# mir-group/nequip

Hardware: AMD Instinct MI355X
Metric: atom-steps/s (energy+forces) for 10k-atom l_max=2 box at 1/2/4/8 MI355X (higher is better)
Workload: dtype f32; 1 GPU; water10k: 10125-atom water box, 400558 edges, r_max 4.5, l_max=2, 64 features, 3 layers, parity=False, radial MLP 8-128(x1)-W, fp32 model / fp64 positions, energy+forces (autograd), random-init weights; atoms_per_gpu=10125, edges_per_gpu=400558, parallelism=replicas x1 (frames independent, no data-path collective), launch=hipGraph replay, radial-MLP backward on a side stream (parallel graph branch)

## Files before the change

include/nequip_amd.h:

```cpp
#ifndef NEQUIP_AMD_H
#define NEQUIP_AMD_H

#include <stdint.h>

#ifdef __cplusplus
extern "C" {
#endif

#define NQA_ABI_VERSION 1

enum nqa_status {
  NQA_OK = 0,
  NQA_ERR_INVALID = -1,
  NQA_ERR_UNSUPPORTED = -2,
  NQA_ERR_LAUNCH = -3,
  NQA_ERR_WORKSPACE = -4
};

enum nqa_dtype { NQA_F32 = 0, NQA_F64 = 1 };
enum nqa_layout { NQA_LAYOUT_MUL_IR = 0, NQA_LAYOUT_IR_MUL = 1 };

enum nqa_plan_field {
  NQA_PLAN_DIM_IN1 = 0,
  NQA_PLAN_DIM_IN2 = 1,
  NQA_PLAN_DIM_OUT = 2,
  NQA_PLAN_WEIGHT_NUMEL = 3,
  NQA_PLAN_NUM_INSTR = 4,
  NQA_PLAN_OUT_NEEDS_ZERO = 5,
  NQA_PLAN_YPART_WIDTH = 6,
  NQA_PLAN_HAS_SPECIALIZED = 7,
  NQA_PLAN_FUSED_ROWS_OK = 8
};

typedef struct nqa_plan nqa_plan;
typedef void* nqa_stream;

int nqa_abi_version(void);
const char* nqa_last_error(void);
int nqa_lmax(void);
int nqa_sh_lmax(void);

int nqa_plan_create(int32_t n_in1, const int32_t* in1_mul, const int32_t* in1_l, const int32_t* in1_p,
                    int32_t n_in2, const int32_t* in2_mul, const int32_t* in2_l, const int32_t* in2_p,
                    int32_t n_out, const int32_t* out_mul, const int32_t* out_l, const int32_t* out_p,
                    int32_t n_instr, const int32_t* instr_i1, const int32_t* instr_i2,
                    const int32_t* instr_io, const double* instr_path_weight,
                    int32_t layout_in1, int32_t layout_out, nqa_plan** plan);
void nqa_plan_destroy(nqa_plan* plan);
int64_t nqa_plan_query(const nqa_plan* plan, int32_t field);
int64_t nqa_plan_image_bytes(const nqa_plan* plan);
int nqa_plan_image_write(const nqa_plan* plan, void* host_dst, int64_t host_dst_bytes);

int64_t nqa_csr_workspace_bytes(int64_t num_nodes, int64_t num_edges);
int nqa_csr_build(const int64_t* key, const int64_t* other, int64_t num_nodes, int64_t num_edges,
                  int32_t* rowptr, int32_t* edge_id, int32_t* other_sorted, int32_t* status_flag,
                  void* workspace, int64_t workspace_bytes, nqa_stream stream);

int nqa_tp_scatter_fwd(const nqa_plan* plan, const void* plan_image, int32_t dtype, const void* x, const void* y, const void* w,
                       const int32_t* rowptr_dst, const int32_t* edge_id_dst, const int32_t* src_sorted,
                       void* out, int64_t num_nodes, int64_t num_edges, nqa_stream stream);

int64_t nqa_tp_bwd_edge_workspace_bytes(const nqa_plan* plan, int32_t dtype, int64_t num_edges);
int nqa_tp_scatter_bwd_edge(const nqa_plan* plan, const void* plan_image, int32_t dtype, const void* x, const void* y, const void* w,
                            const void* grad_out, const int32_t* rowptr_dst, const int32_t* edge_id_dst,
                            const int32_t* src_sorted, void* grad_w, void* grad_y, void* workspace,
                            int64_t workspace_bytes, int64_t num_nodes, int64_t num_edges, nqa_stream stream);

int nqa_tp_scatter_bwd_x(const nqa_plan* plan, const void* plan_image, int32_t dtype, const void* y, const void* w, const void* grad_out,
                         const int32_t* rowptr_src, const int32_t* edge_id_src, const int32_t* dst_sorted,
                         void* grad_x, int64_t num_nodes, int64_t num_edges, nqa_stream stream);

int64_t nqa_tp_bwd_fused_workspace_bytes(const nqa_plan* plan, int32_t dtype, int64_t num_edges);
int nqa_tp_scatter_bwd_fused(const nqa_plan* plan, const void* plan_image, int32_t dtype, const void* x, const void* y,
                             const void* w, const void* grad_out, const int32_t* rowptr_dst,
                             const int32_t* edge_id_dst, const int32_t* src_sorted, const int32_t* rowptr_src,
                             const int32_t* edge_id_src, void* grad_w, void* grad_y, void* grad_x, void* workspace,
                             int64_t workspace_bytes, int64_t num_nodes, int64_t num_edges, nqa_stream stream);

int nqa_edge_vectors_fwd(const double* pos, const int64_t* edge_dst, const int64_t* edge_src,
                         const double* edge_cell_shift, const double* cell, const int64_t* batch,
                         int64_t num_edges, double* edge_vec, nqa_stream stream);
int nqa_edge_vectors_bwd(const double* g_edge_vec, const double* edge_cell_shift, const int32_t* rowptr_dst,
                         const int32_t* edge_id_dst, const int32_t* rowptr_src, const int32_t* edge_id_src,
                         int64_t num_nodes, double sign, double* g_pos, double* g_cell_per_node, nqa_stream stream);
int nqa_virial_finalize(const double* per_atom, const int64_t* batch, const double* cell, int64_t num_nodes,
                        int64_t num_frames, double* virial, double* stress, nqa_stream stream);
int nqa_frame_sum(const double* rows, const int64_t* batch, int64_t num_nodes, int32_t width, int64_t num_frames,
                  double* out, nqa_stream stream);

int nqa_edge_embed_fwd(int32_t dtype, int32_t lmax, const double* edge_vec, int64_t num_edges,
                       double rmax_recip, const double* rmax_recip_edge, int32_t num_bessels,
                       const double* bessel_weights, double cutoff_p, double factor, void* sh, void* emb,
                       void* cutoff, nqa_stream stream);
int nqa_edge_embed_bwd(int32_t dtype, int32_t lmax, const double* edge_vec, int64_t num_edges,
                       double rmax_recip, const double* rmax_recip_edge, int32_t num_bessels,
                       const double* bessel_weights, double cutoff_p, double factor, const void* g_sh,
                       const void* g_emb, double* g_edge_vec, nqa_stream stream);
int nqa_edge_embed_fwd_paired(int32_t dtype, int32_t lmax, const double* edge_vec, int64_t num_edges,
                              double rmax_recip, int32_t num_bessels, const double* bessel_weights, double cutoff_p,
                              double factor, const int32_t* pair_row, int64_t num_pairs, void* sh, void* emb,
                              void* emb_pairs, nqa_stream stream);
int nqa_edge_embed_bwd_paired(int32_t dtype, int32_t lmax, const double* edge_vec, int64_t num_edges,
                              double rmax_recip, int32_t num_bessels, const double* bessel_weights, double cutoff_p,
                              double factor, const int32_t* pair_row, int64_t num_pairs, const void* g_sh,
                              const void* g_emb, const void* g_emb_pairs, double* g_edge_vec, nqa_stream stream);
int nqa_edge_embed_bwd_bwd(int32_t dtype, int32_t lmax, const double* edge_vec, int64_t num_edges,
                           double rmax_recip, const double* rmax_recip_edge, int32_t num_bessels,
                           const double* bessel_weights, double cutoff_p, double factor, const void* g_sh,
                           const void* g_emb, const double* cot_g_edge_vec, void* gg_sh, void* gg_emb,
                           double* g_edge_vec2, nqa_stream stream);

#define NQA_MLP_FP32 0
#define NQA_MLP_BF16X6 1
#define NQA_MLP_F16X3 2
#define NQA_MLP_HINT_DEVICE_IS_IDLE 0x100
int nqa_radial_mlp_supported(int32_t dtype, int32_t num_basis, int32_t hidden, int32_t out_features);
int64_t nqa_radial_mlp_workspace_bytes(int32_t mode, int32_t backward, int32_t hidden, int32_t out_features);
int nqa_radial_mlp_fwd(int32_t dtype, int32_t mode, const void* edge_embedding, const void* w0, double alpha0,
                       const void* w1, double alpha1, int32_t num_basis, int32_t hidden, int32_t out_features,
                       int64_t num_edges, void* edge_weight, void* workspace, int64_t workspace_bytes,
                       int32_t workspace_ready, nqa_stream stream);
int nqa_radial_mlp_bwd(int32_t dtype, int32_t mode, const void* edge_embedding, const void* w0, double alpha0,
                       const void* w1, double alpha1, const void* grad_edge_weight, int32_t num_basis,
                       int32_t hidden, int32_t out_features, int64_t num_edges, void* grad_edge_embedding,
                       void* workspace, int64_t workspace_bytes, int32_t workspace_ready, nqa_stream stream);

int nqa_radial_mlp_bwd_paired(int32_t dtype, int32_t mode, const void* edge_embedding, const void* w0, double alpha0,
                              const void* w1, double alpha1, const void* grad_edge_weight,
                              const void* grad_edge_weight2, int32_t num_basis, int32_t hidden, int32_t out_features,
                              int64_t num_edges, void* grad_edge_embedding, void* workspace, int64_t workspace_bytes,
                              int32_t workspace_ready, nqa_stream stream);
int64_t nqa_radial_mlp_train_tiles(int64_t num_edges);
int nqa_radial_mlp_bwd_train(int32_t dtype, int32_t mode, const void* edge_embedding, const void* cotangent,
                             const void* w0, double alpha0, const void* w1, double alpha1,
                             const void* grad_edge_weight, int32_t num_basis, int32_t hidden, int32_t out_features,
                             int64_t num_edges, void* grad_edge_embedding, void* hidden_out, void* w0_partials,
                             void* workspace, int64_t workspace_bytes, int32_t workspace_ready, nqa_stream stream);
int nqa_radial_mlp_fwd_tangent(int32_t dtype, int32_t mode, const void* edge_embedding, const void* cotangent,
                               const void* w0, double alpha0, const void* w1, double alpha1, int32_t num_basis,
                               int32_t hidden, int32_t out_features, int64_t num_edges, void* out, void* workspace,
                               int64_t workspace_bytes, int32_t workspace_ready, nqa_stream stream);

int nqa_radial_mlp_last_fwd(int32_t dtype, int32_t mode, const void* pre, const void* w, double alpha, int32_t hidden,
                            int32_t out_features, int64_t num_edges, void* out, void* workspace, int64_t workspace_bytes,
                            int32_t workspace_ready, nqa_stream stream);
int nqa_radial_mlp_last_bwd(int32_t dtype, int32_t mode, const void* pre, const void* w, double alpha,
                            const void* grad_out, const void* grad_out2, int32_t hidden, int32_t out_features,
                            int64_t num_edges, void* grad_pre, void* workspace, int64_t workspace_bytes,
                            int32_t workspace_ready, nqa_stream stream);


int nqa_node_linear(int32_t dtype, const void* x, const void* weights, const void* addend, void* out,
                    const int64_t* atom_types, const void* chunk_table, int32_t n_chunks, const void* instr_table,
                    int32_t n_instr, int32_t n_types, int64_t weight_stride, int32_t dim_in, int32_t dim_out,
                    int64_t num_nodes, double scale, int32_t chunk_width, nqa_stream stream);
int nqa_node_linear_ordered(int32_t dtype, const void* x, const void* weights, const void* addend, void* out,
                            const int64_t* atom_types, const int32_t* atom_order, const void* chunk_table, int32_t n_chunks,
                            const void* instr_table, int32_t n_instr, int32_t n_types, int64_t weight_stride,
                            int32_t dim_in, int32_t dim_out, int64_t num_nodes, double scale, int32_t chunk_width,
                            nqa_stream stream);
int nqa_gate(int32_t dtype, int32_t backward, const void* input, const void* grad_out, const void* cotangent,
             void* out, const void* col_table, int32_t dim_in, int32_t dim_out, int64_t num_nodes, nqa_stream stream);

int64_t nqa_node_weights_pack_bytes(const void* chunk_table, int32_t n_chunks, const void* instr_table, int32_t n_instr,
                                    int32_t n_types);
int nqa_node_weights_pack(const void* weights, const void* chunk_table, int32_t n_chunks, const void* instr_table,
                          int32_t n_instr, int32_t n_types, int64_t weight_stride, void* packed, nqa_stream stream);
int nqa_node_linear_packed(const void* x, const void* packed, const void* addend, void* out, const int64_t* atom_types,
                           const void* chunk_table, int32_t n_chunks, const void* instr_table, int32_t n_instr,
                           int32_t n_types, int32_t dim_in, int32_t dim_out, int64_t num_nodes, double scale,
                           nqa_stream stream);
int nqa_node_linear_packed_ordered(const void* x, const void* packed, const void* addend, void* out,
                                   const int64_t* atom_types, const int32_t* atom_order, const void* chunk_table,
                                   int32_t n_chunks, const void* instr_table, int32_t n_instr, int32_t n_types,
                                   int32_t dim_in, int32_t dim_out, int64_t num_nodes, double scale, nqa_stream stream);

typedef struct nqa_gate_block {
  int32_t out_off, d, mul, val_off, gate_off, act;
  double cst;
} nqa_gate_block;

typedef struct nqa_node_part {
  const void* x;
  const void* packed;
  const void* chunk_table;
  const void* instr_table;
  int32_t n_chunks, n_instr, n_types, dim_in;
  void* out;
  const void* addend;
  int32_t dim_out, accumulate;
  double scale;
  const nqa_gate_block* in_gate;
  int32_t n_in_gate, pad;
} nqa_node_part;

int nqa_node_fused(const nqa_node_part* parts, int32_t n_parts, const int64_t* atom_types, const int32_t* atom_order,
                   int64_t num_nodes, const nqa_gate_block* out_gate, int32_t n_out_gate, const void* gate_h,
                   int32_t gate_dim, nqa_stream stream);
int nqa_node_fused_plan(const nqa_node_part* parts, int32_t n_parts, const nqa_gate_block* out_gate, int32_t n_out_gate,
                        int32_t* chunks_out, int32_t chunks_cap, int32_t* instr_out, int32_t instr_cap);

int nqa_energy_head(int32_t backward, const void* h, const void* readout_weight, const void* scales, int32_t n_scales,
                    const void* shifts, int32_t n_shifts, const int64_t* atom_types, const void* grad_e, void* out,
                    int32_t dim, int32_t act, double cst, int64_t num_nodes, nqa_stream stream);

int64_t nqa_energy_head_train_workspace_bytes(int64_t num_nodes, int32_t dim, int32_t n_scales, int32_t n_shifts);
int nqa_energy_head_train_bwd(const void* h, const void* readout_weight, const void* scales, int32_t n_scales,
                              int32_t n_shifts, const int64_t* atom_types, const void* grad_e, void* grad_h, void* grad_w,
                              void* grad_scales, void* grad_shifts, void* workspace, int64_t workspace_bytes, int32_t dim,
                              int32_t act, double cst, int64_t num_nodes, nqa_stream stream);
int nqa_energy_head_train_bwd_bwd(const void* h, const void* readout_weight, const void* scales, int32_t n_scales,
                                  const int64_t* atom_types, const void* grad_e, const void* cot_grad_h, void* grad_grad_e,
                                  void* grad_h, void* grad_w, void* grad_scales, void* workspace, int64_t workspace_bytes,
                                  int32_t dim, int32_t act, double cst, int64_t num_nodes, nqa_stream stream);

int nqa_zbl_fwd(const double* edge_vec, const int32_t* rowptr_dst, const int32_t* edge_id_dst, const int32_t* src_sorted,
                const int64_t* atom_types, const double* z_table, const double* rmax_recip_edge, double rmax_recip, double p,
                int32_t round_f32, const double* qqr2e_half, int64_t num_nodes, int64_t num_out, const double* pe_in,
                double* pe_out, nqa_stream stream);
int nqa_zbl_bwd(const double* edge_vec, const int32_t* rowptr_dst, const int32_t* edge_id_dst, const int32_t* src_sorted,
                const int64_t* atom_types, const double* z_table, const double* rmax_recip_edge, double rmax_recip, double p,
                int32_t round_f32, const double* qqr2e_half, int64_t num_nodes, int64_t num_out, const double* g_pe,
                double* g_edge_vec, nqa_stream stream);
int nqa_zbl_bwd_bwd(const double* edge_vec, const int32_t* rowptr_dst, const int32_t* edge_id_dst,
                    const int32_t* src_sorted, const int64_t* atom_types, const double* z_table,
                    const double* rmax_recip_edge, double rmax_recip, double p, int32_t round_f32, const double* qqr2e_half,
                    int64_t num_nodes, int64_t num_out, const double* g_pe, const double* cot_edge_vec, double* gg_pe,
                    double* g_edge_vec2, nqa_stream stream);

int64_t nqa_edge_pairs_workspace_bytes(int64_t num_edges);
int nqa_edge_pairs(const int64_t* edge_dst, const int64_t* edge_src, const void* edge_cell_shift, int32_t shift_dtype,
                   const int32_t* rowptr_dst, const int32_t* edge_id_dst, const int32_t* src_sorted, int64_t num_edges,
                   int64_t num_nodes, void* workspace, int64_t workspace_bytes, int32_t* weight_rows, int64_t* rep_edge,
                   int32_t* partner_edge, int32_t* ok, nqa_stream stream);
int nqa_csr_from_pairs(const int32_t* edge_id_dst, const int32_t* partner_edge, int64_t num_edges, int32_t* edge_id_src,
                       nqa_stream stream);
int nqa_pair_gather(const void* rows_in, const int64_t* rep_edge, int64_t num_pairs, int32_t width, void* rows_out,
                    nqa_stream stream);
int64_t nqa_pair_owner_workspace_bytes(int64_t num_edges, int64_t num_nodes);
int nqa_pair_owner_lists(const int32_t* weight_rows, const int64_t* rep_edge, const int32_t* rowptr_dst,
                         const int32_t* edge_id_dst, const int32_t* src_sorted, int64_t num_edges, int64_t num_nodes,
                         void* workspace, int64_t workspace_bytes, int32_t* owner_rowptr, int32_t* pair_other,
                         int32_t* pair_row, int32_t* pair_edge_in, int32_t* pair_edge_out, int32_t* other_rowptr,
                         int32_t* other_slot, nqa_stream stream);
int nqa_pair_owner_lists_guard(const int32_t* ok, int64_t num_nodes, int32_t* owner_rowptr, int32_t* other_rowptr,
                               nqa_stream stream);
int nqa_pair_expand(const void* pair_rows, const int32_t* weight_rows, int64_t num_edges, int64_t num_pairs,
                    int32_t width, void* edge_rows, nqa_stream stream);
int nqa_tp_scatter_fwd_paired(const nqa_plan* plan, const void* plan_image, int32_t dtype, const void* x, const void* y,
                              const void* w, const int32_t* rowptr_dst, const int32_t* edge_id_dst,
                              const int32_t* src_sorted, void* out, int64_t num_nodes, int64_t num_edges,
                              const int32_t* weight_rows, int64_t num_pairs, nqa_stream stream);
int nqa_tp_scatter_bwd_edge_paired(const nqa_plan* plan, const void* plan_image, int32_t dtype, const void* x,
                                   const void* y, const void* w, const void* grad_out, const int32_t* rowptr_dst,
                                   const int32_t* edge_id_dst, const int32_t* src_sorted, void* grad_w, void* grad_y,
                                   void* workspace, int64_t workspace_bytes, int64_t num_nodes, int64_t num_edges,
                                   const int32_t* weight_rows, int64_t num_pairs, nqa_stream stream);
int nqa_tp_scatter_bwd_fused_paired(const nqa_plan* plan, const void* plan_image, int32_t dtype, const void* x,
                                    const void* y, const void* w, const void* grad_out, const int32_t* rowptr_dst,
                                    const int32_t* edge_id_dst, const int32_t* src_sorted, const int32_t* rowptr_src,
                                    const int32_t* edge_id_src, void* grad_w, void* grad_y, void* grad_x,
                                    void* workspace, int64_t workspace_bytes, int64_t num_nodes, int64_t num_edges,
                                    const int32_t* weight_rows, int64_t num_pairs, nqa_stream stream);
int nqa_tp_scatter_bwd_x_paired(const nqa_plan* plan, const void* plan_image, int32_t dtype, const void* y,
                                const void* w, const void* grad_out, const int32_t* rowptr_src,
                                const int32_t* edge_id_src, const int32_t* dst_sorted, void* grad_x, int64_t num_nodes,
                                int64_t num_edges, const int32_t* weight_rows, int64_t num_pairs, nqa_stream stream);

int64_t nqa_tp_bwd_pairs_workspace_bytes(const nqa_plan* plan, int32_t dtype, int64_t num_edges);
int nqa_tp_scatter_bwd_pairs(const nqa_plan* plan, const void* plan_image, int32_t dtype, const void* x, const void* y,
                             const void* w, const void* grad_out, const int32_t* owner_rowptr,
                             const int32_t* pair_other, const int32_t* pair_row, const int32_t* pair_edge_in,
                             const int32_t* pair_edge_out, const int32_t* other_rowptr, const int32_t* other_slot,
                             void* grad_w, void* grad_y, void* grad_x, void* workspace, int64_t workspace_bytes,
                             int64_t num_nodes, int64_t num_edges, nqa_stream stream);

int32_t nqa_tp_bwd_pairs_dual_supported(const nqa_plan* plan, int32_t dtype);
int nqa_tp_scatter_bwd_pairs_dual(const nqa_plan* plan, const void* plan_image, int32_t dtype, const void* x,
                                  const void* x_cot, const void* y, const void* y_cot, const void* w, const void* w_cot,
                                  const void* grad_out, const int32_t* owner_rowptr, const int32_t* pair_other,
                                  const int32_t* pair_row, const int32_t* pair_edge_in, const int32_t* pair_edge_out,
                                  void* grad_w, void* grad_y, void* workspace, int64_t workspace_bytes,
                                  int64_t num_nodes, int64_t num_edges, nqa_stream stream);

int32_t nqa_tp_fwd_jvp_supported(const nqa_plan* plan, int32_t dtype);
int nqa_tp_scatter_fwd_jvp(const nqa_plan* plan, const void* plan_image, int32_t dtype, const void* x, const void* y,
                           const void* w, const void* x_cot, const void* y_cot, const void* w_cot,
                           const int32_t* rowptr_dst, const int32_t* edge_id_dst, const int32_t* src_sorted, void* out,
                           int64_t num_nodes, int64_t num_edges, const int32_t* weight_rows, int64_t num_pairs,
                           nqa_stream stream);
int nqa_tp_scatter_bwd_x_dual(const nqa_plan* plan, const void* plan_image, int32_t dtype, const void* y, const void* w,
                              const void* y_cot, const void* w_cot, const void* grad_out, const int32_t* rowptr_src,
                              const int32_t* edge_id_src, const int32_t* dst_sorted, void* grad_x, int64_t num_nodes,
                              int64_t num_edges, const int32_t* weight_rows, int64_t num_pairs, nqa_stream stream);

int32_t nqa_wgrad_splits(const void* instr_table, int32_t n_instr, int32_t n_types, int64_t num_rows);
int nqa_wgrad(int32_t dtype, const void* a_rows, const void* b_rows, const int64_t* row_types,
              const void* instr_table, int32_t n_instr, int64_t lda, int64_t ldb, int64_t num_rows, int32_t n_types,
              int64_t out_stride, int32_t splits, void* partials, nqa_stream stream);

int64_t nqa_neighbor_list_workspace_bytes(int64_t num_atoms);
int nqa_neighbor_list_count(const double* pos, const double* cell, const int32_t* pbc, double r_max, int64_t num_atoms,
                            void* workspace, int64_t workspace_bytes, int32_t* rowptr, nqa_stream stream);
int nqa_neighbor_list_fill(const void* workspace, const int32_t* rowptr, int64_t num_atoms, int64_t num_edges,
                           int64_t* edge_index, double* edge_cell_shift, nqa_stream stream);
int nqa_neighbor_list_fill_padded(const void* workspace, const int32_t* rowptr, int64_t num_atoms, int64_t edge_capacity,
                                  int32_t* rowptr_padded, int64_t* edge_index, double* edge_cell_shift, int32_t* src_sorted,
                                  int32_t* status, nqa_stream stream);
int64_t nqa_neighbor_list_batched_workspace_bytes(int64_t num_atoms, int64_t num_frames);
int nqa_neighbor_list_batched_count(const double* pos, const double* cell, const int32_t* pbc, const int64_t* frame_ptr,
                                    double r_max, int64_t num_atoms, int64_t num_frames, void* workspace,
                                    int64_t workspace_bytes, int32_t* rowptr, int32_t* status, nqa_stream stream);
int nqa_neighbor_list_batched_fill(const void* workspace, const int32_t* rowptr, int64_t num_atoms, int64_t num_frames,
                                   int64_t num_edges, int64_t* edge_index, double* edge_cell_shift, nqa_stream stream);
int64_t nqa_neighbor_list_typed_workspace_bytes(int64_t num_atoms, int64_t num_types);
int nqa_neighbor_list_count_typed(const double* pos, const double* cell, const int32_t* pbc, double r_max,
                                  const int64_t* atom_types, const double* cutoff_table, int64_t num_types, int32_t symmetrise,
                                  int64_t num_atoms, void* workspace, int64_t workspace_bytes, int32_t* rowptr, int32_t* status,
                                  nqa_stream stream);
int nqa_neighbor_list_fill_typed(const void* workspace, const int32_t* rowptr, const int64_t* atom_types, int64_t num_atoms,
                                 int64_t num_types, int64_t num_edges, int64_t* edge_index, double* edge_cell_shift,
                                 nqa_stream stream);
int nqa_neighbor_list_fill_padded_typed(const void* workspace, const int32_t* rowptr, const int64_t* atom_types,
                                        int64_t num_atoms, int64_t num_types, int64_t edge_capacity, int32_t* rowptr_padded,
                                        int64_t* edge_index, double* edge_cell_shift, int32_t* src_sorted, int32_t* status,
                                        nqa_stream stream);
int64_t nqa_neighbor_list_batched_typed_workspace_bytes(int64_t num_atoms, int64_t num_frames, int64_t num_types);
int nqa_neighbor_list_batched_count_typed(const double* pos, const double* cell, const int32_t* pbc, const int64_t* frame_ptr,
                                          double r_max, const int64_t* atom_types, const double* cutoff_table,
                                          int64_t num_types, int64_t num_atoms, int64_t num_frames, void* workspace,
                                          int64_t workspace_bytes, int32_t* rowptr, int32_t* status, nqa_stream stream);
int nqa_neighbor_list_batched_fill_typed(const void* workspace, const int32_t* rowptr, const int64_t* atom_types,
                                         int64_t num_atoms, int64_t num_frames, int64_t num_types, int64_t num_edges,
                                         int64_t* edge_index, double* edge_cell_shift, nqa_stream stream);


#define NQA_METRICS_MAX_STREAMS 8
#define NQA_METRICS_MAX_TERMS 32
#define NQA_METRICS_MAX_TYPES 16
#define NQA_METRICS_MAX_STRATA 8
#define NQA_METRICS_GROUPS 64

enum nqa_metric_kind {
  NQA_METRIC_MSE = 0,
  NQA_METRIC_MAE = 1,
  NQA_METRIC_RMSE = 2,
  NQA_METRIC_MAXABS = 3,
  NQA_METRIC_HUBER = 4,
  NQA_METRIC_STRATIFIED_HUBER = 5
};

typedef struct nqa_metric_stream {
  const void* pred;
  const void* target;
  const double* row_scale;
  const int64_t* group;
  void* grad_pred;
  int64_t rows;
  int32_t cols, pred_dtype, target_dtype, pad;
} nqa_metric_stream;

typedef struct nqa_metric_term {
  int32_t stream, kind, n_groups, ignore_nan, reduce_sum, n_strata, has_coeff, has_group_coeffs, slot0, out0;
  double coeff, delta;
  double bound[NQA_METRICS_MAX_STRATA], stratum_delta[NQA_METRICS_MAX_STRATA];
  double group_coeff[NQA_METRICS_MAX_TYPES];
} nqa_metric_term;

int32_t nqa_metrics_groups(void);
int64_t nqa_metrics_workspace_bytes(int32_t n_slots);
int nqa_metrics_fwd(const nqa_metric_stream* streams, int32_t n_streams, const nqa_metric_term* terms,
                    const nqa_metric_term* terms_device, int32_t n_terms, int32_t n_values, int32_t weighted_sum_index,
                    void* workspace, int64_t workspace_bytes, void* state, void* saved, double* values, nqa_stream stream);
int nqa_metrics_bwd(const nqa_metric_stream* streams, int32_t n_streams, const nqa_metric_term* terms,
                    const nqa_metric_term* terms_device, int32_t n_terms, int32_t n_values, int32_t weighted_sum_index,
                    const void* saved, const double* grad_values, nqa_stream stream);

typedef struct nqa_mt_chunk {
  int64_t offset;
  int32_t tensor, pad;
} nqa_mt_chunk;

#define NQA_EMA_CHUNK 1024

typedef struct nqa_ema_tensor {
  void* ema;
  void* param;
  int64_t numel;
  int32_t dtype, pad;
} nqa_ema_tensor;

int32_t nqa_ema_chunk_elems(void);
int nqa_ema_update(const nqa_ema_tensor* tensors, const nqa_mt_chunk* chunks, int64_t chunk_capacity, const int64_t* n_chunks,
                   double decay, int64_t* counter, nqa_stream stream);
int nqa_ema_swap(const nqa_ema_tensor* tensors, const nqa_mt_chunk* chunks, int64_t chunk_capacity, const int64_t* n_chunks,
                 nqa_stream stream);

typedef struct nqa_sfree_tensor {
  void* param;
  void* grad;
  void* z;
  void* exp_avg_sq;
  int64_t numel;
  int32_t dtype, group;
} nqa_sfree_tensor;

typedef struct nqa_sfree_group {
  double lr, beta1, beta2, eps, weight_decay, r, weight_lr_power;
  int64_t warmup_steps;
  int64_t k;
  double weight_sum, lr_max, scheduled_lr;
} nqa_sfree_group;

int nqa_sfree_step(const nqa_sfree_tensor* tensors, const nqa_mt_chunk* chunks, int64_t chunk_capacity, const int64_t* n_chunks,
                   nqa_sfree_group* groups, int32_t n_groups, nqa_stream stream);
int nqa_sfree_swap(const nqa_sfree_tensor* tensors, const nqa_mt_chunk* chunks, int64_t chunk_capacity, const int64_t* n_chunks,
                   const nqa_sfree_group* groups, int32_t n_groups, int32_t to_eval, nqa_stream stream);

typedef struct nqa_adam_tensor {
  void* param;
  const void* grad;
  void* exp_avg;
  void* exp_avg_sq;
  void* max_exp_avg_sq;
  float* step;
  int64_t numel;
  int32_t dtype, group;
} nqa_adam_tensor;
// ... 171 lines not shown
```

nequip_amd/_lib.py:

```python

from __future__ import annotations

import ctypes
import os
import threading
from ctypes import POINTER, c_char_p, c_double, c_int32, c_int64, c_uint64, c_void_p

_HERE = os.path.dirname(os.path.abspath(__file__))
LIB_PATH = os.path.join(_HERE, "csrc", "libnequip_amd.so")

NQA_OK = 0
NQA_F32 = 0
NQA_F64 = 1
NQA_MLP_FP32 = 0
NQA_MLP_BF16X6 = 1
NQA_MLP_F16X3 = 2
NQA_MLP_HINT_DEVICE_IS_IDLE = 0x100
NQA_LAYOUT_MUL_IR = 0
NQA_LAYOUT_IR_MUL = 1

NQA_PLAN_DIM_IN1 = 0
NQA_PLAN_DIM_IN2 = 1
NQA_PLAN_DIM_OUT = 2
NQA_PLAN_WEIGHT_NUMEL = 3
NQA_PLAN_NUM_INSTR = 4
NQA_PLAN_OUT_NEEDS_ZERO = 5
NQA_PLAN_YPART_WIDTH = 6
NQA_PLAN_HAS_SPECIALIZED = 7
NQA_PLAN_FUSED_ROWS_OK = 8

_P32 = POINTER(c_int32)


class GateBlock(ctypes.Structure):

    _fields_ = [("out_off", c_int32), ("d", c_int32), ("mul", c_int32), ("val_off", c_int32), ("gate_off", c_int32),
                ("act", c_int32), ("cst", c_double)]


class NodePart(ctypes.Structure):

    _fields_ = [("x", c_void_p), ("packed", c_void_p), ("chunk_table", c_void_p), ("instr_table", c_void_p),
                ("n_chunks", c_int32), ("n_instr", c_int32), ("n_types", c_int32), ("dim_in", c_int32),
                ("out", c_void_p), ("addend", c_void_p), ("dim_out", c_int32), ("accumulate", c_int32),
                ("scale", c_double), ("in_gate", c_void_p), ("n_in_gate", c_int32), ("pad", c_int32)]


NQA_METRICS_MAX_STREAMS = 8
NQA_METRICS_MAX_TERMS = 32
NQA_METRICS_MAX_TYPES = 16
NQA_METRICS_MAX_STRATA = 8
NQA_METRICS_GROUPS = 64
NQA_METRIC_MSE, NQA_METRIC_MAE, NQA_METRIC_RMSE, NQA_METRIC_MAXABS, NQA_METRIC_HUBER, NQA_METRIC_STRATIFIED_HUBER = range(6)


class MetricStream(ctypes.Structure):

    _fields_ = [("pred", c_void_p), ("target", c_void_p), ("row_scale", c_void_p), ("group", c_void_p),
                ("grad_pred", c_void_p), ("rows", c_int64), ("cols", c_int32), ("pred_dtype", c_int32),
                ("target_dtype", c_int32), ("pad", c_int32)]


class MetricTerm(ctypes.Structure):

    _fields_ = [("stream", c_int32), ("kind", c_int32), ("n_groups", c_int32), ("ignore_nan", c_int32),
                ("reduce_sum", c_int32), ("n_strata", c_int32), ("has_coeff", c_int32), ("has_group_coeffs", c_int32),
                ("slot0", c_int32), ("out0", c_int32), ("coeff", c_double), ("delta", c_double),
                ("bound", c_double * NQA_METRICS_MAX_STRATA), ("stratum_delta", c_double * NQA_METRICS_MAX_STRATA),
                ("group_coeff", c_double * NQA_METRICS_MAX_TYPES)]


NQA_STATS_MAX_STREAMS = 8
NQA_STATS_MAX_TERMS = 32
NQA_STATS_MAX_NODE_TYPES = 128
NQA_STATS_MAX_EDGE_TYPES = 16
NQA_STATS_MAX_SLOTS = 1024
NQA_STATS_GROUPS = 256
NQA_STATS_F32, NQA_STATS_F64, NQA_STATS_I32, NQA_STATS_I64 = range(4)
NQA_STATS_MOD_IDENTITY, NQA_STATS_MOD_ABS, NQA_STATS_MOD_SQUARE = range(3)
NQA_STATS_GROUP_NONE, NQA_STATS_GROUP_NODE, NQA_STATS_GROUP_EDGE = range(3)


class StatsStream(ctypes.Structure):

    _fields_ = [("data", c_void_p), ("row_scale", c_void_p), ("atom_types", c_void_p), ("edge_index", c_void_p),
                ("rows", c_int64), ("num_atoms", c_int64), ("cols", c_int32), ("dtype", c_int32), ("group_kind", c_int32),
                ("num_types", c_int32)]


class StatsTerm(ctypes.Structure):

    _fields_ = [("stream", c_int32), ("mod", c_int32), ("n_groups", c_int32), ("ignore_nan", c_int32), ("slot0", c_int32),
                ("pad", c_int32 * 3)]


SIGNATURES = {
    "nqa_abi_version": (c_int32, []),
    "nqa_last_error": (c_char_p, []),
    "nqa_lmax": (c_int32, []),
    "nqa_sh_lmax": (c_int32, []),
    "nqa_plan_create": (
        c_int32,
        [c_int32, _P32, _P32, _P32, c_int32, _P32, _P32, _P32, c_int32, _P32, _P32, _P32]
        + [c_int32, _P32, _P32, _P32, POINTER(c_double), c_int32, c_int32, POINTER(c_void_p)],
    ),
    "nqa_plan_destroy": (None, [c_void_p]),
    "nqa_plan_query": (c_int64, [c_void_p, c_int32]),
    "nqa_plan_image_bytes": (c_int64, [c_void_p]),
    "nqa_plan_image_write": (c_int32, [c_void_p, c_void_p, c_int64]),
    "nqa_csr_workspace_bytes": (c_int64, [c_int64, c_int64]),
    "nqa_csr_build": (
        c_int32,
        [c_void_p, c_void_p, c_int64, c_int64, c_void_p, c_void_p, c_void_p, c_void_p, c_void_p, c_int64, c_void_p],
    ),
    "nqa_tp_scatter_fwd": (
        c_int32,
        [c_void_p, c_void_p, c_int32, c_void_p, c_void_p, c_void_p, c_void_p, c_void_p, c_void_p, c_void_p]
        + [c_int64, c_int64, c_void_p],
    ),
    "nqa_tp_bwd_edge_workspace_bytes": (c_int64, [c_void_p, c_int32, c_int64]),
    "nqa_tp_scatter_bwd_edge": (
        c_int32,
        [c_void_p, c_void_p, c_int32, c_void_p, c_void_p, c_void_p, c_void_p, c_void_p, c_void_p, c_void_p]
        + [c_void_p, c_void_p, c_void_p, c_int64, c_int64, c_int64, c_void_p],
    ),
    "nqa_tp_bwd_fused_workspace_bytes": (c_int64, [c_void_p, c_int32, c_int64]),
    "nqa_tp_scatter_bwd_fused": (
        c_int32,
        [c_void_p, c_void_p, c_int32, c_void_p, c_void_p, c_void_p, c_void_p]
        + [c_void_p] * 5
        + [c_void_p, c_void_p, c_void_p, c_void_p, c_int64, c_int64, c_int64, c_void_p],
    ),
    "nqa_tp_scatter_bwd_x": (
        c_int32,
        [c_void_p, c_void_p, c_int32, c_void_p, c_void_p, c_void_p, c_void_p, c_void_p, c_void_p, c_void_p]
        + [c_int64, c_int64, c_void_p],
    ),
    "nqa_frame_sum": (c_int32, [c_void_p, c_void_p, c_int64, c_int32, c_int64, c_void_p, c_void_p]),
    "nqa_edge_pairs_workspace_bytes": (c_int64, [c_int64]),
    "nqa_edge_pairs": (
        c_int32,
        [c_void_p, c_void_p, c_void_p, c_int32, c_void_p, c_void_p, c_void_p, c_int64, c_int64, c_void_p, c_int64, c_void_p,
         c_void_p, c_void_p, c_void_p, c_void_p],
    ),
    "nqa_csr_from_pairs": (c_int32, [c_void_p, c_void_p, c_int64, c_void_p, c_void_p]),
    "nqa_pair_owner_workspace_bytes": (c_int64, [c_int64, c_int64]),
    "nqa_pair_owner_lists": (
        c_int32,
        [c_void_p, c_void_p, c_void_p, c_void_p, c_void_p, c_int64, c_int64, c_void_p, c_int64, c_void_p, c_void_p, c_void_p,
         c_void_p, c_void_p, c_void_p, c_void_p, c_void_p],
    ),
    "nqa_pair_owner_lists_guard": (c_int32, [c_void_p, c_int64, c_void_p, c_void_p, c_void_p]),
    "nqa_pair_gather": (c_int32, [c_void_p, c_void_p, c_int64, c_int32, c_void_p, c_void_p]),
    "nqa_pair_expand": (c_int32, [c_void_p, c_void_p, c_int64, c_int64, c_int32, c_void_p, c_void_p]),
    "nqa_tp_bwd_pairs_workspace_bytes": (c_int64, [c_void_p, c_int32, c_int64]),
    "nqa_tp_scatter_bwd_pairs": (
        c_int32,
        [c_void_p, c_void_p, c_int32, c_void_p, c_void_p, c_void_p, c_void_p]
        + [c_void_p] * 7
        + [c_void_p, c_void_p, c_void_p, c_void_p, c_int64, c_int64, c_int64, c_void_p],
    ),
    "nqa_tp_fwd_jvp_supported": (c_int32, [c_void_p, c_int32]),
    "nqa_tp_scatter_fwd_jvp": (
        c_int32,
        [c_void_p, c_void_p, c_int32] + [c_void_p] * 6
        + [c_void_p, c_void_p, c_void_p, c_void_p, c_int64, c_int64, c_void_p, c_int64, c_void_p],
    ),
    "nqa_tp_scatter_bwd_x_dual": (
        c_int32,
        [c_void_p, c_void_p, c_int32] + [c_void_p] * 5
        + [c_void_p, c_void_p, c_void_p, c_void_p, c_int64, c_int64, c_void_p, c_int64, c_void_p],
    ),
    "nqa_tp_bwd_pairs_dual_supported": (c_int32, [c_void_p, c_int32]),
    "nqa_tp_scatter_bwd_pairs_dual": (
        c_int32,
        [c_void_p, c_void_p, c_int32] + [c_void_p] * 7
        + [c_void_p] * 5
        + [c_void_p, c_void_p, c_void_p, c_int64, c_int64, c_int64, c_void_p],
    ),
    "nqa_edge_vectors_fwd": (
        c_int32,
        [c_void_p, c_void_p, c_void_p, c_void_p, c_void_p, c_void_p, c_int64, c_void_p, c_void_p],
    ),
    "nqa_edge_vectors_bwd": (
        c_int32,
        [c_void_p, c_void_p, c_void_p, c_void_p, c_void_p, c_void_p, c_int64, c_double, c_void_p, c_void_p, c_void_p],
    ),
    "nqa_virial_finalize": (c_int32, [c_void_p, c_void_p, c_void_p, c_int64, c_int64, c_void_p, c_void_p, c_void_p]),
    "nqa_edge_embed_fwd": (
        c_int32,
        [c_int32, c_int32, c_void_p, c_int64, c_double, c_void_p, c_int32, c_void_p, c_double, c_double]
        + [c_void_p, c_void_p, c_void_p, c_void_p],
    ),
    "nqa_edge_embed_bwd": (
        c_int32,
        [c_int32, c_int32, c_void_p, c_int64, c_double, c_void_p, c_int32, c_void_p, c_double, c_double]
        + [c_void_p, c_void_p, c_void_p, c_void_p],
    ),
    "nqa_edge_embed_fwd_paired": (
        c_int32,
        [c_int32, c_int32, c_void_p, c_int64, c_double, c_int32, c_void_p, c_double, c_double, c_void_p, c_int64]
        + [c_void_p, c_void_p, c_void_p, c_void_p],
    ),
    "nqa_edge_embed_bwd_paired": (
        c_int32,
        [c_int32, c_int32, c_void_p, c_int64, c_double, c_int32, c_void_p, c_double, c_double, c_void_p, c_int64]
        + [c_void_p, c_void_p, c_void_p, c_void_p, c_void_p],
    ),
    "nqa_edge_embed_bwd_bwd": (
        c_int32,
        [c_int32, c_int32, c_void_p, c_int64, c_double, c_void_p, c_int32, c_void_p, c_double, c_double]
        + [c_void_p, c_void_p, c_void_p, c_void_p, c_void_p, c_void_p, c_void_p],
    ),
    "nqa_radial_mlp_supported": (c_int32, [c_int32, c_int32, c_int32, c_int32]),
    "nqa_radial_mlp_workspace_bytes": (c_int64, [c_int32, c_int32, c_int32, c_int32]),
    "nqa_radial_mlp_fwd": (
        c_int32,
        [c_int32, c_int32, c_void_p, c_void_p, c_double, c_void_p, c_double, c_int32, c_int32, c_int32, c_int64]
        + [c_void_p, c_void_p, c_int64, c_int32, c_void_p],
    ),
    "nqa_radial_mlp_bwd": (
        c_int32,
        [c_int32, c_int32, c_void_p, c_void_p, c_double, c_void_p, c_double, c_void_p, c_int32, c_int32, c_int32]
        + [c_int64, c_void_p, c_void_p, c_int64, c_int32, c_void_p],
    ),
    "nqa_node_linear": (
        c_int32,
        [c_int32, c_void_p, c_void_p, c_void_p, c_void_p, c_void_p, c_void_p, c_int32, c_void_p, c_int32, c_int32]
        + [c_int64, c_int32, c_int32, c_int64, c_double, c_int32, c_void_p],
    ),
    "nqa_node_weights_pack_bytes": (c_int64, [c_void_p, c_int32, c_void_p, c_int32, c_int32]),
    "nqa_node_weights_pack": (
        c_int32, [c_void_p, c_void_p, c_int32, c_void_p, c_int32, c_int32, c_int64, c_void_p, c_void_p],
    ),
    "nqa_node_linear_packed": (
        c_int32,
        [c_void_p, c_void_p, c_void_p, c_void_p, c_void_p, c_void_p, c_int32, c_void_p, c_int32, c_int32, c_int32, c_int32]
        + [c_int64, c_double, c_void_p],
    ),
    "nqa_node_linear_ordered": (
        c_int32,
        [c_int32, c_void_p, c_void_p, c_void_p, c_void_p, c_void_p, c_void_p, c_void_p, c_int32, c_void_p, c_int32, c_int32,
         c_int64, c_int32, c_int32, c_int64, c_double, c_int32, c_void_p],
    ),
    "nqa_node_linear_packed_ordered": (
        c_int32,
        [c_void_p, c_void_p, c_void_p, c_void_p, c_void_p, c_void_p, c_void_p, c_int32, c_void_p, c_int32, c_int32, c_int32]
        + [c_int32, c_int64, c_double, c_void_p],
    ),
    "nqa_node_fused": (
        c_int32, [c_void_p, c_int32, c_void_p, c_void_p, c_int64, c_void_p, c_int32, c_void_p, c_int32, c_void_p],
    ),
    "nqa_node_fused_plan": (c_int32, [c_void_p, c_int32, c_void_p, c_int32, _P32, c_int32, _P32, c_int32]),
    "nqa_radial_mlp_last_fwd": (
        c_int32,
        [c_int32, c_int32, c_void_p, c_void_p, c_double, c_int32, c_int32, c_int64, c_void_p, c_void_p, c_int64, c_int32,
         c_void_p],
    ),
    "nqa_radial_mlp_last_bwd": (
        c_int32,
        [c_int32, c_int32, c_void_p, c_void_p, c_double, c_void_p, c_void_p, c_int32, c_int32, c_int64, c_void_p, c_void_p,
         c_int64, c_int32, c_void_p],
    ),
    "nqa_energy_head": (
        c_int32,
        [c_int32, c_void_p, c_void_p, c_void_p, c_int32, c_void_p, c_int32, c_void_p, c_void_p, c_void_p, c_int32, c_int32,
         c_double, c_int64, c_void_p],
    ),
    "nqa_energy_head_train_workspace_bytes": (c_int64, [c_int64, c_int32, c_int32, c_int32]),
    "nqa_energy_head_train_bwd": (
        c_int32,
        [c_void_p, c_void_p, c_void_p, c_int32, c_int32, c_void_p, c_void_p, c_void_p, c_void_p, c_void_p, c_void_p, c_void_p,
         c_int64, c_int32, c_int32, c_double, c_int64, c_void_p],
    ),
    "nqa_energy_head_train_bwd_bwd": (
        c_int32,
        [c_void_p, c_void_p, c_void_p, c_int32, c_void_p, c_void_p, c_void_p, c_void_p, c_void_p, c_void_p, c_void_p, c_void_p,
         c_int64, c_int32, c_int32, c_double, c_int64, c_void_p],
    ),
    "nqa_zbl_fwd": (
        c_int32,
        [c_void_p, c_void_p, c_void_p, c_void_p, c_void_p, c_void_p, c_void_p, c_double, c_double, c_int32, c_void_p, c_int64,
         c_int64, c_void_p, c_void_p, c_void_p],
    ),
    "nqa_zbl_bwd": (
        c_int32,
        [c_void_p, c_void_p, c_void_p, c_void_p, c_void_p, c_void_p, c_void_p, c_double, c_double, c_int32, c_void_p, c_int64,
         c_int64, c_void_p, c_void_p, c_void_p],
    ),
    "nqa_zbl_bwd_bwd": (
        c_int32,
        [c_void_p, c_void_p, c_void_p, c_void_p, c_void_p, c_void_p, c_void_p, c_double, c_double, c_int32, c_void_p, c_int64,
         c_int64, c_void_p, c_void_p, c_void_p, c_void_p, c_void_p],
    ),
    "nqa_neighbor_list_workspace_bytes": (c_int64, [c_int64]),
    "nqa_neighbor_list_count": (
        c_int32,
        [c_void_p, c_void_p, c_void_p, c_double, c_int64, c_void_p, c_int64, c_void_p, c_void_p],
    ),
    "nqa_neighbor_list_fill": (c_int32, [c_void_p, c_void_p, c_int64, c_int64, c_void_p, c_void_p, c_void_p]),
    "nqa_neighbor_list_fill_padded": (
        c_int32, [c_void_p, c_void_p, c_int64, c_int64, c_void_p, c_void_p, c_void_p, c_void_p, c_void_p, c_void_p]),
    "nqa_neighbor_list_batched_workspace_bytes": (c_int64, [c_int64, c_int64]),
    "nqa_neighbor_list_batched_count": (
        c_int32,
        [c_void_p, c_void_p, c_void_p, c_void_p, c_double, c_int64, c_int64, c_void_p, c_int64, c_void_p, c_void_p, c_void_p],
    ),
    "nqa_neighbor_list_batched_fill": (c_int32, [c_void_p, c_void_p, c_int64, c_int64, c_int64, c_void_p, c_void_p, c_void_p]),
    "nqa_neighbor_list_typed_workspace_bytes": (c_int64, [c_int64, c_int64]),
    "nqa_neighbor_list_count_typed": (
        c_int32,
        [c_void_p, c_void_p, c_void_p, c_double, c_void_p, c_void_p, c_int64, c_int32, c_int64, c_void_p, c_int64, c_void_p,
         c_void_p, c_void_p],
# ... 151 lines not shown
```

nequip_amd/csrc/radial_mlp.hip:

```cpp
#include <hip/hip_runtime.h>

#include <cstdint>
#include <cstdlib>
#include <string>
#include <type_traits>

#include "launch_status.h"
#include "mfma_split.h"

namespace nqa {

constexpr int kMlpRows = 128;
constexpr int kMaxNb = 8;

typedef float mlp_v4f __attribute__((ext_vector_type(4)));
__device__ __forceinline__ void mlp_store4(float* p, const float4& v) {
  __builtin_nontemporal_store((mlp_v4f){v.x, v.y, v.z, v.w}, reinterpret_cast<mlp_v4f*>(p));
}

__device__ __forceinline__ void lds_barrier() { asm volatile("s_waitcnt lgkmcnt(0)\n\ts_barrier" ::: "memory"); }

__device__ __forceinline__ float silu_f(float x) { return x / (1.0f + __expf(-x)); }
__device__ __forceinline__ void silu_all_f(float x, float& h, float& d1, float& d2) {
  const float sig = 1.0f / (1.0f + __expf(-x));
// ... 698 lines not shown
      } else {
#pragma unroll
        for (int s2 = 0; s2 < kMaxNb / 2; ++s2) {
          const float av = (2 * s2 + half) < nb ? w0v[kb][s2] * a0 : 0.f;
          const float bv = half ? e[2 * s2 + 1] : e[2 * s2];
          hacc = __builtin_amdgcn_mfma_f32_32x32x2f32(av, bv, hacc, 0, 0, 0);
        }
      }
#pragma unroll
      for (int r = 0; r < 16; r += 2) {
        const float h0 = row_ok ? (XIN ? silu_given_f(hacc[r]) : silu_f(hacc[r])) : 0.f;
        const float h1 = row_ok ? (XIN ? silu_given_f(hacc[r + 1]) : silu_f(hacc[r + 1])) : 0.f;
        if constexpr (F16) {
          hv[kb * 16 + r] = h0;
          hv[kb * 16 + r + 1] = h1;
        } else {
          uint32_t a, b, c;
          split_pair(h0, h1, a, b, c);
          const int s = 2 * kb + (r >> 3), tp = (r & 7) >> 1;
          bh[s][tp] = a; bm[s][tp] = b; bl[s][tp] = c;
        }
      }
    }
    if constexpr (F16) {
      float m = 0.f;
#pragma unroll
      for (int i = 0; i < (H / 32) * 16; ++i) m = fmaxf(m, fabsf(hv[i]));
      m = fmaxf(m, __shfl_xor(m, 32));
      const float su = f16_scale_up(m);
      row_scale = 1.f / su;
#pragma unroll
      for (int kb = 0; kb < H / 32; ++kb) {
#pragma unroll
        for (int r = 0; r < 16; r += 2) {
          uint32_t a, b;
          split_pair_f16(hv[kb * 16 + r] * su, hv[kb * 16 + r + 1] * su, a, b);
          const int s = 2 * kb + (r >> 3), tp = (r & 7) >> 1;
          bh[s][tp] = a; bl[s][tp] = b;
        }
      }
    }
  };
  hidden(ev, blk * kMlpRows + wv * 32 + l31 < E, blk);

  float* __restrict__ tb = tbuf + wv * (32 * kTS);
  auto emit = [&](const f32x16& pa, const f32x16& pb, int tile, int64_t wrow0, float rs) __attribute__((always_inline)) {
    if constexpr (F16) {
      const float f = rs * tile_scale[tile];
#pragma unroll
      for (int g = 0; g < 4; ++g)
        *reinterpret_cast<float4*>(tb + l31 * kTS + 8 * g + 4 * half) =
            make_float4((pa[4 * g] + pb[4 * g]) * f, (pa[4 * g + 1] + pb[4 * g + 1]) * f,
                        (pa[4 * g + 2] + pb[4 * g + 2]) * f, (pa[4 * g + 3] + pb[4 * g + 3]) * f);
    } else {
#pragma unroll
      for (int g = 0; g < 4; ++g)
        *reinterpret_cast<float4*>(tb + l31 * kTS + 8 * g + 4 * half) =
            make_float4(pa[4 * g] + pb[4 * g], pa[4 * g + 1] + pb[4 * g + 1], pa[4 * g + 2] + pb[4 * g + 2],
                        pa[4 * g + 3] + pb[4 * g + 3]);
    }
    const int n0 = tile * 32;
    const int c4 = lane & 7, rsub = lane >> 3;
    if (wrow0 + 32 <= E && n0 + 32 <= W) {
      float* __restrict__ ob = out + (wrow0 + rsub) * W + n0 + 4 * c4;
#pragma unroll
      for (int i = 0; i < 4; ++i)
        mlp_store4(ob + (int64_t)(8 * i) * W, *reinterpret_cast<const float4*>(tb + (8 * i + rsub) * kTS + 4 * c4));
    } else {
#pragma unroll
      for (int i = 0; i < 4; ++i) {
        const int r = 8 * i + rsub;
        const float4 v = *reinterpret_cast<const float4*>(tb + r * kTS + 4 * c4);
        if (wrow0 + r < E && n0 + 4 * c4 + 3 < W) *reinterpret_cast<float4*>(out + (wrow0 + r) * W + n0 + 4 * c4) = v;
      }
    }
  };
  int prev_tile = 0;
  int64_t prev_row0 = 0;
  float prev_rs = 1.f;
  auto unit = [&](int64_t i, f32x16& accA, f32x16& accB, const f32x16& prevA, const f32x16& prevB)
      __attribute__((always_inline)) {
    const int64_t left = (u1 - u0) - i;
    if (t == 0 && i > 0) {
      ++blk;
#pragma unroll
      for (int c = 0; c < kMaxNb; ++c) ev[c] = evn[c];
      hidden(ev, blk * kMlpRows + wv * 32 + l31 < E, blk);
    }
    const int buf = (int)(i & 1);
    if (left > 1) stage_store(buf ^ 1);
    if (left > 2) stage_load(tile_after(t, 2));
    if (t == ntiles - 1 && left > 1) load_ev(blk + 1, evn);
    const u32x4* __restrict__ a = as[buf] + lane;
    accA = (f32x16){0};
    accB = (f32x16){0};
    u32x4 fa[2][NPL];
#pragma unroll
    for (int q = 0; q < NPL; ++q) fa[0][q] = a[q * 64];
#pragma unroll
    for (int s = 0; s < KS; ++s) {
      if (s + 1 < KS) {
#pragma unroll
        for (int q = 0; q < NPL; ++q) fa[(s + 1) & 1][q] = a[((s + 1) * NPL + q) * 64];
      }
      __builtin_amdgcn_sched_barrier(0);
      if constexpr (F16) {
        const u32x4 &ah = fa[s & 1][0], &al = fa[s & 1][1];
        if (s & 1) {
          accB = mfma_f16(ah, bl[s], accB);
          accA = mfma_f16(al, bh[s], accA);
          accB = mfma_f16(ah, bh[s], accB);
        } else {
          accA = mfma_f16(ah, bl[s], accA);
          accB = mfma_f16(al, bh[s], accB);
          accA = mfma_f16(ah, bh[s], accA);
        }
      } else {
        const u32x4 &ah = fa[s & 1][0], &am = fa[s & 1][1], &al = fa[s & 1][2];
        accA = mfma_bf16(ah, bh[s], accA);
        accB = mfma_bf16(am, bm[s], accB);
        accA = mfma_bf16(ah, bm[s], accA);
        accB = mfma_bf16(ah, bl[s], accB);
        accA = mfma_bf16(am, bh[s], accA);
        accB = mfma_bf16(al, bh[s], accB);
      }
      __builtin_amdgcn_sched_barrier(0);
      if (s == 1 && i > 0) {
        emit(prevA, prevB, prev_tile, prev_row0, prev_rs);
        __builtin_amdgcn_sched_barrier(0);
      }
    }
    lds_barrier();
    prev_tile = t;
    prev_row0 = blk * kMlpRows + wv * 32;
    prev_rs = row_scale;
    if (++t == ntiles) t = 0;
  };
  f32x16 a0A, a0B, a1A, a1B;
  const int64_t n = u1 - u0;
  for (int64_t i = 0; i < n; i += 2) {
    unit(i, a0A, a0B, a1A, a1B);
    if (i + 1 < n) unit(i + 1, a1A, a1B, a0A, a0B);
  }
  if (n & 1)
    emit(a0A, a0B, prev_tile, prev_row0, prev_rs);
  else
    emit(a1A, a1B, prev_tile, prev_row0, prev_rs);
}

}
#include "radial_mlp_pipe.h"
namespace nqa {

template <int H, int TM, bool PAIR = false, bool F16 = false, bool XIN = false>
__global__ __launch_bounds__(256, 2) void radial_mlp_bwd_split_kernel(const float* __restrict__ emb,
                                                                    const float* __restrict__ W0,
                                                                    const u32x4* __restrict__ Wb,
                                                                    const float* __restrict__ gw, float a0, int nb,
                                                                    int W, int64_t E, float* __restrict__ g_emb,
                                                                    int dbg, const float* __restrict__ cemb,
                                                                    float* __restrict__ hid_out,
                                                                    float* __restrict__ w0_part,
                                                                    const float* __restrict__ gw2 = nullptr,
                                                                    const int* __restrict__ chunk_exp = nullptr) {
  constexpr int NT = H / 32;
  constexpr int NPL = F16 ? 2 : 3;
  constexpr int CH = 2 * NPL * NT * 64;
  constexpr int NV = CH / 256;
  constexpr int GS = H + 1;
  constexpr int kMainBytes = 2 * CH * 16;
  constexpr int kEpiBytes = kMlpRows * GS * 4;
  constexpr int kBufBytes = kMainBytes > kEpiBytes ? kMainBytes : kEpiBytes;
  __shared__ __align__(16) unsigned char smem_raw[kBufBytes];
  __shared__ float w0s[H * kMaxNb];
  __shared__ float w0t[kMaxNb * H];
  __shared__ float es[kMlpRows * kMaxNb];
  __shared__ int rowexp[F16 ? kMlpRows : 1];
  __shared__ float cs_own[(TM == 2 && H * kMaxNb < kMlpRows * kMaxNb) ? kMlpRows * kMaxNb : 1];
  float* __restrict__ cs = (H * kMaxNb >= kMlpRows * kMaxNb) ? w0s : cs_own;
  u32x4* __restrict__ bsm = reinterpret_cast<u32x4*>(smem_raw);
  const int tid = threadIdx.x;
  const int lane = tid & 63;
  const int wv = tid >> 6;
  const int half = lane >> 5;
  const int l31 = lane & 31;
  const int64_t blk0 = (int64_t)blockIdx.x * kMlpRows;
  const int64_t myrow = blk0 + wv * 32 + l31;
  const bool row_ok = myrow < E;

  if constexpr (!XIN) {
    for (int i = tid; i < H * kMaxNb; i += 256) {
      const int k = i / kMaxNb, c = i - k * kMaxNb;
      const float v = c < nb ? W0[c * H + k] * a0 : 0.f;
      w0s[i] = v;
      w0t[c * H + k] = v;
    }
    for (int i = tid; i < kMlpRows * kMaxNb; i += 256) {
      const int r = i / kMaxNb, c = i - r * kMaxNb;
      const int64_t rr = blk0 + r < E ? blk0 + r : E - 1;
      const float v = emb[rr * nb + (c < nb ? c : nb - 1)];
      es[i] = (c < nb && blk0 + r < E) ? v : 0.f;
    }
  }
  float cvr[kMaxNb];
  if (TM == 2) {
    const float* __restrict__ cr = cemb + (row_ok ? myrow : (E - 1)) * nb;
#pragma unroll
    for (int c = 0; c < kMaxNb; ++c) cvr[c] = cr[c < nb ? c : nb - 1];
#pragma unroll
    for (int c = 0; c < kMaxNb; ++c) cvr[c] = (row_ok && c < nb) ? cvr[c] : 0.f;
  }

  const int nchunks = (W + 31) / 32;
  u32x4 pb[NV];
  const float* __restrict__ grow = gw + (row_ok ? myrow : 0) * W + 16 * half;
  const float* __restrict__ grow2 = PAIR ? gw2 + (row_ok ? myrow : 0) * W + 16 * half : nullptr;
  const bool rows_full = blk0 + kMlpRows <= E;
  auto load_rows = [&](const float* __restrict__ gr, int ch, float4 (&pa)[4]) {
    if (rows_full && 32 * ch + 32 <= W) {
#pragma unroll
      for (int v = 0; v < 4; ++v) pa[v] = *reinterpret_cast<const float4*>(gr + 32 * ch + 4 * v);
    } else {
#pragma unroll
      for (int v = 0; v < 4; ++v) {
        const int k = 32 * ch + 16 * half + 4 * v;
        pa[v] = (row_ok && k + 3 < W) ? *reinterpret_cast<const float4*>(gr + 32 * ch + 4 * v)
                                      : make_float4(0.f, 0.f, 0.f, 0.f);
      }
    }
  };
  auto load_a = [&](int ch, float4 (&pa)[4], float4 (&pc)[4]) {
    if (dbg & 1) return;
    load_rows(grow, ch, pa);
    if (PAIR) load_rows(grow2, ch, pc);
  };
  auto load_b = [&](int ch) {
#pragma unroll
    for (int v = 0; v < NV; ++v) pb[v] = Wb[(int64_t)ch * CH + tid + v * 256];
  };
  auto store_b = [&](int buf) {
#pragma unroll
    for (int v = 0; v < NV; ++v) bsm[buf * CH + tid + v * 256] = pb[v];
  };
  float4 paA[4], paB[4];
  float4 pcA[PAIR ? 4 : 1], pcB[PAIR ? 4 : 1];
  load_b(0);
  load_a(0, paA, reinterpret_cast<float4(&)[4]>(pcA));
  store_b(0);
  if (nchunks > 1) load_a(1, paB, reinterpret_cast<float4(&)[4]>(pcB));
  __syncthreads();

  f32x16 acc[NT];
#pragma unroll
  for (int t = 0; t < NT; ++t) acc[t] = (f32x16){0};
  constexpr int kUnset = 1 << 20;
  int S = kUnset;
  int we_next = F16 ? chunk_exp[0] : 0;
  auto rows_from_lanes = [&](int value, int (&out)[16]) __attribute__((always_inline)) {
    int* __restrict__ rb = rowexp + wv * 32;
    if (half == 0) rb[l31] = value;
    __builtin_amdgcn_fence(__ATOMIC_RELEASE, "wavefront");
    __builtin_amdgcn_wave_barrier();
    __builtin_amdgcn_fence(__ATOMIC_ACQUIRE, "wavefront");
#pragma unroll
    for (int r = 0; r < 16; ++r) out[r] = rb[(r & 3) + 8 * (r >> 2) + 4 * half];
    __builtin_amdgcn_fence(__ATOMIC_RELEASE, "wavefront");
    __builtin_amdgcn_wave_barrier();
  };

  auto body = [&](int ch, float4 (&pa)[4], float4 (&pc)[4]) {
    const int buf = ch & 1;
    if (PAIR) {
#pragma unroll
      for (int v = 0; v < 4; ++v) {
        pa[v].x += pc[v].x; pa[v].y += pc[v].y; pa[v].z += pc[v].z; pa[v].w += pc[v].w;
      }
    }
    u32x4 ah[2], am[F16 ? 1 : 2], al[2];
    if constexpr (F16) {
      const int we = we_next;
      if (ch + 1 < nchunks) we_next = chunk_exp[ch + 1];
      float m = 0.f;
#pragma unroll
      for (int v = 0; v < 4; ++v)
        m = fmaxf(m, fmaxf(fmaxf(fabsf(pa[v].x), fabsf(pa[v].y)), fmaxf(fabsf(pa[v].z), fabsf(pa[v].w))));
      m = fmaxf(m, __shfl_xor(m, 32));
      int shift = 0;
      if (m > 0.f && m < 3.0e38f) {
        int em;
        (void)frexpf(m, &em);
        const int cap = 15 - em + we;
        if (cap < S) {
          int ns = cap - 3;
          ns = ns > we + 100 ? we + 100 : (ns < we - 100 ? we - 100 : ns);
          shift = S == kUnset ? 0 : S - ns;
          S = ns;
        }
      }
      if (ch > 0 && __any(shift > 0)) {
        int kr[16];
        rows_from_lanes(shift, kr);
#pragma unroll
        for (int t = 0; t < NT; ++t)
#pragma unroll
          for (int r = 0; r < 16; ++r) acc[t][r] = ldexpf(acc[t][r], -kr[r]);
      }
      int q = S == kUnset ? 0 : S - we;
      q = q > 120 ? 120 : (q < -120 ? -120 : q);
      const float qs = ldexpf(1.f, q);
#pragma unroll
      for (int s = 0; s < 2; ++s) {
        uint32_t a, b;
        split_pair_f16(pa[2 * s].x * qs, pa[2 * s].y * qs, a, b);
        ah[s][0] = a; al[s][0] = b;
        split_pair_f16(pa[2 * s].z * qs, pa[2 * s].w * qs, a, b);
        ah[s][1] = a; al[s][1] = b;
        split_pair_f16(pa[2 * s + 1].x * qs, pa[2 * s + 1].y * qs, a, b);
// ... 23 lines not shown
      if constexpr (F16) {
#pragma unroll
        for (int q = 0; q < 2; ++q)
#pragma unroll
          for (int t = 0; t < NT; ++t) fb[q][t] = bs[((s * 2 + q) * NT + t) * 64];
        __builtin_amdgcn_sched_barrier(0);
#pragma unroll
        for (int t = 0; t < NT; ++t) acc[t] = mfma_f16(al[s], fb[0][t], acc[t]);
#pragma unroll
        for (int t = 0; t < NT; ++t) acc[t] = mfma_f16(ah[s], fb[1][t], acc[t]);
#pragma unroll
        for (int t = 0; t < NT; ++t) acc[t] = mfma_f16(ah[s], fb[0][t], acc[t]);
        __builtin_amdgcn_sched_barrier(0);
        continue;
      }
      if (!(dbg & 16) || ch == 0) {
#pragma unroll
        for (int q = 0; q < 3; ++q)
#pragma unroll
          for (int t = 0; t < NT; ++t) fb[q][t] = bs[((s * 3 + q) * NT + t) * 64];
      } else {
#pragma unroll
        for (int q = 0; q < 3; ++q)
#pragma unroll
          for (int t = 0; t < NT; ++t) fb[q][t] = (u32x4){0x3f803f80u + (unsigned)lane, 0x3c003c00u, 0x38003800u + (unsigned)t, 0x3f803f80u + (unsigned)q};
      }
      __builtin_amdgcn_sched_barrier(0);
#pragma unroll
      for (int t = 0; t < NT; ++t) acc[t] = mfma_bf16(am[s], fb[1][t], acc[t]);
#pragma unroll
      for (int t = 0; t < NT; ++t) acc[t] = mfma_bf16(ah[s], fb[2][t], acc[t]);
#pragma unroll
      for (int t = 0; t < NT; ++t) acc[t] = mfma_bf16(al[s], fb[0][t], acc[t]);
#pragma unroll
      for (int t = 0; t < NT; ++t) acc[t] = mfma_bf16(ah[s], fb[1][t], acc[t]);
#pragma unroll
      for (int t = 0; t < NT; ++t) acc[t] = mfma_bf16(am[s], fb[0][t], acc[t]);
#pragma unroll
      for (int t = 0; t < NT; ++t) acc[t] = mfma_bf16(ah[s], fb[0][t], acc[t]);
      __builtin_amdgcn_sched_barrier(0);
    }
    if (ch + 1 < nchunks && !(dbg & 2) && !((dbg & 8) && (ch & 1))) store_b(buf ^ 1);
    if (!(dbg & 4)) lds_barrier();
  };
  for (int ch = 0; ch < nchunks; ch += 2) {
    body(ch, paA, reinterpret_cast<float4(&)[4]>(pcA));
    if (ch + 1 < nchunks) body(ch + 1, paB, reinterpret_cast<float4(&)[4]>(pcB));
  }

  if constexpr (F16) {
    int sr[16];
    rows_from_lanes(S == kUnset ? 0 : S, sr);
#pragma unroll
    for (int t = 0; t < NT; ++t)
#pragma unroll
      for (int r = 0; r < 16; ++r) acc[t][r] = ldexpf(acc[t][r], -sr[r]);
  }
  if constexpr (XIN) {
    static_assert(!XIN || TM == 0, "XIN is an inference backward");
#pragma unroll
    for (int t = 0; t < NT; ++t) {
      const int col = t * 32 + l31;
      float pv[16];
#pragma unroll
      for (int r = 0; r < 16; ++r) {
        const int64_t row = blk0 + wv * 32 + (r & 3) + 8 * (r >> 2) + 4 * half;
        pv[r] = emb[(row < E ? row : (E - 1)) * H + col];
      }
#pragma unroll
      for (int r = 0; r < 16; ++r) {
        const int64_t row = blk0 + wv * 32 + (r & 3) + 8 * (r >> 2) + 4 * half;
        if (row < E) g_emb[row * H + col] = acc[t][r] * silu_grad_given_f(pv[r]);
      }
    }
    return;
  }
  float* __restrict__ gp = reinterpret_cast<float*>(smem_raw);
  {
    const float* __restrict__ erow = es + (wv * 32 + l31) * kMaxNb;
#pragma unroll
    for (int t = 0; t < NT; ++t) {
      f32x16 pacc = {0};
#pragma unroll
      for (int s2 = 0; s2 < kMaxNb / 2; ++s2) {
        const float av = erow[2 * s2 + half];
        const float bv = w0t[(2 * s2 + half) * H + t * 32 + l31];
        pacc = __builtin_amdgcn_mfma_f32_32x32x2f32(av, bv, pacc, 0, 0, 0);
      }
      f32x16 qacc = {0};
      if (TM == 2) {
#pragma unroll
        for (int s2 = 0; s2 < kMaxNb / 2; ++s2) {
          const float av = half ? cvr[2 * s2 + 1] : cvr[2 * s2];
          const float bv = w0t[(2 * s2 + half) * H + t * 32 + l31];
          qacc = __builtin_amdgcn_mfma_f32_32x32x2f32(av, bv, qacc, 0, 0, 0);
        }
      }
      const int col = t * 32 + l31;
      if (TM == 0) {
#pragma unroll
        for (int r = 0; r < 16; ++r) {
          const int lr = wv * 32 + (r & 3) + 8 * (r >> 2) + 4 * half;
          gp[lr * GS + col] = acc[t][r] * silu_grad_f(pacc[r]);
        }
      } else {
        float hv[16];
#pragma unroll
        for (int r = 0; r < 16; ++r) {
          const int lr = wv * 32 + (r & 3) + 8 * (r >> 2) + 4 * half;
          float h, d1, d2;
          silu_all_f(pacc[r], h, d1, d2);
          if (TM == 1) {
            gp[lr * GS + col] = acc[t][r] * d1;
            hv[r] = h;
          } else {
            gp[lr * GS + col] = qacc[r] * acc[t][r] * d2;
            hv[r] = qacc[r] * d1;
            acc[t][r] *= d1;
          }
        }
        float* __restrict__ hrow = hid_out + (blk0 + wv * 32 + 4 * half) * (int64_t)H + col;
        if (rows_full) {
#pragma unroll
          for (int r = 0; r < 16; ++r) hrow[(int64_t)((r & 3) + 8 * (r >> 2)) * H] = hv[r];
        } else {
#pragma unroll
          for (int r = 0; r < 16; ++r) {
            const int lr = wv * 32 + (r & 3) + 8 * (r >> 2) + 4 * half;
            if (blk0 + lr < E) hrow[(int64_t)((r & 3) + 8 * (r >> 2)) * H] = hv[r];
          }
        }
      }
    }
  }
  __syncthreads();
  {
    const int r = tid >> 1, kh = tid & 1;
    float sacc[kMaxNb];
#pragma unroll
    for (int c = 0; c < kMaxNb; ++c) sacc[c] = 0.f;
    const float* __restrict__ gr = gp + r * GS + kh * (H / 2);
    const float* __restrict__ wr = w0s + kh * (H / 2) * kMaxNb;
#pragma unroll 4
    for (int k = 0; k < H / 2; ++k) {
      const float gv = gr[k];
      const float4 w0 = *reinterpret_cast<const float4*>(wr + k * kMaxNb);
      const float4 w1 = *reinterpret_cast<const float4*>(wr + k * kMaxNb + 4);
      sacc[0] += gv * w0.x; sacc[1] += gv * w0.y; sacc[2] += gv * w0.z; sacc[3] += gv * w0.w;
      sacc[4] += gv * w1.x; sacc[5] += gv * w1.y; sacc[6] += gv * w1.z; sacc[7] += gv * w1.w;
    }
#pragma unroll
    for (int c = 0; c < kMaxNb; ++c) sacc[c] += __shfl_xor(sacc[c], 1, 64);
    if (kh == 0 && blk0 + r < E) {
      for (int c = 0; c < nb; ++c) g_emb[(blk0 + r) * nb + c] = sacc[c];
    }
  }
  if (TM != 0) {
    constexpr int NCG = 256 / H, CPT = kMaxNb / NCG;
    const int k = tid % H, cg = tid / H;
    float part[CPT];
#pragma unroll
    for (int i = 0; i < CPT; ++i) part[i] = 0.f;
    for (int r = 0; r < kMlpRows; ++r) {
      const float gv = gp[r * GS + k];
#pragma unroll
      for (int i = 0; i < CPT; ++i) part[i] += es[r * kMaxNb + cg * CPT + i] * gv;
    }
    if (TM == 2) {
      __syncthreads();
#pragma unroll
      for (int t = 0; t < NT; ++t)
#pragma unroll
        for (int r = 0; r < 16; ++r)
          gp[(wv * 32 + (r & 3) + 8 * (r >> 2) + 4 * half) * GS + t * 32 + l31] = acc[t][r];
      if (half == 0) {
#pragma unroll
        for (int c = 0; c < kMaxNb; ++c) cs[(wv * 32 + l31) * kMaxNb + c] = cvr[c];
      }
      __syncthreads();
      for (int r = 0; r < kMlpRows; ++r) {
        const float gv = gp[r * GS + k];
#pragma unroll
        for (int i = 0; i < CPT; ++i) part[i] += cs[r * kMaxNb + cg * CPT + i] * gv;
      }
    }
    float* __restrict__ wp = w0_part + (int64_t)blockIdx.x * nb * H;
#pragma unroll
    for (int i = 0; i < CPT; ++i) {
      const int c = cg * CPT + i;
      if (c < nb) wp[c * H + k] = part[i];
    }
  }
}

}

using namespace nqa;

namespace {

int mlp_num_cus() {
  static const int num_cus = [] {
    int dev = 0, n = 0;
    if (hipGetDevice(&dev) != hipSuccess ||
        hipDeviceGetAttribute(&n, hipDeviceAttributeMultiprocessorCount, dev) != hipSuccess || n <= 0)
      n = 256;
    return n;
  }();
  return num_cus;
}

struct MlpLayout {
  int64_t total;
  int64_t second;
};
MlpLayout mlp_layout(int32_t mode, int32_t backward, int32_t H, int32_t W) {
  if (H <= 0 || W <= 0) return {-1, -1};
  const int64_t n32 = (W + 31) / 32;
  if (mode == NQA_MLP_F16X3) {
    const int64_t frag = backward ? n32 * 2 * 2 * (H / 32) * 1024 : n32 * (H / 16) * 2 * 1024;
    return {frag + ((n32 * 4 + 255) & ~(int64_t)255), frag};
  }
  if (mode == NQA_MLP_BF16X6) return {n32 * (H / 16) * 3 * 1024, -1};
  if (mode != NQA_MLP_FP32) return {-1, -1};
  if (!backward) return {0, -1};
  return {(int64_t)H * W * (int64_t)sizeof(float) + 4 * 64 * H * (int64_t)sizeof(float), -1};
}
struct MlpWorkspace {
  u32x4* fragments;
  void* second;
  template <class T>
  T* second_as() const { return static_cast<T*>(second); }
};
MlpWorkspace mlp_view(void* workspace, const MlpLayout& lay) {
  return {static_cast<u32x4*>(workspace),
          lay.second < 0 ? nullptr : reinterpret_cast<void*>(static_cast<char*>(workspace) + lay.second)};
}

int fail(int rc, const std::string& text) {
  set_error(text);
  return rc;
}

struct MlpCall {
  const char* fn;
  int32_t dtype, mode;
  bool xin;
  const void *in, *w0;
  double alpha0;
  const void* w1;
  double alpha1;
  int32_t nb, H, W;
  int64_t E;
  void* workspace;
  int64_t workspace_bytes;
  int32_t workspace_ready;
  nqa_stream stream;
};

int mlp_check(const MlpCall& c, bool io_ok) {
  const std::string fn(c.fn);
  const bool h_ok = c.H == 64 || c.H == 128;
  if (c.xin) {
    if (c.dtype != NQA_F32 || c.mode != NQA_MLP_F16X3)
      return fail(NQA_ERR_UNSUPPORTED, fn + ": float32 on the two-plane fp16 split (NQA_MLP_F16X3) only");
    if (c.E < 0 || !h_ok || c.W <= 0 || c.W % 4 != 0 || (c.E > 0 && (!c.in || !c.w1 || !io_ok)))
      return fail(h_ok ? NQA_ERR_INVALID : NQA_ERR_UNSUPPORTED,
                  fn + ": invalid argument (hidden 64 / 128, out_features % 4 == 0)");
    return NQA_OK;
  }
  if (c.dtype != NQA_F32) return fail(NQA_ERR_UNSUPPORTED, fn + ": only float32 is implemented on MFMA");
  if (c.mode != NQA_MLP_FP32 && c.mode != NQA_MLP_BF16X6 && c.mode != NQA_MLP_F16X3)
    return fail(NQA_ERR_INVALID, fn + ": unknown mode");
  if (c.E < 0 || c.nb <= 0 || c.nb > kMaxNb || c.W <= 0 || (c.E > 0 && (!c.in || !c.w0 || !c.w1)))
    return fail(NQA_ERR_INVALID, fn + ": invalid argument");
  if (!h_ok) return fail(NQA_ERR_UNSUPPORTED, fn + ": hidden width must be 64 or 128 for the fused MFMA kernel");
  return NQA_OK;
}

template <int V>
using ic = std::integral_constant<int, V>;
template <class F>
void by_h(int H, F&& f) {
  if (H == 128) f(ic<128>{});
  else f(ic<64>{});
}
template <class F>
void by_h_tm_pair(int H, int tm, bool pair, F&& f) {
  by_h(H, [&](auto h) {
    if (pair) f(h, ic<0>{}, std::true_type{});
    else if (tm == 0) f(h, ic<0>{}, std::false_type{});
    else if (tm == 1) f(h, ic<1>{}, std::false_type{});
    else f(h, ic<2>{}, std::false_type{});
  });
}

int mlp_fwd(const MlpCall& c, const void* cotangent, void* out) {
  const std::string fn(c.fn);
  int rc = mlp_check(c, out != nullptr);
  if (rc != NQA_OK || c.E == 0) return rc;
  if (out == nullptr || c.W % 4 != 0) return fail(NQA_ERR_INVALID, fn + ": invalid output (needs out_features % 4 == 0)");
  const MlpLayout lay = mlp_layout(c.mode, 0, c.H, c.W);
  if (lay.total > 0 && (c.workspace == nullptr || c.workspace_bytes < lay.total))
    return fail(NQA_ERR_WORKSPACE, fn + ": workspace missing or too small");
  if (cotangent != nullptr && c.mode != NQA_MLP_BF16X6)
    return fail(NQA_ERR_UNSUPPORTED,
                c.mode == NQA_MLP_F16X3
                    ? "nqa_radial_mlp_fwd_tangent: NQA_MLP_F16X3 is a mode of the plain forward (use NQA_MLP_BF16X6)"
                    : "nqa_radial_mlp_fwd_tangent: only NQA_MLP_BF16X6 is implemented");
  const MlpWorkspace ws = mlp_view(c.workspace, lay);
  hipStream_t s = static_cast<hipStream_t>(c.stream);
  const int nb = c.nb, H = c.H, W = c.W;
  const int64_t E = c.E;
  const float a0 = (float)c.alpha0, a1 = (float)c.alpha1;
  const float* e = static_cast<const float*>(c.in);
  const float* a = static_cast<const float*>(c.w0);
  const float* b = static_cast<const float*>(c.w1);
  float* o = static_cast<float*>(out);
  u32x4* wf = ws.fragments;
  const int ntiles = (W + 31) / 32;
  const unsigned grid = (unsigned)((E + kMlpRows - 1) / kMlpRows);
  const auto balanced_grid = [&] {
    const int64_t units = (int64_t)grid * ntiles, slots = 2 * (int64_t)mlp_num_cus();
    return (unsigned)(units < slots ? units : slots);
  };
  if (c.mode == NQA_MLP_F16X3) {
    float* ts = ws.second_as<float>();
    if (!c.workspace_ready)
      hipLaunchKernelGGL(radial_mlp_split_w1_fwd_f16_kernel, dim3((unsigned)ntiles), dim3(256), 0, s, b, a1, H, W, wf, ts);
    const unsigned gb = balanced_grid();
    if (!c.xin && env_flag("NQA_MLP_PIPE", true) && H == 128 && W % 32 == 0 && ntiles <= 128) {
      if (env_flag("NQA_MLP_PIPE_DIRECT", false))
        hipLaunchKernelGGL((radial_mlp_fwd_pipe_kernel<128, true>), dim3(gb), dim3(256), 0, s, e, a, wf, a0, nb, W, E, o, ts);
      else
        hipLaunchKernelGGL((radial_mlp_fwd_pipe_kernel<128, false>), dim3(gb), dim3(256), 0, s, e, a, wf, a0, nb, W, E, o, ts);
      return launch_status(c.fn);
    }
    by_h(H, [&](auto h) {
      constexpr int HH = decltype(h)::value;
      if (c.xin)
        hipLaunchKernelGGL((radial_mlp_fwd_split_bal_kernel<HH, true, true>), dim3(gb), dim3(256), 0, s, e, a, wf, a0, nb,
                           W, E, o, ts);
      else
        hipLaunchKernelGGL((radial_mlp_fwd_split_bal_kernel<HH, true>), dim3(gb), dim3(256), 0, s, e, a, wf, a0, nb, W, E,
                           o, ts);
    });
    return launch_status(c.fn);
  }
  if (c.mode == NQA_MLP_BF16X6) {
    const int nfrag = ntiles * (H / 16) * 64;
    if (!c.workspace_ready)
      hipLaunchKernelGGL(radial_mlp_split_w1_fwd_kernel, dim3((unsigned)((nfrag + 255) / 256)), dim3(256), 0, s, b, a1, H,
                         W, wf);
    if (cotangent != nullptr) {
      const float* ct = static_cast<const float*>(cotangent);
      by_h(H, [&](auto h) {
        hipLaunchKernelGGL((radial_mlp_fwd_bf16x6_kernel<decltype(h)::value, true>), dim3(grid), dim3(256), 0, s, e, a, wf,
                           a0, nb, W, E, o, ct);
      });
      return launch_status("nqa_radial_mlp_fwd_tangent");
    }
    if (env_flag("NQA_MLP_FWD_BALANCED", true)) {
      const unsigned gb = balanced_grid();
      by_h(H, [&](auto h) {
        hipLaunchKernelGGL((radial_mlp_fwd_split_bal_kernel<decltype(h)::value, false>), dim3(gb), dim3(256), 0, s, e, a,
                           wf, a0, nb, W, E, o, nullptr);
      });
      return launch_status(c.fn);
    }
    by_h(H, [&](auto h) {
      hipLaunchKernelGGL((radial_mlp_fwd_bf16x6_kernel<decltype(h)::value>), dim3(grid), dim3(256), 0, s, e, a, wf, a0, nb,
                         W, E, o, nullptr);
    });
    return launch_status(c.fn);
  }
  by_h(H, [&](auto h) {
    hipLaunchKernelGGL(radial_mlp_fwd_kernel<decltype(h)::value>, dim3(grid), dim3(256), 0, s, e, a, b, a0, a1, nb, W, E,
                       o, 0);
  });
  return launch_status(c.fn);
}

int mlp_bwd(MlpCall c, int tm, const void* cotangent, void* hidden_out, void* w0_partials, const void* gw, const void* gw2,
            void* grad_in) {
  const std::string fn(c.fn);
  const bool device_idle = !c.xin && (c.mode & NQA_MLP_HINT_DEVICE_IS_IDLE) != 0;
  if (!c.xin) c.mode &= ~NQA_MLP_HINT_DEVICE_IS_IDLE;
  int rc = mlp_check(c, gw != nullptr && grad_in != nullptr);
  if (rc != NQA_OK || c.E == 0) return rc;
  if (gw == nullptr || grad_in == nullptr || c.W % 4 != 0)
    return fail(NQA_ERR_INVALID, fn + ": invalid argument (needs out_features % 4 == 0)");
  const MlpLayout lay = mlp_layout(c.mode, 1, c.H, c.W);
  if (c.workspace == nullptr || c.workspace_bytes < lay.total)
    return fail(NQA_ERR_WORKSPACE, fn + ": workspace missing or too small");
  if (c.mode == NQA_MLP_FP32 && (tm != 0 || gw2 != nullptr))
    return fail(NQA_ERR_UNSUPPORTED,
                "nqa_radial_mlp_bwd_train / _paired: NQA_MLP_BF16X6 or NQA_MLP_F16X3 (no exact-fp32 form)");
  if (gw2 != nullptr && tm != 0) return fail(NQA_ERR_UNSUPPORTED, "nqa_radial_mlp_bwd_paired: inference backward only");
  const MlpWorkspace ws = mlp_view(c.workspace, lay);
  hipStream_t s = static_cast<hipStream_t>(c.stream);
  const int nb = c.nb, H = c.H, W = c.W;
  const int64_t E = c.E;
  const float a0 = (float)c.alpha0, a1 = (float)c.alpha1;
  const float* e = static_cast<const float*>(c.in);
  const float* a = static_cast<const float*>(c.w0);
  const float* b = static_cast<const float*>(c.w1);
  const float* g = static_cast<const float*>(gw);
  const float* g2 = static_cast<const float*>(gw2);
  const float* ct = static_cast<const float*>(cotangent);
  float* ho = static_cast<float*>(hidden_out);
  float* wp = static_cast<float*>(w0_partials);
  float* o = static_cast<float*>(grad_in);
  u32x4* wb = ws.fragments;
  const int nchunks = (W + 31) / 32;
  const unsigned grid = (unsigned)((E + kMlpRows - 1) / kMlpRows);
  const char* launch_fn = g2 != nullptr && !c.xin ? "nqa_radial_mlp_bwd_paired" : c.fn;
  if (c.mode == NQA_MLP_F16X3) {
    int* ce = ws.second_as<int>();
    if (!c.workspace_ready)
      hipLaunchKernelGGL(radial_mlp_split_w1_bwd_f16_kernel, dim3((unsigned)nchunks), dim3(256), 0, s, b, a1, H, W, wb, ce);
    if (!c.xin && tm == 0 && g2 == nullptr && env_flag("NQA_MLP_PIPE", true)) {
      const int small_mode = env_int("NQA_MLP_BWD_SMALL", 0);
      if ((small_mode == 2 || (small_mode == 1 && device_idle)) && H == 128 && W % 32 == 0 && W <= 256) {
        const size_t lds = (size_t)nchunks * (2 * 2 * (H / 32) * 64) * 16 + (size_t)(H / 32) * 16 * 2 * kMaxNb * 4 +
                           (size_t)kMaxNb * H * 4 + (((size_t)nchunks * 4 + 15) & ~(size_t)15);
        static bool attr_set = false;
        if (!attr_set) {
          if (hipFuncSetAttribute(reinterpret_cast<const void*>(&radial_mlp_bwd_small_kernel<128>),
                                  hipFuncAttributeMaxDynamicSharedMemorySize, 160 * 1024 - 512) != hipSuccess) {
            (void)hipGetLastError();
          }
          attr_set = true;
        }
        const int64_t want = ((E + 31) / 32 + 7) / 8;
        const unsigned gb = (unsigned)(want < (int64_t)mlp_num_cus() ? want : (int64_t)mlp_num_cus());
        hipLaunchKernelGGL((radial_mlp_bwd_small_kernel<128>), dim3(gb), dim3(512), lds, s, e, a, wb, g, a0, nb, W, E, o, ce);
        return launch_status(c.fn);
      }
      const bool balanced = env_flag("NQA_MLP_BWD_BALANCED", false);
      const bool use_coal = env_flag("NQA_MLP_BWD_COAL", false) && H == 128 && W % 64 == 0;
      if (use_coal || (balanced && W % 32 == 0)) {
        const int per_cu = env_int("NQA_MLP_BWD_WGS_PER_CU", 2);
        const int64_t slots = (int64_t)(per_cu >= 1 && per_cu <= 2 ? per_cu : 2) * mlp_num_cus();
        const unsigned gb = (unsigned)((int64_t)grid < slots ? (int64_t)grid : slots);
        if (hipMemsetAsync(o, 0, (size_t)E * nb * sizeof(float), s) != hipSuccess)
          return fail(NQA_ERR_LAUNCH, fn + ": hipMemsetAsync failed");
        const auto launch = [&](auto h, auto pf) {
          hipLaunchKernelGGL((radial_mlp_bwd_pipe_kernel<decltype(h)::value, decltype(pf)::value>), dim3(gb), dim3(256), 0,
                             s, e, a, wb, g, a0, nb, W, E, o, ce);
        };
        if (use_coal && !balanced)
          hipLaunchKernelGGL((radial_mlp_bwd_coal_kernel<128>), dim3(gb), dim3(256), 0, s, e, a, wb, g, a0, nb, W, E, o, ce);
        else if (H == 64) launch(ic<64>{}, ic<2>{});
        else if (env_int("NQA_MLP_BWD_PF", 2) == 4) launch(ic<128>{}, ic<4>{});
        else launch(ic<128>{}, ic<2>{});
        return launch_status(c.fn);
      }
    }
    by_h_tm_pair(H, tm, g2 != nullptr, [&](auto h, auto t, auto p) {
      constexpr int HH = decltype(h)::value, TT = decltype(t)::value;
      constexpr bool PP = decltype(p)::value;
      if constexpr (TT == 0) {
        if (c.xin) {
          hipLaunchKernelGGL((radial_mlp_bwd_split_kernel<HH, 0, PP, true, true>), dim3(grid), dim3(256), 0, s, e, a, wb, g,
                             a0, nb, W, E, o, 0, ct, ho, wp, g2, ce);
          return;
        }
      }
      hipLaunchKernelGGL((radial_mlp_bwd_split_kernel<HH, TT, PP, true>), dim3(grid), dim3(256), 0, s, e, a, wb, g, a0, nb,
                         W, E, o, 0, ct, ho, wp, g2, ce);
    });
    return launch_status(launch_fn);
  }
  if (c.mode == NQA_MLP_BF16X6) {
    const int nfrag = nchunks * 2 * (H / 32) * 64;
    if (!c.workspace_ready)
      hipLaunchKernelGGL(radial_mlp_split_w1_bwd_kernel, dim3((unsigned)((nfrag + 255) / 256)), dim3(256), 0, s, b, a1, H,
                         W, wb);
    by_h_tm_pair(H, tm, g2 != nullptr, [&](auto h, auto t, auto p) {
      constexpr int HH = decltype(h)::value, TT = decltype(t)::value;
      constexpr bool PP = decltype(p)::value;
      hipLaunchKernelGGL((radial_mlp_bwd_split_kernel<HH, TT, PP>), dim3(grid), dim3(256), 0, s, e, a, wb, g, a0, nb, W, E,
                         o, 0, ct, ho, wp, g2, nullptr);
    });
    return launch_status(launch_fn);
  }
  float* w1t = static_cast<float*>(c.workspace);
  if (!c.workspace_ready)
    hipLaunchKernelGGL(radial_mlp_transpose_w1_kernel, dim3((unsigned)((H * W + 255) / 256)), dim3(256), 0, s, b, a1, H, W,
                       w1t);
  by_h(H, [&](auto h) {
    hipLaunchKernelGGL(radial_mlp_bwd_kernel<decltype(h)::value>, dim3(grid), dim3(256), 0, s, e, a, w1t, g, a0, nb, W, E,
                       o);
  });
  return launch_status(c.fn);
}

}

extern "C" {

int nqa_radial_mlp_supported(int32_t dtype, int32_t num_basis, int32_t hidden, int32_t out_features) {
  return (dtype == NQA_F32 && num_basis > 0 && num_basis <= kMaxNb && (hidden == 64 || hidden == 128) &&
          out_features > 0 && out_features % 4 == 0)
             ? 1
             : 0;
}

int64_t nqa_radial_mlp_workspace_bytes(int32_t mode, int32_t backward, int32_t hidden, int32_t out_features) {
  return mlp_layout(mode, backward, hidden, out_features).total;
}

int64_t nqa_radial_mlp_train_tiles(int64_t num_edges) {
  return num_edges <= 0 ? 0 : (num_edges + kMlpRows - 1) / kMlpRows;
}

int nqa_radial_mlp_fwd(int32_t dtype, int32_t mode, const void* edge_embedding, const void* w0, double alpha0,
                       const void* w1, double alpha1, int32_t num_basis, int32_t hidden, int32_t out_features,
                       int64_t num_edges, void* edge_weight, void* workspace, int64_t workspace_bytes,
                       int32_t workspace_ready, nqa_stream stream) {
  return mlp_fwd({"nqa_radial_mlp_fwd", dtype, mode, false, edge_embedding, w0, alpha0, w1, alpha1, num_basis, hidden,
                  out_features, num_edges, workspace, workspace_bytes, workspace_ready, stream},
                 nullptr, edge_weight);
}

int nqa_radial_mlp_fwd_tangent(int32_t dtype, int32_t mode, const void* edge_embedding, const void* cotangent,
                               const void* w0, double alpha0, const void* w1, double alpha1, int32_t num_basis,
                               int32_t hidden, int32_t out_features, int64_t num_edges, void* out, void* workspace,
                               int64_t workspace_bytes, int32_t workspace_ready, nqa_stream stream) {
  if (num_edges > 0 && cotangent == nullptr)
    return fail(NQA_ERR_INVALID, "nqa_radial_mlp_fwd_tangent: cotangent is required");
  return mlp_fwd({"nqa_radial_mlp_fwd", dtype, mode, false, edge_embedding, w0, alpha0, w1, alpha1, num_basis, hidden,
                  out_features, num_edges, workspace, workspace_bytes, workspace_ready, stream},
                 cotangent, out);
}

int nqa_radial_mlp_bwd(int32_t dtype, int32_t mode, const void* edge_embedding, const void* w0, double alpha0,
                       const void* w1, double alpha1, const void* grad_edge_weight, int32_t num_basis,
                       int32_t hidden, int32_t out_features, int64_t num_edges, void* grad_edge_embedding,
                       void* workspace, int64_t workspace_bytes, int32_t workspace_ready, nqa_stream stream) {
  return mlp_bwd({"nqa_radial_mlp_bwd", dtype, mode, false, edge_embedding, w0, alpha0, w1, alpha1, num_basis, hidden,
                  out_features, num_edges, workspace, workspace_bytes, workspace_ready, stream},
                 0, nullptr, nullptr, nullptr, grad_edge_weight, nullptr, grad_edge_embedding);
}

int nqa_radial_mlp_bwd_paired(int32_t dtype, int32_t mode, const void* edge_embedding, const void* w0, double alpha0,
                              const void* w1, double alpha1, const void* grad_edge_weight,
                              const void* grad_edge_weight2, int32_t num_basis, int32_t hidden, int32_t out_features,
                              int64_t num_edges, void* grad_edge_embedding, void* workspace, int64_t workspace_bytes,
                              int32_t workspace_ready, nqa_stream stream) {
  if (num_edges > 0 && grad_edge_weight2 == nullptr)
    return fail(NQA_ERR_INVALID, "nqa_radial_mlp_bwd_paired: second gradient stream is required");
  return mlp_bwd({"nqa_radial_mlp_bwd", dtype, mode, false, edge_embedding, w0, alpha0, w1, alpha1, num_basis, hidden,
                  out_features, num_edges, workspace, workspace_bytes, workspace_ready, stream},
                 0, nullptr, nullptr, nullptr, grad_edge_weight, grad_edge_weight2, grad_edge_embedding);
}

int nqa_radial_mlp_bwd_train(int32_t dtype, int32_t mode, const void* edge_embedding, const void* cotangent,
                             const void* w0, double alpha0, const void* w1, double alpha1,
                             const void* grad_edge_weight, int32_t num_basis, int32_t hidden, int32_t out_features,
                             int64_t num_edges, void* grad_edge_embedding, void* hidden_out, void* w0_partials,
                             void* workspace, int64_t workspace_bytes, int32_t workspace_ready, nqa_stream stream) {
  if (num_edges > 0 && (hidden_out == nullptr || w0_partials == nullptr))
    return fail(NQA_ERR_INVALID, "nqa_radial_mlp_bwd_train: hidden_out and w0_partials are required");
  return mlp_bwd({"nqa_radial_mlp_bwd", dtype, mode, false, edge_embedding, w0, alpha0, w1, alpha1, num_basis, hidden,
                  out_features, num_edges, workspace, workspace_bytes, workspace_ready, stream},
                 cotangent ? 2 : 1, cotangent, hidden_out, w0_partials, grad_edge_weight, nullptr, grad_edge_embedding);
}

int nqa_radial_mlp_last_fwd(int32_t dtype, int32_t mode, const void* pre, const void* w, double alpha, int32_t hidden,
                            int32_t out_features, int64_t num_edges, void* out, void* workspace, int64_t workspace_bytes,
                            int32_t workspace_ready, nqa_stream stream) {
  return mlp_fwd({"nqa_radial_mlp_last_fwd", dtype, mode, true, pre, nullptr, 1.0, w, alpha, 0, hidden, out_features,
                  num_edges, workspace, workspace_bytes, workspace_ready, stream},
                 nullptr, out);
}

int nqa_radial_mlp_last_bwd(int32_t dtype, int32_t mode, const void* pre, const void* w, double alpha,
                            const void* grad_out, const void* grad_out2, int32_t hidden, int32_t out_features,
                            int64_t num_edges, void* grad_pre, void* workspace, int64_t workspace_bytes,
                            int32_t workspace_ready, nqa_stream stream) {
  return mlp_bwd({"nqa_radial_mlp_last_bwd", dtype, mode, true, pre, nullptr, 1.0, w, alpha, 0, hidden, out_features,
                  num_edges, workspace, workspace_bytes, workspace_ready, stream},
                 0, nullptr, nullptr, nullptr, grad_out, grad_out2, grad_pre);
}

}
```

nequip_amd/csrc/tp_generic.hip:

```cpp
#include <hip/hip_runtime.h>

#include <algorithm>
#include <cstdint>

#include "generated/cg_generated.h"
#include "plan.h"
#include "tp_spec.h"

namespace nqa {

constexpr int kWavesPerBlock = 4;
constexpr int kBlock = 64 * kWavesPerBlock;

template <typename T>
struct TPArgs {
  const T* __restrict__ x;
  const T* __restrict__ y;
  const T* __restrict__ w;
  const T* __restrict__ g;
  T* __restrict__ out;
  T* __restrict__ gw;
  T* __restrict__ ypart;
  const int32_t* __restrict__ rowptr;
  const int32_t* __restrict__ eid;
// ... 339 lines not shown
  }
  return NQA_OK;
}

template <typename T>
static int launch_bwd_x(TPArgs<T> a, void* gx, int64_t N, hipStream_t stream) {
  a.out = static_cast<T*>(gx);
  a.n_items = N * (int64_t)a.n_xchunks;
  if (a.n_items == 0) return NQA_OK;
  unsigned grid;
  int rc = grid_for(a.n_items, &grid);
  if (rc != NQA_OK) return rc;
  hipLaunchKernelGGL(tp_bwd_x_kernel<T>, dim3(grid), dim3(kBlock), 0, stream, a);
  return check_launch("nqa_tp_scatter_bwd_x");
}

static bool force_generic() {
  static const bool v = env_set("NQA_FORCE_GENERIC");
  return v;
}
static bool spec_masked() {
  static const bool v = env_flag("NQA_SPEC_MASKED", false);
  return v;
}

static bool use_spec(const nqa_plan* P, int32_t dtype) {
  return P->spec != nullptr && dtype == NQA_F32 && !force_generic();
}

static int spec_chunks(const nqa_plan* P) { return (P->uniform_mul + 63) / 64; }

static int spec_wpn(const nqa_plan* P, int64_t N) {
  const int64_t items = N * (int64_t)spec_chunks(P);
  const int forced = env_int("NQA_SPEC_WPN", 0);
  if (forced == 1 || forced == 4) return forced;
  return items < 49152 ? 4 : 1;
}

static int spec_launch(const nqa_plan* P, SpecKernel which, const SpecArgs<float>& a, hipStream_t stream, bool ring = false) {
  const bool sums = which == SpecKernel::RowsSumSrc || which == SpecKernel::RowsSumPairs || which == SpecKernel::AccFinish;
  return P->spec->launch(which, SpecLaunchOpts{sums ? 1 : spec_wpn(P, a.N), ring, spec_masked()}, a, stream);
}

__global__ __launch_bounds__(256) void spec_gy_reduce_kernel(const float* __restrict__ part, float* __restrict__ gy,
                                                             int32_t S, int32_t nchunk, int64_t total) {
  const int64_t t = (int64_t)blockIdx.x * blockDim.x + threadIdx.x;
  if (t >= total) return;
  const int64_t e = t / S;
  const int j = (int)(t - e * S);
  float r = 0.f;
  for (int c = 0; c < nchunk; ++c) r += part[e * (int64_t)(nchunk * S) + c * S + j];
  gy[t] = r;
}

static SpecArgs<float> spec_node_operands(const nqa_plan* P, int64_t N) {
  SpecArgs<float> a{};
  a.N = (int32_t)N;
  a.mul = P->uniform_mul;
  a.din = P->dim_in1;
  a.dout = P->dim_out;
  a.wn = P->weight_numel;
  a.gy_stride = P->dim_in2;
  return a;
}

static SpecArgs<float> spec_edge_operands(const nqa_plan* P, int64_t N, const Values& v, const EdgeCsr& c,
                                          const PairedRows* paired) {
  SpecArgs<float> a = spec_node_operands(P, N);
  a.x = static_cast<const float*>(v.x);
  a.y = static_cast<const float*>(v.y);
  a.w = static_cast<const float*>(v.w);
  a.g = static_cast<const float*>(v.g);
  a.rowptr = c.rowptr;
  a.eid = c.eid;
  a.nbr = c.nbr;
  a.wid = paired ? paired->rows : c.eid;
  a.wP = paired ? (int32_t)paired->num_pairs : INT32_MAX;
  return a;
}

static SpecArgs<float> spec_owner_operands(const nqa_plan* P, int64_t N, const Values& v, const OwnerCsr& c) {
  const PairedRows own_rows{c.row, INT32_MAX};
  SpecArgs<float> a = spec_edge_operands(P, N, v, EdgeCsr{c.rowptr, c.edge_in, c.other}, &own_rows);
  a.eid2 = c.edge_out;
  return a;
}

enum class TpWs { Edge, Fused, Pairs };
struct TpWsLayout {
  int64_t total;
  int32_t nchunk;
  int32_t gy_stride;
  int64_t gxe_off;
};

static TpWsLayout tp_ws_layout(const nqa_plan* plan, int32_t dtype, TpWs kind, int64_t num_edges) {
  TpWsLayout l{-1, 1, 0, 0};
  if (plan == nullptr || num_edges < 0) return l;
  const bool spec = use_spec(plan, dtype);
  if (kind != TpWs::Edge && !spec) return l;
  if (kind == TpWs::Pairs && ((num_edges & 1) || !plan->spec->pair)) return l;
  if (spec) {
    l.nchunk = spec_chunks(plan) * (kind == TpWs::Pairs ? plan->spec->pair : 1);
    l.gy_stride = plan->dim_in2 * l.nchunk;
  }
  if (kind == TpWs::Edge) {
    const int64_t per_edge = std::max<int64_t>(plan->ypart_width, spec ? l.gy_stride : 0);
    l.total = num_edges * per_edge * (dtype == NQA_F64 ? 8 : 4);
    return l;
  }
  const int64_t ypart = l.nchunk > 1 ? num_edges * (int64_t)l.gy_stride * 4 : 0;
  const int64_t rows = kind == TpWs::Pairs ? num_edges / 2 : num_edges;
  l.gxe_off = (ypart + 255) & ~(int64_t)255;
  l.total = l.gxe_off + rows * (int64_t)plan->dim_in1 * 4;
  return l;
}

struct TpWsView {
  float* ypart;
  float* gxe;
};
static TpWsView tp_ws_view(void* workspace, const TpWsLayout& l) {
  return {static_cast<float*>(workspace), reinterpret_cast<float*>(static_cast<char*>(workspace) + l.gxe_off)};
}

enum class GyMode {
  Direct,
  Partial,
  Atomic,
};

static void route_gy(SpecArgs<float>& a, const TpWsLayout& l, void* grad_y, void* workspace, GyMode mode) {
  if (mode == GyMode::Partial) {
    a.gy = tp_ws_view(workspace, l).ypart;
    a.gy_stride = l.gy_stride;
  } else {
    a.gy = static_cast<float*>(grad_y);
    a.gy_atomic = mode == GyMode::Atomic;
  }
}

static int finish_gy(const nqa_plan* plan, const TpWsLayout& l, void* grad_y, void* workspace, GyMode mode,
                     int64_t num_edges, const char* label, hipStream_t s) {
  if (mode != GyMode::Partial || num_edges == 0) return NQA_OK;
  const int64_t total = num_edges * (int64_t)plan->dim_in2;
  hipLaunchKernelGGL(spec_gy_reduce_kernel, dim3((unsigned)((total + 255) / 256)), dim3(256), 0, s,
                     tp_ws_view(workspace, l).ypart, static_cast<float*>(grad_y), plan->dim_in2, l.nchunk, total);
  return check_launch(label);
}

struct PairForm {
  bool ring, gx_atomic, gy_atomic;
};
static PairForm pair_form(const nqa_plan* plan, const TpWsLayout& l, int64_t N, int64_t E, bool want_gx) {
  const bool R = env_flag("NQA_PAIR_RING", true), A = env_flag("NQA_PAIR_GX_ATOMIC", true);
  const int ring = plan->spec->ring;
  const bool fits = (plan->uniform_mul & 63) == 0 && E / 2 >= N;
  const bool acc = A && fits && (ring == 2 || (ring == 1 && R));
  const bool many = l.nchunk > 1 && E > 0;
  return {R, acc && want_gx, acc && R && many && (ring == 1 || want_gx)};
}

static int check_common(const nqa_plan* P, const void* image, int32_t dtype, const char* fn) {
  if (P == nullptr || image == nullptr) {
    set_error(std::string(fn) + ": NULL plan or plan image");
    return NQA_ERR_INVALID;
  }
  if (dtype != NQA_F32 && dtype != NQA_F64) {
    set_error(std::string(fn) + ": unsupported dtype");
    return NQA_ERR_UNSUPPORTED;
  }
  return NQA_OK;
}

static int fail(int code, const char* fn, const char* what) {
  set_error(std::string(fn) + what);
  return code;
}
static const char kNullOperand[] = ": NULL operand";
static const char kNoSpec[] = ": no structure-specialised float32 kernel for this plan";
static const char kNoSpecPaired[] = "_paired: no structure-specialised float32 kernel for this plan";
static const char kWorkspace[] = ": workspace missing or too small";

static int check_paired(const char* fn, const int32_t* rows, int64_t num_pairs) {
  if (rows == nullptr || num_pairs <= 0 || num_pairs > 1073741823)
    return fail(NQA_ERR_INVALID, fn, "_paired: weight_rows / num_pairs missing or out of range");
  return NQA_OK;
}

static int tp_fwd(const nqa_plan* plan, const void* image, int32_t dtype, const Values& v, const EdgeCsr& dst, void* out,
                  int64_t N, int64_t E, const PairedRows* paired, hipStream_t s) {
  const char* fn = "nqa_tp_scatter_fwd";
  int rc = check_common(plan, image, dtype, fn);
  if (rc != NQA_OK) return rc;
  if (N < 0 || E < 0 || (N > 0 && (!out || !dst.rowptr)) || (E > 0 && (!v.x || !v.y || !v.w || !dst.eid || !dst.nbr)))
    return fail(NQA_ERR_INVALID, fn, kNullOperand);
  if (use_spec(plan, dtype)) {
    if (N == 0) return NQA_OK;
    SpecArgs<float> a = spec_edge_operands(plan, N, v, dst, paired);
    a.out = static_cast<float*>(out);
    spec_launch(plan, SpecKernel::Fwd, a, s);
    return check_launch("nqa_tp_scatter_fwd(spec)");
  }
  if (paired != nullptr) return fail(NQA_ERR_UNSUPPORTED, fn, kNoSpecPaired);
  return by_dtype(dtype, [&](auto t) { return launch_fwd(generic_args<decltype(t)>(plan, image, v, dst), out, N, s); });
}

static int tp_bwd_edge(const nqa_plan* plan, const void* image, int32_t dtype, const Values& v, const EdgeCsr& dst,
                       void* grad_w, void* grad_y, void* workspace, int64_t workspace_bytes, int64_t N, int64_t E,
                       const PairedRows* paired, hipStream_t s) {
  const char* fn = "nqa_tp_scatter_bwd_edge";
  int rc = check_common(plan, image, dtype, fn);
  if (rc != NQA_OK) return rc;
  if (grad_w == nullptr && grad_y == nullptr) return NQA_OK;
  if (E > 0 && (!v.x || !v.y || !v.w || !v.g || !dst.rowptr || !dst.eid || !dst.nbr))
    return fail(NQA_ERR_INVALID, fn, kNullOperand);
  const TpWsLayout l = tp_ws_layout(plan, dtype, TpWs::Edge, E);
  if (grad_y != nullptr && E > 0 && (workspace == nullptr || workspace_bytes < l.total))
    return fail(NQA_ERR_WORKSPACE, fn, kWorkspace);
  if (use_spec(plan, dtype)) {
    if (N == 0 || E == 0) return NQA_OK;
    SpecArgs<float> a = spec_edge_operands(plan, N, v, dst, paired);
    a.gw = static_cast<float*>(grad_w);
    const GyMode mode = l.nchunk == 1 || grad_y == nullptr ? GyMode::Direct : GyMode::Partial;
    route_gy(a, l, grad_y, workspace, mode);
    spec_launch(plan, SpecKernel::BwdEdge, a, s);
    rc = check_launch("nqa_tp_scatter_bwd_edge(spec)");
    if (rc != NQA_OK) return rc;
    return finish_gy(plan, l, grad_y, workspace, mode, E, "nqa_tp_scatter_bwd_edge(spec reduce)", s);
  }
  if (paired != nullptr) return fail(NQA_ERR_UNSUPPORTED, fn, kNoSpecPaired);
  return by_dtype(dtype, [&](auto t) {
    return launch_bwd_edge(generic_args<decltype(t)>(plan, image, v, dst), plan, image, grad_w, grad_y, workspace, N, E, s);
  });
}

static int tp_bwd_fused(const nqa_plan* plan, const void* image, int32_t dtype, const Values& v, const EdgeCsr& dst,
                        const EdgeCsr& src, void* grad_w, void* grad_y, void* grad_x, void* workspace,
                        int64_t workspace_bytes, int64_t N, int64_t E, const PairedRows* paired, hipStream_t s) {
  const char* fn = "nqa_tp_scatter_bwd_fused";
  int rc = check_common(plan, image, dtype, fn);
  if (rc != NQA_OK) return rc;
  if (!use_spec(plan, dtype)) return fail(NQA_ERR_UNSUPPORTED, fn, kNoSpec);
  if ((N > 0 && (!grad_x || !dst.rowptr || !src.rowptr)) ||
      (E > 0 && (!v.x || !v.y || !v.w || !v.g || !dst.eid || !dst.nbr || !src.eid || !grad_w || !grad_y)))
    return fail(NQA_ERR_INVALID, fn, kNullOperand);
  const TpWsLayout l = tp_ws_layout(plan, dtype, TpWs::Fused, E);
  if (E > 0 && (workspace == nullptr || workspace_bytes < l.total)) return fail(NQA_ERR_WORKSPACE, fn, kWorkspace);
  if (N == 0) return NQA_OK;
  float* gxe = tp_ws_view(workspace, l).gxe;
  if (E > 0) {
    SpecArgs<float> a = spec_edge_operands(plan, N, v, dst, paired);
    a.gw = static_cast<float*>(grad_w);
    a.gxe = gxe;
    const GyMode mode = l.nchunk == 1 ? GyMode::Direct : GyMode::Partial;
    route_gy(a, l, grad_y, workspace, mode);
    spec_launch(plan, SpecKernel::BwdEdge, a, s);
    rc = check_launch("nqa_tp_scatter_bwd_fused(edge)");
    if (rc != NQA_OK) return rc;
    rc = finish_gy(plan, l, grad_y, workspace, mode, E, "nqa_tp_scatter_bwd_fused(reduce)", s);
    if (rc != NQA_OK) return rc;
  }
  SpecArgs<float> b = spec_node_operands(plan, N);
  b.gxe = gxe;
  b.out = static_cast<float*>(grad_x);
  b.rowptr = src.rowptr;
  b.eid = src.eid;
  spec_launch(plan, SpecKernel::RowsSumSrc, b, s);
  return check_launch("nqa_tp_scatter_bwd_fused(sum)");
}

static int tp_bwd_x(const nqa_plan* plan, const void* image, int32_t dtype, const Values& v, const EdgeCsr& src,
                    void* grad_x, int64_t N, int64_t E, const PairedRows* paired, hipStream_t s) {
  const char* fn = "nqa_tp_scatter_bwd_x";
  int rc = check_common(plan, image, dtype, fn);
  if (rc != NQA_OK) return rc;
  if ((N > 0 && (!grad_x || !src.rowptr)) || (E > 0 && (!v.y || !v.w || !v.g || !src.eid || !src.nbr)))
    return fail(NQA_ERR_INVALID, fn, kNullOperand);
  if (use_spec(plan, dtype)) {
    if (N == 0) return NQA_OK;
    SpecArgs<float> a = spec_edge_operands(plan, N, v, src, paired);
    a.out = static_cast<float*>(grad_x);
    spec_launch(plan, SpecKernel::BwdX, a, s);
    return check_launch("nqa_tp_scatter_bwd_x(spec)");
  }
  if (paired != nullptr) return fail(NQA_ERR_UNSUPPORTED, fn, kNoSpecPaired);
  return by_dtype(dtype, [&](auto t) { return launch_bwd_x(generic_args<decltype(t)>(plan, image, v, src), grad_x, N, s); });
}

}

using namespace nqa;

extern "C" {

int64_t nqa_tp_bwd_edge_workspace_bytes(const nqa_plan* plan, int32_t dtype, int64_t num_edges) {
  return tp_ws_layout(plan, dtype, TpWs::Edge, num_edges).total;
}

int64_t nqa_tp_bwd_fused_workspace_bytes(const nqa_plan* plan, int32_t dtype, int64_t num_edges) {
  return tp_ws_layout(plan, dtype, TpWs::Fused, num_edges).total;
}

int64_t nqa_tp_bwd_pairs_workspace_bytes(const nqa_plan* plan, int32_t dtype, int64_t num_edges) {
  return tp_ws_layout(plan, dtype, TpWs::Pairs, num_edges).total;
}

int nqa_tp_scatter_fwd(const nqa_plan* plan, const void* plan_image, int32_t dtype, const void* x, const void* y,
                       const void* w, const int32_t* rowptr_dst, const int32_t* edge_id_dst,
                       const int32_t* src_sorted, void* out, int64_t num_nodes, int64_t num_edges,
                       nqa_stream stream) {
  return tp_fwd(plan, plan_image, dtype, {x, y, w, nullptr}, {rowptr_dst, edge_id_dst, src_sorted}, out, num_nodes,
                num_edges, nullptr, static_cast<hipStream_t>(stream));
}

int nqa_tp_scatter_fwd_paired(const nqa_plan* plan, const void* plan_image, int32_t dtype, const void* x, const void* y,
                              const void* w, const int32_t* rowptr_dst, const int32_t* edge_id_dst,
                              const int32_t* src_sorted, void* out, int64_t num_nodes, int64_t num_edges,
                              const int32_t* weight_rows, int64_t num_pairs, nqa_stream stream) {
  const PairedRows paired{weight_rows, num_pairs};
  int rc = check_paired("nqa_tp_scatter_fwd", weight_rows, num_pairs);
  if (rc != NQA_OK) return rc;
  return tp_fwd(plan, plan_image, dtype, {x, y, w, nullptr}, {rowptr_dst, edge_id_dst, src_sorted}, out, num_nodes,
                num_edges, &paired, static_cast<hipStream_t>(stream));
}

int nqa_tp_scatter_bwd_edge(const nqa_plan* plan, const void* plan_image, int32_t dtype, const void* x,
                            const void* y, const void* w, const void* grad_out, const int32_t* rowptr_dst,
                            const int32_t* edge_id_dst, const int32_t* src_sorted, void* grad_w, void* grad_y,
                            void* workspace, int64_t workspace_bytes, int64_t num_nodes, int64_t num_edges,
                            nqa_stream stream) {
  return tp_bwd_edge(plan, plan_image, dtype, {x, y, w, grad_out}, {rowptr_dst, edge_id_dst, src_sorted}, grad_w, grad_y,
                     workspace, workspace_bytes, num_nodes, num_edges, nullptr, static_cast<hipStream_t>(stream));
}

int nqa_tp_scatter_bwd_edge_paired(const nqa_plan* plan, const void* plan_image, int32_t dtype, const void* x,
                                   const void* y, const void* w, const void* grad_out, const int32_t* rowptr_dst,
                                   const int32_t* edge_id_dst, const int32_t* src_sorted, void* grad_w, void* grad_y,
                                   void* workspace, int64_t workspace_bytes, int64_t num_nodes, int64_t num_edges,
                                   const int32_t* weight_rows, int64_t num_pairs, nqa_stream stream) {
  const PairedRows paired{weight_rows, num_pairs};
  int rc = check_paired("nqa_tp_scatter_bwd_edge", weight_rows, num_pairs);
  if (rc != NQA_OK) return rc;
  return tp_bwd_edge(plan, plan_image, dtype, {x, y, w, grad_out}, {rowptr_dst, edge_id_dst, src_sorted}, grad_w, grad_y,
                     workspace, workspace_bytes, num_nodes, num_edges, &paired, static_cast<hipStream_t>(stream));
}

int nqa_tp_scatter_bwd_fused(const nqa_plan* plan, const void* plan_image, int32_t dtype, const void* x,
                             const void* y, const void* w, const void* grad_out, const int32_t* rowptr_dst,
                             const int32_t* edge_id_dst, const int32_t* src_sorted, const int32_t* rowptr_src,
                             const int32_t* edge_id_src, void* grad_w, void* grad_y, void* grad_x, void* workspace,
                             int64_t workspace_bytes, int64_t num_nodes, int64_t num_edges, nqa_stream stream) {
  return tp_bwd_fused(plan, plan_image, dtype, {x, y, w, grad_out}, {rowptr_dst, edge_id_dst, src_sorted},
                      {rowptr_src, edge_id_src, nullptr}, grad_w, grad_y, grad_x, workspace, workspace_bytes, num_nodes,
                      num_edges, nullptr, static_cast<hipStream_t>(stream));
}

int nqa_tp_scatter_bwd_fused_paired(const nqa_plan* plan, const void* plan_image, int32_t dtype, const void* x,
                                    const void* y, const void* w, const void* grad_out, const int32_t* rowptr_dst,
                                    const int32_t* edge_id_dst, const int32_t* src_sorted, const int32_t* rowptr_src,
                                    const int32_t* edge_id_src, void* grad_w, void* grad_y, void* grad_x, void* workspace,
                                    int64_t workspace_bytes, int64_t num_nodes, int64_t num_edges,
                                    const int32_t* weight_rows, int64_t num_pairs, nqa_stream stream) {
  const PairedRows paired{weight_rows, num_pairs};
  int rc = check_paired("nqa_tp_scatter_bwd_fused", weight_rows, num_pairs);
  if (rc != NQA_OK) return rc;
  return tp_bwd_fused(plan, plan_image, dtype, {x, y, w, grad_out}, {rowptr_dst, edge_id_dst, src_sorted},
                      {rowptr_src, edge_id_src, nullptr}, grad_w, grad_y, grad_x, workspace, workspace_bytes, num_nodes,
                      num_edges, &paired, static_cast<hipStream_t>(stream));
}

int nqa_tp_scatter_bwd_x(const nqa_plan* plan, const void* plan_image, int32_t dtype, const void* y, const void* w,
                         const void* grad_out, const int32_t* rowptr_src, const int32_t* edge_id_src,
                         const int32_t* dst_sorted, void* grad_x, int64_t num_nodes, int64_t num_edges,
                         nqa_stream stream) {
  return tp_bwd_x(plan, plan_image, dtype, {nullptr, y, w, grad_out}, {rowptr_src, edge_id_src, dst_sorted}, grad_x,
                  num_nodes, num_edges, nullptr, static_cast<hipStream_t>(stream));
}

int nqa_tp_scatter_bwd_x_paired(const nqa_plan* plan, const void* plan_image, int32_t dtype, const void* y, const void* w,
                                const void* grad_out, const int32_t* rowptr_src, const int32_t* edge_id_src,
                                const int32_t* dst_sorted, void* grad_x, int64_t num_nodes, int64_t num_edges,
                                const int32_t* weight_rows, int64_t num_pairs, nqa_stream stream) {
  const PairedRows paired{weight_rows, num_pairs};
  int rc = check_paired("nqa_tp_scatter_bwd_x", weight_rows, num_pairs);
  if (rc != NQA_OK) return rc;
  return tp_bwd_x(plan, plan_image, dtype, {nullptr, y, w, grad_out}, {rowptr_src, edge_id_src, dst_sorted}, grad_x,
                  num_nodes, num_edges, &paired, static_cast<hipStream_t>(stream));
}

int nqa_tp_scatter_bwd_pairs(const nqa_plan* plan, const void* plan_image, int32_t dtype, const void* x, const void* y,
                             const void* w, const void* grad_out, const int32_t* owner_rowptr,
                             const int32_t* pair_other, const int32_t* pair_row, const int32_t* pair_edge_in,
                             const int32_t* pair_edge_out, const int32_t* other_rowptr, const int32_t* other_slot,
                             void* grad_w, void* grad_y, void* grad_x, void* workspace, int64_t workspace_bytes,
                             int64_t num_nodes, int64_t num_edges, nqa_stream stream) {
  const char* fn = "nqa_tp_scatter_bwd_pairs";
  int rc = check_common(plan, plan_image, dtype, fn);
  if (rc != NQA_OK) return rc;
  const TpWsLayout l = tp_ws_layout(plan, dtype, TpWs::Pairs, num_edges);
  if (l.total < 0)
    return fail(NQA_ERR_UNSUPPORTED, fn, ": no pair-centric float32 kernel for this plan (or an odd edge count)");
  if ((num_nodes > 0 && (!owner_rowptr || (grad_x && !other_rowptr))) ||
      (num_edges > 0 && (!x || !y || !w || !grad_out || !pair_other || !pair_row || !pair_edge_in || !pair_edge_out ||
                         (grad_x && !other_slot) || !grad_w || !grad_y)))
    return fail(NQA_ERR_INVALID, fn, kNullOperand);
  if (num_edges > 0 && (workspace == nullptr || workspace_bytes < l.total)) return fail(NQA_ERR_WORKSPACE, fn, kWorkspace);
  if (num_nodes == 0) return NQA_OK;
  hipStream_t s = static_cast<hipStream_t>(stream);
  const PairForm form = pair_form(plan, l, num_nodes, num_edges, grad_x != nullptr);
  float* gxe = tp_ws_view(workspace, l).gxe;
  SpecArgs<float> a = spec_owner_operands(plan, num_nodes, {x, y, w, grad_out},
                                          {owner_rowptr, pair_other, pair_row, pair_edge_in, pair_edge_out});
  a.gw = static_cast<float*>(grad_w);
  a.gxe = grad_x ? gxe : nullptr;
  a.out = static_cast<float*>(grad_x);
  a.gx_atomic = form.gx_atomic;
  if (form.gx_atomic && hipMemsetAsync(gxe, 0, (size_t)num_nodes * plan->dim_in1 * 4, s) != hipSuccess)
    return fail(NQA_ERR_LAUNCH, fn, ": hipMemsetAsync of the grad_x accumulator failed");
  const GyMode mode = l.nchunk == 1 ? GyMode::Direct : (form.gy_atomic ? GyMode::Atomic : GyMode::Partial);
  if (mode == GyMode::Atomic && hipMemsetAsync(grad_y, 0, (size_t)num_edges * plan->dim_in2 * 4, s) != hipSuccess)
    return fail(NQA_ERR_LAUNCH, fn, ": hipMemsetAsync of grad_y failed");
  route_gy(a, l, grad_y, workspace, mode);
  if (spec_launch(plan, SpecKernel::BwdPairs, a, s, form.ring) != 0) return fail(NQA_ERR_UNSUPPORTED, fn, ": kernel not available");
  rc = check_launch("nqa_tp_scatter_bwd_pairs(pairs)");
  if (rc != NQA_OK) return rc;
  rc = finish_gy(plan, l, grad_y, workspace, mode, num_edges, "nqa_tp_scatter_bwd_pairs(reduce)", s);
  if (rc != NQA_OK) return rc;
  if (grad_x == nullptr) return NQA_OK;
  SpecArgs<float> b = spec_node_operands(plan, num_nodes);
  b.gxe = gxe;
  b.out = static_cast<float*>(grad_x);
  if (form.gx_atomic) {
    if (spec_launch(plan, SpecKernel::AccFinish, b, s) != 0)
      return fail(NQA_ERR_UNSUPPORTED, fn, ": this structure has no accumulator kernel");
    return check_launch("nqa_tp_scatter_bwd_pairs(accumulator)");
  }
  b.rowptr = other_rowptr;
  b.eid = other_slot;
  if (spec_launch(plan, SpecKernel::RowsSumPairs, b, s) != 0)
    return fail(NQA_ERR_UNSUPPORTED, fn, ": this structure has no grad_x row-sum kernel");
  return check_launch("nqa_tp_scatter_bwd_pairs(sum)");
}

int32_t nqa_tp_bwd_pairs_dual_supported(const nqa_plan* plan, int32_t dtype) {
  return (plan != nullptr && use_spec(plan, dtype) && plan->spec->pair == 1) ? 1 : 0;
}

int nqa_tp_scatter_bwd_pairs_dual(const nqa_plan* plan, const void* plan_image, int32_t dtype, const void* x,
                                  const void* x_cot, const void* y, const void* y_cot, const void* w, const void* w_cot,
                                  const void* grad_out, const int32_t* owner_rowptr, const int32_t* pair_other,
                                  const int32_t* pair_row, const int32_t* pair_edge_in, const int32_t* pair_edge_out,
                                  void* grad_w, void* grad_y, void* workspace, int64_t workspace_bytes,
                                  int64_t num_nodes, int64_t num_edges, nqa_stream stream) {
  const char* fn = "nqa_tp_scatter_bwd_pairs_dual";
  int rc = check_common(plan, plan_image, dtype, fn);
  if (rc != NQA_OK) return rc;
  if (!nqa_tp_bwd_pairs_dual_supported(plan, dtype) || (num_edges & 1))
    return fail(NQA_ERR_UNSUPPORTED, fn, ": no dual pair-centric kernel for this plan (or an odd edge count)");
  const TpWsLayout l = tp_ws_layout(plan, dtype, TpWs::Pairs, num_edges);
  if ((num_nodes > 0 && !owner_rowptr) ||
      (num_edges > 0 && (!x || !x_cot || !y || !y_cot || !w || !grad_out || !pair_other || !pair_row || !pair_edge_in ||
                         !pair_edge_out || !grad_w || !grad_y)))
    return fail(NQA_ERR_INVALID, fn, kNullOperand);
  if (num_edges > 0 && (workspace == nullptr || workspace_bytes < l.total)) return fail(NQA_ERR_WORKSPACE, fn, kWorkspace);
  if (num_nodes == 0 || num_edges == 0) return NQA_OK;
  hipStream_t s = static_cast<hipStream_t>(stream);
  SpecArgs<float> a = spec_owner_operands(plan, num_nodes, {x, y, w, grad_out},
                                          {owner_rowptr, pair_other, pair_row, pair_edge_in, pair_edge_out});
  a.x2 = static_cast<const float*>(x_cot);
  a.y2 = static_cast<const float*>(y_cot);
  a.w2 = static_cast<const float*>(w_cot);
  a.gw = static_cast<float*>(grad_w);
  const GyMode mode = l.nchunk == 1 ? GyMode::Direct : GyMode::Partial;
  route_gy(a, l, grad_y, workspace, mode);
  if (spec_launch(plan, SpecKernel::BwdPairsDual, a, s) != 0) return fail(NQA_ERR_UNSUPPORTED, fn, ": kernel not available");
  rc = check_launch("nqa_tp_scatter_bwd_pairs_dual");
  if (rc != NQA_OK) return rc;
  return finish_gy(plan, l, grad_y, workspace, mode, num_edges, "nqa_tp_scatter_bwd_pairs_dual(reduce)", s);
}

int32_t nqa_tp_fwd_jvp_supported(const nqa_plan* plan, int32_t dtype) {
  return (plan != nullptr && use_spec(plan, dtype)) ? 1 : 0;
}

static bool bad_optional_rows(const int32_t* weight_rows, int64_t num_pairs) {
  return weight_rows != nullptr && (num_pairs <= 0 || num_pairs > 1073741823);
}

int nqa_tp_scatter_fwd_jvp(const nqa_plan* plan, const void* plan_image, int32_t dtype, const void* x, const void* y,
                           const void* w, const void* x_cot, const void* y_cot, const void* w_cot,
                           const int32_t* rowptr_dst, const int32_t* edge_id_dst, const int32_t* src_sorted, void* out,
                           int64_t num_nodes, int64_t num_edges, const int32_t* weight_rows, int64_t num_pairs,
                           nqa_stream stream) {
  const char* fn = "nqa_tp_scatter_fwd_jvp";
  int rc = check_common(plan, plan_image, dtype, fn);
  if (rc != NQA_OK) return rc;
  if (!use_spec(plan, dtype)) return fail(NQA_ERR_UNSUPPORTED, fn, kNoSpec);
  if (num_nodes < 0 || num_edges < 0 || (num_nodes > 0 && (!out || !rowptr_dst)) ||
      (num_edges > 0 && (!x || !y || !w || !edge_id_dst || !src_sorted || (!x_cot && !y_cot && !w_cot))) ||
      bad_optional_rows(weight_rows, num_pairs))
    return fail(NQA_ERR_INVALID, fn, ": NULL operand (at least one cotangent is required)");
  if (num_nodes == 0) return NQA_OK;
  hipStream_t s = static_cast<hipStream_t>(stream);
  if (num_edges == 0) {
    if (hipMemsetAsync(out, 0, (size_t)num_nodes * plan->dim_out * 4, s) != hipSuccess)
      return fail(NQA_ERR_LAUNCH, fn, ": hipMemsetAsync failed");
    return NQA_OK;
  }
  const PairedRows paired{weight_rows, num_pairs};
  SpecArgs<float> a = spec_edge_operands(plan, num_nodes, {x, y, w, nullptr}, {rowptr_dst, edge_id_dst, src_sorted},
                                         weight_rows ? &paired : nullptr);
  a.x2 = static_cast<const float*>(x_cot);
  a.y2 = static_cast<const float*>(y_cot);
  a.w2 = static_cast<const float*>(w_cot);
  a.out = static_cast<float*>(out);
  if (spec_launch(plan, SpecKernel::FwdJvp, a, s) != 0)
    return fail(NQA_ERR_UNSUPPORTED, fn, ": this structure has no forward-JVP kernel");
  return check_launch("nqa_tp_scatter_fwd_jvp");
}

int nqa_tp_scatter_bwd_x_dual(const nqa_plan* plan, const void* plan_image, int32_t dtype, const void* y, const void* w,
                              const void* y_cot, const void* w_cot, const void* grad_out, const int32_t* rowptr_src,
                              const int32_t* edge_id_src, const int32_t* dst_sorted, void* grad_x, int64_t num_nodes,
                              int64_t num_edges, const int32_t* weight_rows, int64_t num_pairs, nqa_stream stream) {
  const char* fn = "nqa_tp_scatter_bwd_x_dual";
  int rc = check_common(plan, plan_image, dtype, fn);
  if (rc != NQA_OK) return rc;
  if (!use_spec(plan, dtype)) return fail(NQA_ERR_UNSUPPORTED, fn, kNoSpec);
  if ((num_nodes > 0 && (!grad_x || !rowptr_src)) ||
      (num_edges > 0 && (!y || !w || !y_cot || !w_cot || !grad_out || !edge_id_src || !dst_sorted)) ||
      bad_optional_rows(weight_rows, num_pairs))
    return fail(NQA_ERR_INVALID, fn, kNullOperand);
  if (num_nodes == 0) return NQA_OK;
  hipStream_t s = static_cast<hipStream_t>(stream);
  if (num_edges == 0) {
    if (hipMemsetAsync(grad_x, 0, (size_t)num_nodes * plan->dim_in1 * 4, s) != hipSuccess)
      return fail(NQA_ERR_LAUNCH, fn, ": hipMemsetAsync failed");
    return NQA_OK;
  }
  const PairedRows paired{weight_rows, num_pairs};
  SpecArgs<float> a = spec_edge_operands(plan, num_nodes, {nullptr, y, w, grad_out}, {rowptr_src, edge_id_src, dst_sorted},
                                         weight_rows ? &paired : nullptr);
  a.y2 = static_cast<const float*>(y_cot);
  a.w2 = static_cast<const float*>(w_cot);
  a.out = static_cast<float*>(grad_x);
  if (spec_launch(plan, SpecKernel::BwdXDual, a, s) != 0) return fail(NQA_ERR_UNSUPPORTED, fn, ": kernel not available");
  return check_launch("nqa_tp_scatter_bwd_x_dual");
}

}
```

nequip_amd/nn/_paired_radial.py:

```python

from __future__ import annotations

import os

import torch

from .. import _lib
from . import mlp as _mlp
from ._tp_scatter_base import _Kernels
from ._topology import EdgePairing, EdgeTopology


_side_streams = {}


def side_stream(device: torch.device, slot: int = 0) -> torch.cuda.Stream:
    key = (device.type, device.index, slot)
    st = _side_streams.get(key)
    if st is None:
        st = _side_streams[key] = torch.cuda.Stream(device=device)
    return st


class RadialBackwardQueue:

    def __init__(self, device: torch.device):
        self.stream = side_stream(device, 0)
        self.layers = 0
        self.acc = None
        self.pending = None

    @staticmethod
    def lagged() -> bool:
        return os.environ.get("NQA_RADIAL_LAG", "1") not in ("", "0")

    def flush(self) -> None:
        item, self.pending = self.pending, None
        if item is not None:
            item()

    def submit(self, launch, ready: "torch.cuda.Event", reads, last: bool) -> None:
        def item():
            self.stream.wait_event(ready)
            with torch.cuda.stream(self.stream):
                part = launch()
                self.acc = part if self.acc is None else self.acc.add_(part)
            for t in reads:
                t.record_stream(self.stream)

        self.flush()
        if last or not self.lagged():
            item()
        else:
            self.pending = item

    @staticmethod
    def enabled() -> bool:
        return os.environ.get("NQA_NO_OVERLAP", "") in ("", "0")


def _pair_backward_pays(g: torch.Tensor) -> bool:
    if os.environ.get("NQA_NO_PAIR_BWD", "") not in ("", "0"):
        return False
    limit_mb = os.environ.get("NQA_PAIR_BWD_MAX_MB", "")
    return limit_mb == "" or g.numel() * g.element_size() <= float(limit_mb) * (1 << 20)


class _PairedRadialTPFn(torch.autograd.Function):
    @staticmethod
    def forward(ctx, emb_half, x, y, w0, w1, alpha0: float, alpha1: float, mode: int, cache, k: _Kernels,
                topo: EdgeTopology, pairing: EdgePairing, queue=None):
        emb_half, x, y = emb_half.contiguous(), x.contiguous(), y.contiguous()
        w_half = _mlp._launch_fwd(emb_half, w0, w1, alpha0, alpha1, mode, cache)
        out = k.fwd(x, y, w_half, topo, pairing)
        ctx.save_for_backward(emb_half, x, y, w_half, w0, w1)
        ctx.args = (alpha0, alpha1, mode, cache, k, topo, pairing)
        ctx.queue = queue
        if queue is not None:
            queue.layers += 1
        return out

    @staticmethod
    @torch.autograd.function.once_differentiable
    def backward(ctx, g):
        emb_half, x, y, w_half, w0, w1 = ctx.saved_tensors
        alpha0, alpha1, mode, cache, k, topo, pairing = ctx.args
        need_emb, need_x, need_y = ctx.needs_input_grad[:3]
        if ctx.queue is not None:
            ctx.queue.flush()
        g = g.contiguous()
        P = pairing.num_pairs
        gx = gy = G = None
        fused = None
        folded = False
        if need_emb and need_x and need_y and k.prefer_fused_bwd and os.environ.get("NQA_NO_FUSED_BWD", "") in ("", "0"):
            if _pair_backward_pays(g):
                fused = k.bwd_pairs(x, y, w_half, g, topo, pairing)
                folded = fused is not None
            if fused is None and k.fused_rows_ok:
                fused = k.bwd_fused(x, y, w_half, g, topo, pairing=pairing)
        if fused is not None:
            gx, G, gy = fused
        else:
            if need_x:
                gx = k.bwd_x(y, w_half, g, topo, pairing)
            pairs = k.bwd_pairs(x, y, w_half, g, topo, pairing, need_gx=False) if (need_emb and need_y and _pair_backward_pays(g)) else None
            if pairs is not None:
                _, G, gy = pairs
                folded = True
            else:
                G, gy = k.bwd_edge(x, y, w_half, g, topo, need_gw=need_emb, need_gy=need_y, pairing=pairing)
        g_emb = None
        q = ctx.queue
        if q is not None:
            q.layers -= 1
        if need_emb and q is not None:
            cur = torch.cuda.current_stream(g.device)
            try:
                ready = torch.cuda.Event()
                ready.record(cur)
                last = q.layers <= 0

                def launch():
                    if folded:
                        return _mlp._launch_bwd(emb_half, w0, w1, alpha0, alpha1, G, mode, cache, device_idle=last)
                    return _mlp._launch_bwd_paired(emb_half, w0, w1, alpha0, alpha1, G[:P], G[P:], mode, cache)

                q.submit(launch, ready, (G, emb_half, w0, w1), last)
            except BaseException:
                cur.wait_stream(q.stream)
                q.acc, q.layers, q.pending = None, 0, None
                raise
            if q.layers <= 0:
                assert q.acc is not None and q.layers == 0, "radial backward queue out of step with the layers"
                cur.wait_stream(q.stream)
                g_emb, q.acc = q.acc, None
                g_emb.record_stream(cur)
        elif need_emb and folded:
            g_emb = _mlp._launch_bwd(emb_half, w0, w1, alpha0, alpha1, G, mode, cache)
        elif need_emb:
            g_emb = _mlp._launch_bwd_paired(emb_half, w0, w1, alpha0, alpha1, G[:P], G[P:], mode, cache)
        return (g_emb, gx, gy) + (None,) * 10


class _PairRowsFn(torch.autograd.Function):

    @staticmethod
    def forward(ctx, emb, pairing: EdgePairing):
        from ._topology import _ptr, current_stream_ptr

        emb = emb.contiguous()
        assert emb.dim() == 2 and emb.element_size() == 4
        out = torch.empty((pairing.num_pairs, emb.shape[1]), dtype=emb.dtype, device=emb.device)
        with torch.cuda.device(emb.device):
            rc = _lib.load().nqa_pair_gather(_ptr(emb), _ptr(pairing.rep_edge), pairing.num_pairs, emb.shape[1],
                                             _ptr(out), current_stream_ptr(emb.device))
        _lib.check(rc, "nqa_pair_gather")
        ctx.pairing, ctx.num_edges = pairing, emb.shape[0]
        return out

    @staticmethod
    def backward(ctx, g):
        return _PairExpandFn.apply(g, ctx.pairing, ctx.num_edges), None


class _PairExpandFn(torch.autograd.Function):
    @staticmethod
    def forward(ctx, g, pairing: EdgePairing, num_edges: int):
        from ._topology import _ptr, current_stream_ptr

        g = g.contiguous()
        out = torch.empty((num_edges, g.shape[1]), dtype=g.dtype, device=g.device)
        with torch.cuda.device(g.device):
            rc = _lib.load().nqa_pair_expand(_ptr(g), _ptr(pairing.rows), num_edges, pairing.num_pairs, g.shape[1],
                                             _ptr(out), current_stream_ptr(g.device))
        _lib.check(rc, "nqa_pair_expand")
        ctx.pairing = pairing
        return out

    @staticmethod
    def backward(ctx, c):
        return _PairRowsFn.apply(c, ctx.pairing), None, None


def pair_rows(emb: torch.Tensor, pairing: EdgePairing) -> torch.Tensor:
    return _PairRowsFn.apply(emb, pairing)


def available(edge_mlp, tp_scatter, x: torch.Tensor, emb: torch.Tensor) -> bool:
    if not x.is_cuda or x.dtype != torch.float32 or emb.dtype != torch.float32:
        return False
    from ..utils.tracing import traceable

    if traceable():
        return False
    if os.environ.get("NQA_NO_PAIRED", "") not in ("", "0"):
        return False
    if not edge_mlp._fused_ok(emb) or _mlp.radial_mlp_mode() != _lib.NQA_MLP_BF16X6:
        return False
    if tp_scatter.use_dispatcher_ops or tp_scatter.model_dtype != torch.float32:
        return False
    return tp_scatter._get_kernels().has_spec(torch.float32)


def paired_radial_tp(edge_mlp, tp_scatter, emb, x, edge_attr, topo: EdgeTopology, pairing: EdgePairing,
                     emb_half=None, queue=None):
    cache = getattr(edge_mlp, "_weight_images", None)
    if cache is None:
        cache = edge_mlp._weight_images = _mlp._WeightImages()
    cache.validate(edge_mlp.mlp[2].weight)
    if emb_half is None:
        emb_half = pair_rows(emb, pairing)
    from ..utils.wgrad import differentiable_parameters

    if differentiable_parameters(edge_mlp.training, edge_mlp.mlp[0].weight, edge_mlp.mlp[2].weight):
        w_half = edge_mlp(emb_half)
        return tp_scatter(x, edge_attr, w_half, topo._dst, topo._src, topology=topo, pairing=pairing)
    return _PairedRadialTPFn.apply(
        emb_half, x, edge_attr, edge_mlp.mlp[0].weight.detach(), edge_mlp.mlp[2].weight.detach(),
        edge_mlp._alphas[0], edge_mlp._alphas[1], _mlp.radial_mlp_mode(), cache, tp_scatter._get_kernels(), topo, pairing,
        queue,
    )
```

nequip_amd/nn/_tp_scatter_base.py:

```python

from __future__ import annotations

import os
from typing import Optional, Tuple

import torch

from .. import _lib
from ..utils import ktimer
from ..o3.irreps import Irreps
from ..o3.tensor_product import NativePlan, TensorProduct
from ._topology import EdgeTopology, _ptr, current_stream_ptr, topology_cache


def _nqa_dtype(dtype: torch.dtype) -> int:
    if dtype == torch.float32:
        return _lib.NQA_F32
    if dtype == torch.float64:
        return _lib.NQA_F64
    raise RuntimeError(f"nequip_amd kernels support float32/float64 model dtypes, got {dtype}")


def _switched_off(name: str) -> bool:
    return os.environ.get(name, "") not in ("", "0")


class _Kernels:

    def __init__(self, plan: NativePlan, image: torch.Tensor):
        self.plan = plan
        self.image = image
        self.dim_in1 = plan.query(_lib.NQA_PLAN_DIM_IN1)
        self.dim_in2 = plan.query(_lib.NQA_PLAN_DIM_IN2)
        self.dim_out = plan.query(_lib.NQA_PLAN_DIM_OUT)
        self.weight_numel = plan.query(_lib.NQA_PLAN_WEIGHT_NUMEL)
        self.out_needs_zero = bool(plan.query(_lib.NQA_PLAN_OUT_NEEDS_ZERO))
        self.prefer_fused_bwd = (self.weight_numel + self.dim_out) >= 3 * self.dim_in1
        self.fused_rows_ok = bool(plan.query(_lib.NQA_PLAN_FUSED_ROWS_OK))
        self._support = {}

    def _supports(self, kind: str, dtype: torch.dtype) -> bool:
        if (kind, dtype) not in self._support:
            lib, h, dt = _lib.load(), self.plan.handle, _nqa_dtype(dtype)
            self._support[kind, dtype] = {
                "spec": lambda: lib.nqa_tp_bwd_fused_workspace_bytes(h, dt, 0) >= 0,
                "pairs": lambda: lib.nqa_tp_bwd_pairs_workspace_bytes(h, dt, 0) >= 0,
                "jvp": lambda: bool(lib.nqa_tp_fwd_jvp_supported(h, dt)),
                "dual": lambda: bool(lib.nqa_tp_bwd_pairs_dual_supported(h, dt)),
            }[kind]()
        return self._support[kind, dtype]

    def has_spec(self, dtype: torch.dtype) -> bool:
        return self._supports("spec", dtype)

    def has_pairs_kernel(self, dtype: torch.dtype) -> bool:
        return self._supports("pairs", dtype)

    def has_fwd_jvp(self, dtype: torch.dtype) -> bool:
        return self._supports("jvp", dtype)

    def has_dual_pairs_kernel(self, dtype: torch.dtype) -> bool:
        return self._supports("dual", dtype)

    def _call(self, name: str, pairing, slots: Optional[str], ref: torch.Tensor, *args) -> None:
        fn = f"nqa_tp_scatter_{name}"
        argv = [self.plan.handle, _ptr(self.image), _nqa_dtype(ref.dtype)]
        argv += [a if isinstance(a, int) else _ptr(a) for a in args]
        if pairing is not None:
            argv += [_ptr(getattr(pairing, slots)), pairing.num_pairs]
        rc = getattr(_lib.load(), fn + ("_paired" if pairing is not None else ""))(*argv, current_stream_ptr(ref.device))
        _lib.check(rc, fn)

    def _check(self, x, y, w, topo: EdgeTopology, pairing=None):
        N, E = topo.num_nodes, topo.num_edges
        if x is not None:
            assert x.shape == (N, self.dim_in1), f"x has shape {tuple(x.shape)}, expected {(N, self.dim_in1)}"
        if y is not None:
            assert y.shape == (E, self.dim_in2), f"edge_attr has shape {tuple(y.shape)}, expected {(E, self.dim_in2)}"
        if w is not None:
            rows = E if pairing is None else pairing.num_pairs
            assert w.shape == (rows, self.weight_numel), (
                f"edge_weight has shape {tuple(w.shape)}, expected {(rows, self.weight_numel)}"
            )

    def fwd(self, x, y, w, topo: EdgeTopology, pairing=None) -> torch.Tensor:
        self._check(x, y, w, topo, pairing)
        alloc = torch.zeros if self.out_needs_zero else torch.empty
        out = alloc((topo.num_nodes, self.dim_out), dtype=x.dtype, device=x.device)
        csr = topo.by_dst
        es = x.element_size()
        nbytes = topo.num_edges * (es * (self.weight_numel + self.dim_in2) + 16) + topo.num_nodes * es * (
            self.dim_in1 + self.dim_out
        )
        with torch.cuda.device(x.device), ktimer.region("tp_fwd", nbytes, 0.0, topo.num_edges * es * self.weight_numel,
                                                        self.weight_numel):
            self._call("fwd", pairing, "slots_dst", x, x, y, w, *csr, out,
                       topo.num_nodes, topo.num_edges)
        return out

    def bwd_edge(self, x, y, w, g, topo: EdgeTopology, need_gw: bool, need_gy: bool, pairing=None, gw_out=None):
        self._check(x, y, w, topo, pairing)
        lib = _lib.load()
        E = topo.num_edges
        gw_rows = E if pairing is None else 2 * pairing.num_pairs
        gw = None
        if need_gw:
            if gw_out is not None:
                assert gw_out.shape == (gw_rows, self.weight_numel) and gw_out.is_contiguous() and gw_out.dtype == x.dtype
                gw = gw_out
            else:
                gw = torch.empty((gw_rows, self.weight_numel), dtype=x.dtype, device=x.device)
        gy = torch.empty((E, self.dim_in2), dtype=x.dtype, device=x.device) if need_gy else None
        if not (need_gw or need_gy):
            return None, None
        ws, ws_bytes = None, 0
        if need_gy:
            ws_bytes = lib.nqa_tp_bwd_edge_workspace_bytes(self.plan.handle, _nqa_dtype(x.dtype), E)
            ws = torch.empty(max(ws_bytes, 1), dtype=torch.uint8, device=x.device)
        csr = topo.by_dst
        es = x.element_size()
        nbytes = E * (es * (self.weight_numel + self.dim_in2) + 16) + topo.num_nodes * es * (
            self.dim_in1 + self.dim_out
        )
        nbytes += E * es * ((self.weight_numel if need_gw else 0) + (self.dim_in2 if need_gy else 0))
        with torch.cuda.device(x.device), ktimer.region("tp_bwd_edge", nbytes, 0.0,
                                                        E * es * self.weight_numel * (2 if need_gw else 1), self.weight_numel):
            self._call("bwd_edge", pairing, "slots_dst", x, x, y, w, g, *csr, gw, gy, ws,
                       ws_bytes, topo.num_nodes, E)
        return gw, gy

    def bwd_fused(self, x, y, w, g, topo: EdgeTopology, need_gw: bool = True, need_gy: bool = True, pairing=None):
        lib = _lib.load()
        E, N = topo.num_edges, topo.num_nodes
        ws_bytes = lib.nqa_tp_bwd_fused_workspace_bytes(self.plan.handle, _nqa_dtype(x.dtype), E)
        if ws_bytes < 0:
            return None
        self._check(x, y, w, topo, pairing)
        gx = torch.empty((N, self.dim_in1), dtype=x.dtype, device=x.device)
        gw_rows = E if pairing is None else 2 * pairing.num_pairs
        gw = torch.empty((gw_rows, self.weight_numel), dtype=x.dtype, device=x.device) if need_gw else None
        gy = torch.empty((E, self.dim_in2), dtype=x.dtype, device=x.device) if need_gy else None
        ws = torch.empty(max(ws_bytes, 1), dtype=torch.uint8, device=x.device)
        csr = topo.by_dst
        rowptr_s, eid_s, _ = topo.by_src
        es = x.element_size()
        nbytes = E * (es * (self.weight_numel + self.dim_in2) + 16) + N * es * (2 * self.dim_in1 + self.dim_out)
        nbytes += E * es * ((self.weight_numel if need_gw else 0) + (self.dim_in2 if need_gy else 0))
        with torch.cuda.device(x.device), ktimer.region("tp_bwd_fused", nbytes, 0.0,
                                                        E * es * self.weight_numel * (2 if need_gw else 1), self.weight_numel):
            self._call("bwd_fused", pairing, "slots_dst", x, x, y, w, g, *csr, rowptr_s, eid_s,
                       gw, gy, gx, ws, ws_bytes, N, E)
        return gx, gw, gy

    def bwd_pairs(self, x, y, w, g, topo: EdgeTopology, pairing, need_gx: bool = True):
        lib = _lib.load()
        E, N = topo.num_edges, topo.num_nodes
        ws_bytes = lib.nqa_tp_bwd_pairs_workspace_bytes(self.plan.handle, _nqa_dtype(x.dtype), E)
        if ws_bytes < 0:
            return None
        self._check(x, y, w, topo, pairing)
        P = pairing.num_pairs
        gx = torch.empty((N, self.dim_in1), dtype=x.dtype, device=x.device) if need_gx else None
        gw = torch.empty((P, self.weight_numel), dtype=x.dtype, device=x.device)
        gy = torch.empty((E, self.dim_in2), dtype=x.dtype, device=x.device)
        ws = torch.empty(max(ws_bytes, 1), dtype=torch.uint8, device=x.device)
        owner = pairing.owner_csr
        es = x.element_size()
        nbytes = E * (es * (2 * self.weight_numel + 2 * self.dim_in2) + 16) + N * es * (
            (2 if need_gx else 1) * self.dim_in1 + self.dim_out)
        with torch.cuda.device(x.device), ktimer.region("tp_bwd_fused" if need_gx else "tp_bwd_edge", nbytes, 0.0,
                                                        E * es * 2 * self.weight_numel, self.weight_numel):
            self._call("bwd_pairs", None, None, x, x, y, w, g, *owner, gw, gy, gx, ws, ws_bytes, N, E)
        return gx, gw, gy

    def fwd_jvp(self, x, y, w, c_x, c_y, c_w, topo: EdgeTopology, pairing=None) -> torch.Tensor:
        self._check(x, y, w, topo, pairing)
        out = torch.empty((topo.num_nodes, self.dim_out), dtype=x.dtype, device=x.device)
        csr = topo.by_dst
        es = x.element_size()
        nterms = sum(t is not None for t in (c_x, c_y, c_w))
        nbytes = topo.num_edges * (es * (self.weight_numel * (2 if c_w is not None else 1) + 2 * self.dim_in2) + 16) + \
            topo.num_nodes * es * (2 * self.dim_in1 + self.dim_out)
        with torch.cuda.device(x.device), ktimer.region("tp_fwd", nbytes):
            self._call("fwd_jvp", None, None, x, x, y, w, c_x, c_y, c_w, *csr, out, topo.num_nodes, topo.num_edges,
                       *((pairing.slots_dst, pairing.num_pairs) if pairing is not None else (None, 0)))
        assert nterms > 0
        return out

    def bwd_x_dual(self, y, w, c_y, c_w, g, topo: EdgeTopology, pairing=None) -> torch.Tensor:
        self._check(None, y, w, topo, pairing)
        gx = torch.empty((topo.num_nodes, self.dim_in1), dtype=g.dtype, device=g.device)
        csr = topo.by_src
        es = g.element_size()
        nbytes = topo.num_edges * (es * 2 * (self.weight_numel + self.dim_in2) + 16) + topo.num_nodes * es * (
            self.dim_in1 + self.dim_out)
        with torch.cuda.device(g.device), ktimer.region("tp_bwd_x", nbytes):
            self._call("bwd_x_dual", None, None, g, y, w, c_y, c_w, g, *csr, gx, topo.num_nodes, topo.num_edges,
                       *((pairing.slots_src, pairing.num_pairs) if pairing is not None else (None, 0)))
        return gx

    def edge_grads_dual(self, x, x_cot, y, y_cot, w, g, topo: EdgeTopology, pairing, w_cot=None):
        lib = _lib.load()
        E, N = topo.num_edges, topo.num_nodes
        self._check(x, y, w, topo, pairing)
        ws_bytes = lib.nqa_tp_bwd_pairs_workspace_bytes(self.plan.handle, _nqa_dtype(x.dtype), E)
        gw = torch.empty((pairing.num_pairs, self.weight_numel), dtype=x.dtype, device=x.device)
        gy = torch.empty((E, self.dim_in2), dtype=x.dtype, device=x.device)
        ws = torch.empty(max(ws_bytes, 1), dtype=torch.uint8, device=x.device)
        owner = pairing.owner_csr[:5]
        es = x.element_size()
        nbytes = E * (es * (2 * self.weight_numel + 3 * self.dim_in2) + 16) + N * es * (2 * self.dim_in1 + self.dim_out)
        with torch.cuda.device(x.device), ktimer.region("tp_bwd_edge", nbytes):
            self._call("bwd_pairs_dual", None, None, x, x, x_cot, y, y_cot, w, w_cot, g, *owner, gw, gy,
                       ws, ws_bytes, N, E)
        return gw, gy

    def use_pairs(self, dtype: torch.dtype, pairing) -> bool:
        return pairing is not None and not _switched_off("NQA_NO_PAIR_BWD") and self.has_pairs_kernel(dtype)

    def edge_grads_folded(self, x, y, w, g, topo: EdgeTopology, pairing, need_gw: bool, need_gy: bool):
        if need_gw and self.use_pairs(x.dtype, pairing):
            res = self.bwd_pairs(x, y, w, g, topo, pairing, need_gx=False)
            if res is not None:
                _, gw, gy = res
                return gw, (gy if need_gy else None)
        gw, gy = self.bwd_edge(x, y, w, g, topo, need_gw=need_gw, need_gy=need_gy, pairing=pairing)
        return _fold(gw, pairing), gy

    def bwd_x(self, y, w, g, topo: EdgeTopology, pairing=None) -> torch.Tensor:
        self._check(None, y, w, topo, pairing)
        gx = torch.empty((topo.num_nodes, self.dim_in1), dtype=g.dtype, device=g.device)
        csr = topo.by_src
        es = g.element_size()
        nbytes = topo.num_edges * (es * (self.weight_numel + self.dim_in2) + 16) + topo.num_nodes * es * (
            self.dim_in1 + self.dim_out
        )
        with torch.cuda.device(g.device), ktimer.region("tp_bwd_x", nbytes, 0.0, topo.num_edges * es * self.weight_numel,
                                                        self.weight_numel):
            self._call("bwd_x", pairing, "slots_src", g, y, w, g, *csr, gx,
                       topo.num_nodes, topo.num_edges)
        return gx


def _fold(G, pairing):
    if G is None or pairing is None:
        return G
    P = pairing.num_pairs
    return G[:P] + G[P:]


class _TPScatterFn(torch.autograd.Function):

    @staticmethod
    def forward(ctx, x, y, w, k: _Kernels, topo: EdgeTopology, pairing=None):
        x, y, w = x.contiguous(), y.contiguous(), w.contiguous()
        out = k.fwd(x, y, w, topo, pairing)
        ctx.save_for_backward(x, y, w)
        ctx.k, ctx.topo, ctx.pairing = k, topo, pairing
        return out

    @staticmethod
    def backward(ctx, g):
        x, y, w = ctx.saved_tensors
        need = tuple(ctx.needs_input_grad[:3])
        gx, gy, gw = _TPScatterBwdFn.apply(g, x, y, w, ctx.k, ctx.topo, need, ctx.pairing)
        return gx, gy, gw, None, None, None


class _TPScatterBwdFn(torch.autograd.Function):

    @staticmethod
    def forward(ctx, g, x, y, w, k: _Kernels, topo: EdgeTopology, need: Tuple[bool, bool, bool], pairing=None):
        g = g.contiguous()
        fused = None
        folded = False
        if need[0] and need[1] and need[2] and k.prefer_fused_bwd and not _switched_off("NQA_NO_FUSED_BWD"):
            if k.use_pairs(x.dtype, pairing):
                fused = k.bwd_pairs(x, y, w, g, topo, pairing)
                folded = fused is not None
            if fused is None and k.fused_rows_ok:
                fused = k.bwd_fused(x, y, w, g, topo, need_gw=need[2], need_gy=need[1], pairing=pairing)
        if fused is not None:
            gx, gw, gy = fused
            if not folded:
                gw = _fold(gw, pairing)
        else:
            gx = k.bwd_x(y, w, g, topo, pairing) if need[0] else None
            gw, gy = k.edge_grads_folded(x, y, w, g, topo, pairing, need_gw=need[2], need_gy=need[1])
        ctx.save_for_backward(g, x, y, w)
        ctx.k, ctx.topo, ctx.pairing = k, topo, pairing
        ctx.mark_non_differentiable(*[t for t, n in zip((gx, gy, gw), need) if not n and t is not None])
        return gx, gy, gw

    @staticmethod
    @torch.autograd.function.once_differentiable
    def backward(ctx, c_x, c_y, c_w):
        g, x, y, w = ctx.saved_tensors
        k, topo, pr = ctx.k, ctx.topo, ctx.pairing
        need_g, need_x, need_y, need_w = ctx.needs_input_grad[:4]
        c_x = c_x.contiguous() if c_x is not None else None
        c_y = c_y.contiguous() if c_y is not None else None
        c_w = c_w.contiguous() if c_w is not None else None

        def add(a, b):
            return b if a is None else (a if b is None else a + b)

        gg = gxx = gyy = gww = None
        if need_g and sum(t is not None for t in (c_x, c_y, c_w)) > 1 and k.has_fwd_jvp(x.dtype) and \
                not _switched_off("NQA_NO_FWD_JVP"):
            gg = k.fwd_jvp(x, y, w, c_x, c_y, c_w, topo, pr)
        elif need_g:
            if c_x is not None:
                gg = add(gg, k.fwd(c_x, y, w, topo, pr))
            if c_y is not None:
                gg = add(gg, k.fwd(x, c_y, w, topo, pr))
            if c_w is not None:
                gg = add(gg, k.fwd(x, y, c_w, topo, pr))
        if need_x and c_y is not None and c_w is not None and k.has_fwd_jvp(x.dtype) and \
                not _switched_off("NQA_NO_FWD_JVP"):
            gxx = k.bwd_x_dual(y, w, c_y, c_w, g, topo, pr)
        elif need_x:
            if c_y is not None:
                gxx = add(gxx, k.bwd_x(c_y, w, g, topo, pr))
            if c_w is not None:
                gxx = add(gxx, k.bwd_x(y, c_w, g, topo, pr))
# ... 93 lines not shown
```

nequip_amd/nn/embedding/_edge.py:

```python

from __future__ import annotations

import ctypes
import os
from typing import Dict, List, Optional, Union

import torch

from ... import _lib
from ...utils import ktimer
from ...data import AtomicDataDict
from ...o3.irreps import Irreps
from .._graph_mixin import GraphModuleMixin
from .._topology import _ptr, current_stream_ptr
from ..utils import with_edge_vectors_
from ...utils.tracing import traceable


def _embed(edge_vec, bessel_weights, cfg):
    if traceable():
        from ._edge_ops import edge_embed

        return edge_embed(edge_vec, bessel_weights, cfg)
    return _EdgeEmbedFn.apply(edge_vec, bessel_weights, cfg)
# ... 39 lines not shown
    _check_cotangent(fn, "g_sh", g_sh, (E, (max(cfg["lmax"], 0) + 1) ** 2), cfg["dtype"], vec.device)
    _check_cotangent(fn, "g_emb", g_emb, (E, cfg["nb"]), cfg["dtype"], vec.device)


class _EdgeEmbedFn(torch.autograd.Function):

    @staticmethod
    def forward(ctx, edge_vec, bessel_weights, cfg):
        _check_operands("edge_embed_fwd", edge_vec, bessel_weights, cfg)
        if not edge_vec.is_cuda:
            raise RuntimeError(_GPU_ONLY)
        assert edge_vec.dtype == torch.float64, "edge vectors must be float64 (nequip _GLOBAL_DTYPE)"
        lib = _lib.load()
        vec = edge_vec.contiguous()
        E = vec.shape[0]
        out_dtype = cfg["dtype"]
        lmax = cfg["lmax"]
        sh = torch.empty((E, (lmax + 1) ** 2), dtype=out_dtype, device=vec.device) if cfg["want_sh"] else None
        emb = torch.empty((E, cfg["nb"]), dtype=out_dtype, device=vec.device) if cfg["want_emb"] else None
        nbytes = E * (24 + out_dtype.itemsize * (((lmax + 1) ** 2 if cfg["want_sh"] else 0) + (cfg["nb"] if cfg["want_emb"] else 0)))
        with torch.cuda.device(vec.device), ktimer.region("edge_embed_fwd", nbytes):
            rc = lib.nqa_edge_embed_fwd(
                _dt(out_dtype), max(lmax, 0), _ptr(vec), E, cfg["rmax_recip"], _ptr(cfg.get("rmax_edge")), cfg["nb"],
                _ptr(bessel_weights), cfg["p"], cfg["factor"], _ptr(sh), _ptr(emb), ctypes.c_void_p(),
                current_stream_ptr(vec.device),
            )
        _lib.check(rc, "nqa_edge_embed_fwd")
        ctx.save_for_backward(vec, bessel_weights)
        ctx.cfg = cfg
        outs = tuple(t for t in (sh, emb) if t is not None)
        return outs if len(outs) > 1 else outs[0]

    @staticmethod
    def backward(ctx, *grads):
        vec, bw = ctx.saved_tensors
        cfg = ctx.cfg
        grads = list(grads)
        g_sh = grads.pop(0) if cfg["want_sh"] else None
        g_emb = grads.pop(0) if cfg["want_emb"] else None
        return _EdgeEmbedBwdFn.apply(vec, bw, g_sh, g_emb, cfg), None, None


class _EdgeEmbedBwdFn(torch.autograd.Function):

    @staticmethod
    def forward(ctx, vec, bw, g_sh, g_emb, cfg):
        _check_operands("edge_embed_bwd", vec, bw, cfg)
        _check_first_order_cotangents("edge_embed_bwd", vec, g_sh, g_emb, cfg)
        if not vec.is_cuda:
            raise RuntimeError(_GPU_ONLY)
        lib = _lib.load()
        g_sh = g_sh.contiguous() if g_sh is not None else None
        g_emb = g_emb.contiguous() if g_emb is not None else None
        E = vec.shape[0]
        g_vec = torch.empty((E, 3), dtype=torch.float64, device=vec.device)
        nbytes = E * (48 + cfg["dtype"].itemsize * (((cfg["lmax"] + 1) ** 2 if g_sh is not None else 0) + (cfg["nb"] if g_emb is not None else 0)))
        with torch.cuda.device(vec.device), ktimer.region("edge_embed_bwd", nbytes):
            rc = lib.nqa_edge_embed_bwd(
                _dt(cfg["dtype"]), max(cfg["lmax"], 0), _ptr(vec), E, cfg["rmax_recip"], _ptr(cfg.get("rmax_edge")),
                cfg["nb"], _ptr(bw), cfg["p"], cfg["factor"], _ptr(g_sh), _ptr(g_emb), _ptr(g_vec),
                current_stream_ptr(vec.device),
            )
        _lib.check(rc, "nqa_edge_embed_bwd")
        ctx.save_for_backward(vec, bw, g_sh, g_emb)
        ctx.cfg = cfg
        return g_vec

    @staticmethod
    @torch.autograd.function.once_differentiable
    def backward(ctx, c):
        vec, bw, g_sh, g_emb = ctx.saved_tensors
        need_vec, _, need_gsh, need_gemb = ctx.needs_input_grad[:4]
        g_vec2, gg_sh, gg_emb = _edge_embed_second_order(vec, bw, g_sh, g_emb, c, ctx.cfg, need_vec, need_gsh, need_gemb)
        return g_vec2, None, gg_sh, gg_emb, None


def _edge_embed_second_order(vec, bw, g_sh, g_emb, c, cfg, need_vec: bool, need_gsh: bool, need_gemb: bool):
    _check_operands("edge_embed_bwd_bwd", vec, bw, cfg)
    _check_first_order_cotangents("edge_embed_bwd_bwd", vec, g_sh, g_emb, cfg)
    _check_cotangent("edge_embed_bwd_bwd", "c", c, (vec.shape[0], 3), torch.float64, vec.device)
    if not vec.is_cuda:
        raise RuntimeError(_GPU_ONLY)
    lib = _lib.load()
    c = c.contiguous()
    g_sh = g_sh.contiguous() if g_sh is not None else None
    g_emb = g_emb.contiguous() if g_emb is not None else None
    E = vec.shape[0]
    g_vec2 = torch.empty((E, 3), dtype=torch.float64, device=vec.device) if need_vec else None
    gg_sh = torch.empty_like(g_sh) if (g_sh is not None and need_gsh) else None
    gg_emb = torch.empty_like(g_emb) if (g_emb is not None and need_gemb) else None
    with torch.cuda.device(vec.device):
        rc = lib.nqa_edge_embed_bwd_bwd(
            _dt(cfg["dtype"]), max(cfg["lmax"], 0), _ptr(vec), E, cfg["rmax_recip"], _ptr(cfg.get("rmax_edge")),
            cfg["nb"], _ptr(bw), cfg["p"], cfg["factor"], _ptr(g_sh), _ptr(g_emb), _ptr(c), _ptr(gg_sh),
            _ptr(gg_emb), _ptr(g_vec2), current_stream_ptr(vec.device),
        )
    _lib.check(rc, "nqa_edge_embed_bwd_bwd")
    return g_vec2, gg_sh, gg_emb


def cutoff_partialdict_to_tensor(partial_dict: Dict, type_names: List[str], r_max: float) -> torch.Tensor:
    rows = []
    for centre in type_names:
        entry = partial_dict.get(centre, None)
        if entry is None:
            rows.append([float(r_max)] * len(type_names))
        elif isinstance(entry, (int, float)):
            rows.append([float(entry)] * len(type_names))
        else:
            rows.append([float(entry.get(other, r_max)) for other in type_names])
    table = torch.as_tensor(rows, dtype=_GLOBAL_DTYPE).contiguous()
    assert torch.all(table > 0), "per-edge-type cutoffs must be positive"
    return table


def cutoff_tensor_to_str(cutoff_tensor: torch.Tensor) -> str:
    return " ".join(str(float(v)) for v in cutoff_tensor.detach().to(_GLOBAL_DTYPE).reshape(-1).tolist())


def cutoff_str_to_fulldict(cutoff_str: Optional[str], type_names: List[str]) -> Optional[Dict[str, Dict[str, float]]]:
    if cutoff_str is None or cutoff_str == "":
        return None
    values = [float(x) for x in cutoff_str.split()]
    T = len(type_names)
    if len(values) != T * T:
        raise ValueError(f"expected {T * T} cutoff values for {T} types, got {len(values)}")
    return {a: {b: values[i * T + j] for j, b in enumerate(type_names)} for i, a in enumerate(type_names)}


class _EdgeEmbedPairedFn(torch.autograd.Function):

    @staticmethod
    def forward(ctx, edge_vec, bessel_weights, cfg, pairing):
        _check_operands("edge_embed_fwd_paired", edge_vec, bessel_weights, cfg)
        if not edge_vec.is_cuda:
            raise RuntimeError(_GPU_ONLY)
        assert edge_vec.dtype == torch.float64, "edge vectors must be float64 (nequip _GLOBAL_DTYPE)"
        lib = _lib.load()
        vec = edge_vec.contiguous()
        E, P = vec.shape[0], pairing.num_pairs
        out_dtype, lmax, nb = cfg["dtype"], cfg["lmax"], cfg["nb"]
        sh = torch.empty((E, (lmax + 1) ** 2), dtype=out_dtype, device=vec.device)
        emb = torch.empty((E, nb), dtype=out_dtype, device=vec.device)
        emb_pairs = torch.empty((P, nb), dtype=out_dtype, device=vec.device)
        nbytes = E * (24 + out_dtype.itemsize * ((lmax + 1) ** 2 + nb)) + P * nb * out_dtype.itemsize
        with torch.cuda.device(vec.device), ktimer.region("edge_embed_fwd", nbytes):
            rc = lib.nqa_edge_embed_fwd_paired(
                _dt(out_dtype), lmax, _ptr(vec), E, cfg["rmax_recip"], nb, _ptr(bessel_weights), cfg["p"], cfg["factor"],
                _ptr(pairing.rows), P, _ptr(sh), _ptr(emb), _ptr(emb_pairs), current_stream_ptr(vec.device),
            )
        _lib.check(rc, "nqa_edge_embed_fwd_paired")
        ctx.save_for_backward(vec, bessel_weights)
        ctx.cfg, ctx.pairing = cfg, pairing
        return sh, emb, emb_pairs

    @staticmethod
    @torch.autograd.function.once_differentiable
    def backward(ctx, g_sh, g_emb, g_pairs):
        vec, bw = ctx.saved_tensors
        cfg, pairing = ctx.cfg, ctx.pairing
        _check_first_order_cotangents("edge_embed_bwd_paired", vec, g_sh, g_emb, cfg)
        _check_cotangent("edge_embed_bwd_paired", "g_pairs", g_pairs, (pairing.num_pairs, cfg["nb"]), cfg["dtype"], vec.device)
        lib = _lib.load()
        g_sh = g_sh.contiguous() if g_sh is not None else None
        g_emb = g_emb.contiguous() if g_emb is not None else None
        g_pairs = g_pairs.contiguous() if g_pairs is not None else None
        E = vec.shape[0]
        g_vec = torch.empty((E, 3), dtype=torch.float64, device=vec.device)
        nbytes = E * (48 + cfg["dtype"].itemsize * ((cfg["lmax"] + 1) ** 2)) + pairing.num_pairs * cfg["nb"] * cfg["dtype"].itemsize
        with torch.cuda.device(vec.device), ktimer.region("edge_embed_bwd", nbytes):
            rc = lib.nqa_edge_embed_bwd_paired(
                _dt(cfg["dtype"]), cfg["lmax"], _ptr(vec), E, cfg["rmax_recip"], cfg["nb"], _ptr(bw), cfg["p"],
                cfg["factor"], _ptr(pairing.rows), pairing.num_pairs, _ptr(g_sh), _ptr(g_emb), _ptr(g_pairs), _ptr(g_vec),
                current_stream_ptr(vec.device),
            )
        _lib.check(rc, "nqa_edge_embed_bwd_paired")
        return g_vec, None, None, None


class EdgeLengthNormalizer(GraphModuleMixin, torch.nn.Module):

    def __init__(self, r_max: float, type_names: List[str], per_edge_type_cutoff: Optional[Dict] = None,
                 edge_type_field: str = AtomicDataDict.EDGE_TYPE_KEY,
                 norm_length_field: str = AtomicDataDict.NORM_LENGTH_KEY, irreps_in=None):
        super().__init__()
        self.r_max = float(r_max)
        self.num_types = len(type_names)
        self.edge_type_field = edge_type_field
        self.norm_length_field = norm_length_field
        self._per_edge_type = per_edge_type_cutoff is not None
        if self._per_edge_type:
            table = cutoff_partialdict_to_tensor(per_edge_type_cutoff, list(type_names), self.r_max)
            assert float(table.max()) <= self.r_max + 1e-12, "per-edge-type cutoffs cannot exceed r_max"
            rmax_recip = table.reciprocal().view(-1)
            self.symmetric = bool(torch.equal(table, table.t()))
        else:
            rmax_recip = torch.as_tensor(1.0 / self.r_max, dtype=_GLOBAL_DTYPE)
            self.symmetric = True
        self.register_buffer("_rmax_recip", rmax_recip)
        irreps_out = {self.norm_length_field: Irreps("1x0e")}
        if self._per_edge_type:
            irreps_out[self.edge_type_field] = None
        self._init_irreps(irreps_in=irreps_in, irreps_out=irreps_out)

    def forward(self, data: AtomicDataDict.Type) -> AtomicDataDict.Type:
        data = with_edge_vectors_(data, with_lengths=False)
        data["_nqa_rmax_recip"] = 1.0 / self.r_max
        if self._per_edge_type:
            if self.edge_type_field not in data:
                data[self.edge_type_field] = torch.index_select(
                    data[AtomicDataDict.ATOM_TYPE_KEY].reshape(-1), 0,
                    data[AtomicDataDict.EDGE_INDEX_KEY].reshape(-1)).view(2, -1)
            et = data[self.edge_type_field]
            data["_nqa_rmax_recip_edge"] = torch.index_select(self._rmax_recip, 0, et[0] * self.num_types + et[1])
        return data


class BesselEdgeLengthEncoding(GraphModuleMixin, torch.nn.Module):

    def __init__(self, cutoff: torch.nn.Module, num_bessels: int = 8, trainable: bool = False,
                 edge_invariant_field: str = AtomicDataDict.EDGE_EMBEDDING_KEY,
                 norm_length_field: str = AtomicDataDict.NORM_LENGTH_KEY, irreps_in=None):
        super().__init__()
        self.cutoff = cutoff
        self.num_bessels = num_bessels
        self.trainable = trainable
        self.edge_invariant_field = edge_invariant_field
        self.norm_length_field = norm_length_field
        bessel_weights = torch.linspace(1.0, num_bessels, num_bessels, dtype=_GLOBAL_DTYPE).unsqueeze(0)
        if trainable:
            self.bessel_weights = torch.nn.Parameter(bessel_weights)
        else:
            self.register_buffer("bessel_weights", bessel_weights)
        self.factor = 1.0
        self._init_irreps(
            irreps_in=irreps_in,
            irreps_out={self.edge_invariant_field: Irreps([(num_bessels, (0, 1))])},
        )
        self._output_dtype = torch.get_default_dtype()

    def _forward_differentiable_weights(self, data, vec, rmax_edge):
        r = torch.linalg.norm(vec, dim=-1, keepdim=True)
        x = r * (rmax_edge.view(-1, 1) if rmax_edge is not None else float(data["_nqa_rmax_recip"]))
        bessel = (torch.sinc(x * self.bessel_weights) * self.bessel_weights).to(self._output_dtype)
        p = float(self.cutoff.p)
        cut = 1.0 - ((p + 1.0) * (p + 2.0) / 2.0) * torch.pow(x, p) + p * (p + 2.0) * torch.pow(x, p + 1.0) \
            - (p * (p + 1.0) / 2) * torch.pow(x, p + 2.0)
        cut = (cut * (x < 1.0)).to(self._output_dtype)
        emb = bessel * cut
        return emb * self.factor if self.factor != 1.0 else emb

    def forward(self, data: AtomicDataDict.Type) -> AtomicDataDict.Type:
        data = with_edge_vectors_(data, with_lengths=False)
        vec = data[AtomicDataDict.EDGE_VECTORS_KEY]
        rmax_edge = data.get("_nqa_rmax_recip_edge")
        pre = data.pop("_nqa_fused_edge_embedding", None)
        if pre is not None and pre[1] is self and rmax_edge is None:
            data[self.edge_invariant_field] = pre[0]
            return data
        if self.trainable and self.bessel_weights.requires_grad and torch.is_grad_enabled() and self.training:
            data[self.edge_invariant_field] = self._forward_differentiable_weights(data, vec, rmax_edge)
            return data
        if rmax_edge is not None and traceable():
            raise NotImplementedError("per-edge-type cutoffs are not part of the dispatcher-op (compile) form of the edge "
                                      "embedding: evaluate this model eagerly")
        cfg = dict(dtype=self._output_dtype, lmax=0, want_sh=False, want_emb=True, nb=self.num_bessels,
                   rmax_recip=float(data["_nqa_rmax_recip"]), p=float(self.cutoff.p), factor=float(self.factor))
        if rmax_edge is not None:
            cfg["rmax_edge"] = rmax_edge.contiguous()
        data[self.edge_invariant_field] = _embed(vec, self.bessel_weights.detach().view(-1), cfg)
        return data


class SphericalHarmonicEdgeAttrs(GraphModuleMixin, torch.nn.Module):

    def __init__(self, irreps_edge_sh: Union[int, str, Irreps], edge_sh_normalization: str = "component",
                 edge_sh_normalize: bool = True, irreps_in=None, out_field: str = AtomicDataDict.EDGE_ATTRS_KEY):
        super().__init__()
        self.out_field = out_field
        if isinstance(irreps_edge_sh, int):
            self.irreps_edge_sh = Irreps.spherical_harmonics(irreps_edge_sh)
        else:
            self.irreps_edge_sh = Irreps(str(irreps_edge_sh))
        lmax = self.irreps_edge_sh.lmax
        if self.irreps_edge_sh != Irreps.spherical_harmonics(lmax):
            raise NotImplementedError("edge spherical harmonics must be the full range 0..lmax with parity (-1)^l")
        if edge_sh_normalization != "component" or not edge_sh_normalize:
            raise NotImplementedError("only the nequip defaults (normalize=True, 'component') are implemented")
        self.lmax = lmax
        self._init_irreps(irreps_in=irreps_in, irreps_out={out_field: self.irreps_edge_sh})
        self._output_dtype = torch.get_default_dtype()
        self.register_buffer("_dummy_bw", torch.ones(1, dtype=_GLOBAL_DTYPE), persistent=False)

    @staticmethod
    def _known_pairing(data, vec):
        K = AtomicDataDict
        if (vec.dtype != torch.float64 or K.POSITIONS_KEY not in data
                or os.environ.get("NQA_NO_PAIRED_EMBED", "") not in ("", "0")
                or os.environ.get("NQA_NO_PAIRED", "") not in ("", "0")):
            return None
        ei = data.get(K.EDGE_INDEX_KEY)
        if ei is None or not ei.is_cuda:
            return None
        from .._topology import topology_cache

        topo = topology_cache.get(ei[0], ei[1], data[K.POSITIONS_KEY].shape[0])
# ... 28 lines not shown
```

nequip_amd/nn/mlp.py:

```python

import os
from math import sqrt
from typing import Optional

import torch

from .. import _lib
from ..data import AtomicDataDict
from ..o3.irreps import Irreps
from ..utils import ktimer
from ..utils.wgrad import _WeightCacheMixin, differentiable_parameters
from ._graph_mixin import GraphModuleMixin


def radial_mlp_mode() -> int:
    return _lib.NQA_MLP_FP32 if os.environ.get("NQA_MLP_EXACT_FP32", "") not in ("", "0") else _lib.NQA_MLP_BF16X6


def forward_mode(mode: int) -> int:
    if mode == _lib.NQA_MLP_BF16X6 and os.environ.get("NQA_MLP_FWD_F16", "") not in ("0",):
        return _lib.NQA_MLP_F16X3
    return mode


def backward_mode(mode: int) -> int:
    if mode == _lib.NQA_MLP_BF16X6 and os.environ.get("NQA_MLP_BWD_F16", "") not in ("0",):
        return _lib.NQA_MLP_F16X3
    return mode


from ..utils.tracing import traceable

class _WeightImages:

    def __init__(self):
        self.key = None
        self.images = {}

    def validate(self, param: torch.Tensor) -> None:
        key = (id(param), param.data_ptr(), param._version, param.device)
        if key != self.key:
            self.key, self.images = key, {}

    def get(self, w1: torch.Tensor, mode: int, backward: int, nbytes: int, rows: int = 1):
        if rows == 0:
            return torch.empty(max(nbytes, 1), dtype=torch.uint8, device=w1.device), False
        hit = (mode, backward) in self.images
        if not hit:
            self.images[(mode, backward)] = torch.empty(max(nbytes, 1), dtype=torch.uint8, device=w1.device)
        return self.images[(mode, backward)], hit


_P = _lib.ptr


def _launch(name: str, *, region: str, nbytes: float, flops: float, resolve, mode: int, backward: int, w1,
            cache: _WeightImages, rows: int, device, alloc, call):
    lib = _lib.load()
    H, W = w1.shape
    if resolve is not None:
        mode = resolve(mode)
    ws_bytes = lib.nqa_radial_mlp_workspace_bytes(mode, backward, H, W)
    ws, ready = cache.get(w1, mode, backward, ws_bytes, rows)
    outs = alloc()
    with torch.cuda.device(device), ktimer.region(region, nbytes, flops):
        rc = call(getattr(lib, name), mode, outs, _P(ws), ws_bytes, int(ready), _lib.stream_ptr(device))
    _lib.check(rc, name)
    return outs


def _launch_fwd(emb, w0, w1, alpha0: float, alpha1: float, mode: int, cache: _WeightImages):
    E, nb = emb.shape
    H, W = w1.shape
    out = torch.empty((E, W), dtype=emb.dtype, device=emb.device)
    _launch("nqa_radial_mlp_fwd", region="radial_mlp_fwd", nbytes=4.0 * E * (nb + W), flops=2.0 * E * (nb * H + H * W),
            resolve=forward_mode, mode=mode, backward=0, w1=w1, cache=cache, rows=E, device=emb.device, alloc=lambda: (out,),
            call=lambda fn, m, outs, *ws: fn(_lib.NQA_F32, m, _P(emb), _P(w0), alpha0, _P(w1), alpha1, nb, H, W, E, _P(out),
                                             *ws))
    return out


def _launch_bwd(emb, w0, w1, alpha0: float, alpha1: float, g_w, mode: int, cache: _WeightImages, device_idle: bool = False):
    E, nb = emb.shape
    H, W = w1.shape
    g_emb = torch.empty_like(emb)
    hint = _lib.NQA_MLP_HINT_DEVICE_IS_IDLE if device_idle else 0
    _launch("nqa_radial_mlp_bwd", region="radial_mlp_bwd", nbytes=4.0 * E * (2 * nb + W),
            flops=2.0 * E * (nb * H * 2 + H * W), resolve=backward_mode, mode=mode, backward=1, w1=w1, cache=cache, rows=E,
            device=emb.device, alloc=lambda: (g_emb,),
            call=lambda fn, m, outs, *ws: fn(_lib.NQA_F32, m | hint, _P(emb), _P(w0), alpha0, _P(w1), alpha1, _P(g_w), nb, H,
                                             W, E, _P(g_emb), *ws))
    return g_emb


def _launch_bwd_train(emb, w0, w1, alpha0: float, alpha1: float, g_w, cot, mode: int, cache: _WeightImages):
    E, nb = emb.shape
    H, W = w1.shape
    g_emb = torch.empty_like(emb)
    hid = torch.empty((E, H), dtype=emb.dtype, device=emb.device)
    tiles = _lib.load().nqa_radial_mlp_train_tiles(E)
    parts = torch.empty((tiles, nb, H), dtype=emb.dtype, device=emb.device)
    _launch("nqa_radial_mlp_bwd_train", region="radial_mlp_bwd_train", nbytes=4.0 * E * (3 * nb + W + H),
            flops=2.0 * E * (nb * H * (3 if cot is None else 5) + H * W), resolve=backward_mode, mode=mode, backward=1, w1=w1,
            cache=cache, rows=E, device=emb.device, alloc=lambda: (g_emb, hid, parts),
            call=lambda fn, m, outs, *ws: fn(_lib.NQA_F32, m, _P(emb), _P(cot), _P(w0), alpha0, _P(w1), alpha1, _P(g_w), nb, H,
                                             W, E, _P(g_emb), _P(hid), _P(parts), *ws))
    return g_emb, hid, parts.sum(0)


def _launch_fwd_tangent(emb, cot, w0, w1, alpha0: float, alpha1: float, mode: int, cache: _WeightImages):
    E, nb = emb.shape
    H, W = w1.shape
    out = torch.empty((E, W), dtype=emb.dtype, device=emb.device)
    _launch("nqa_radial_mlp_fwd_tangent", region="radial_mlp_fwd", nbytes=4.0 * E * (2 * nb + W),
            flops=2.0 * E * (2 * nb * H + H * W), resolve=None, mode=mode, backward=0, w1=w1, cache=cache, rows=E,
            device=emb.device, alloc=lambda: (out,),
            call=lambda fn, m, outs, *ws: fn(_lib.NQA_F32, m, _P(emb), _P(cot), _P(w0), alpha0, _P(w1), alpha1, nb, H, W, E,
                                             _P(out), *ws))
    return out


def _launch_bwd_paired(emb, w0, w1, alpha0: float, alpha1: float, g_a, g_b, mode: int, cache: _WeightImages):
    E, nb = emb.shape
    H, W = w1.shape
    assert g_a.shape == (E, W) and g_b.shape == (E, W) and g_a.is_contiguous() and g_b.is_contiguous()
    g_emb = torch.empty_like(emb)
    _launch("nqa_radial_mlp_bwd_paired", region="radial_mlp_bwd", nbytes=4.0 * E * (2 * nb + 2 * W),
            flops=2.0 * E * (nb * H * 2 + H * W), resolve=backward_mode, mode=mode, backward=1, w1=w1, cache=cache, rows=E,
            device=emb.device, alloc=lambda: (g_emb,),
            call=lambda fn, m, outs, *ws: fn(_lib.NQA_F32, m, _P(emb), _P(w0), alpha0, _P(w1), alpha1, _P(g_a), _P(g_b), nb,
                                             H, W, E, _P(g_emb), *ws))
    return g_emb


def _launch_wgrad(a, b):
    from ..utils import wgrad as _wg

    M, N = a.shape[1], b.shape[1]
    return _wg.wgrad(a, b, _wg.WgradTable([(0, 0, M, N, 1, 0)], M * N)).view(M, N)


class _RadialMLPFn(torch.autograd.Function):

    @staticmethod
    def forward(ctx, emb, w0, w1, alpha0: float, alpha1: float, mode: int, cache: _WeightImages):
        emb = emb.contiguous()
        out = _launch_fwd(emb, w0, w1, alpha0, alpha1, mode, cache)
        ctx.save_for_backward(emb, w0, w1)
        ctx.alphas = (alpha0, alpha1)
        ctx.mode, ctx.cache = mode, cache
        return out

    @staticmethod
    @torch.autograd.function.once_differentiable
    def backward(ctx, g_w):
        emb, w0, w1 = ctx.saved_tensors
        g_emb = _launch_bwd(emb, w0, w1, ctx.alphas[0], ctx.alphas[1], g_w.contiguous(), ctx.mode, ctx.cache)
        return g_emb, None, None, None, None, None, None


def _launch_last(pre, w, alpha: float, cache: _WeightImages, g=None):
    E, H = pre.shape
    W = w.shape[1]
    common = dict(flops=2.0 * E * H * W, resolve=None, mode=_lib.NQA_MLP_F16X3, w1=w, cache=cache, rows=E, device=pre.device)
    if g is None:
        return _launch("nqa_radial_mlp_last_fwd", region="radial_mlp_fwd", nbytes=4.0 * E * (H + W), backward=0, **common,
                       alloc=lambda: (torch.empty((E, W), dtype=pre.dtype, device=pre.device),),
                       call=lambda fn, m, outs, *ws: fn(_lib.NQA_F32, m, _P(pre), _P(w), alpha, H, W, E, _P(outs[0]), *ws))[0]
    return _launch("nqa_radial_mlp_last_bwd", region="radial_mlp_bwd", nbytes=4.0 * E * (2 * H + W), backward=1, **common,
                   alloc=lambda: (torch.empty_like(pre),),
                   call=lambda fn, m, outs, *ws: fn(_lib.NQA_F32, m, _P(pre), _P(w), alpha, _P(g), None, H, W, E,
                                                    _P(outs[0]), *ws))[0]


class _RadialMLPLastFn(torch.autograd.Function):

    @staticmethod
    def forward(ctx, pre, w, alpha: float, cache: _WeightImages):
        pre = pre.contiguous()
        out = _launch_last(pre, w, alpha, cache)
        ctx.save_for_backward(pre, w)
        ctx.alpha, ctx.cache = alpha, cache
        return out

    @staticmethod
    @torch.autograd.function.once_differentiable
    def backward(ctx, g):
        pre, w = ctx.saved_tensors
        return _launch_last(pre, w, ctx.alpha, ctx.cache, g=g.contiguous()), None, None, None


def _silu_derivs(p):
    sig = torch.sigmoid(p)
    one_m = 1.0 - sig
    return sig * (1.0 + p * one_m), sig * one_m * (2.0 + p * (1.0 - 2.0 * sig))


class _RadialMLPTrainFn(torch.autograd.Function):

    @staticmethod
    def forward(ctx, emb, w0, w1, alpha0: float, alpha1: float, mode: int, cache: _WeightImages):
        emb = emb.contiguous()
        out = _launch_fwd(emb, w0.detach(), w1.detach(), alpha0, alpha1, mode, cache)
        ctx.save_for_backward(emb, w0, w1)
        ctx.args = (alpha0, alpha1, mode, cache)
        return out

    @staticmethod
    def backward(ctx, g):
        emb, w0, w1 = ctx.saved_tensors
        g_emb, g_w0, g_w1 = _RadialMLPTrainBwdFn.apply(emb, w0, w1, g, *ctx.args)
        return g_emb, g_w0, g_w1, None, None, None, None


class _RadialMLPTrainBwdFn(torch.autograd.Function):

    @staticmethod
    def forward(ctx, emb, w0, w1, g, alpha0: float, alpha1: float, mode: int, cache: _WeightImages):
        from ..utils import wgrad as _wg

        g = g.contiguous()
        w0d, w1d = w0.detach(), w1.detach()
        g_w0 = g_w1 = None
        want_params = _wg.param_grads_wanted() and (w0.requires_grad or w1.requires_grad)
        if not want_params:
            g_emb = _launch_bwd(emb, w0d, w1d, alpha0, alpha1, g, mode, cache)
        elif mode == _lib.NQA_MLP_BF16X6:
            g_emb, h, p0 = _launch_bwd_train(emb, w0d, w1d, alpha0, alpha1, g, None, mode, cache)
            g_w0 = p0 * alpha0
            if w1.is_leaf and w1.requires_grad and _wg.deferring():
                _wg.defer(w1, lambda: _launch_wgrad(h, g) * alpha1, h, g)
            else:
                g_w1 = _launch_wgrad(h, g) * alpha1
        else:
            g_emb = _launch_bwd(emb, w0d, w1d, alpha0, alpha1, g, mode, cache)
            P = emb @ (w0d * alpha0)
            s1, _ = _silu_derivs(P)
            g_w1 = _launch_wgrad(P * torch.sigmoid(P), g) * alpha1
            g_w0 = _launch_wgrad(emb, (g @ (w1d * alpha1).t()) * s1) * alpha0
        ctx.save_for_backward(emb, w0, w1, g)
        ctx.args = (alpha0, alpha1, mode, cache)
        ctx.mark_non_differentiable(*[t for t in (g_w0, g_w1) if t is not None])
        return g_emb, g_w0, g_w1

    @staticmethod
    @torch.autograd.function.once_differentiable
    def backward(ctx, c, c_w0, c_w1):
        emb, w0, w1, g = ctx.saved_tensors
        alpha0, alpha1, mode, cache = ctx.args
        w0d, w1d = w0.detach(), w1.detach()
        c = c.contiguous()
        need_emb, need_w0, need_w1, need_g = ctx.needs_input_grad[:4]
        d_emb = d_w0 = d_w1 = d_g = None
        if mode == _lib.NQA_MLP_BF16X6:
            if need_emb or need_w0 or need_w1:
                d_emb, R, p0 = _launch_bwd_train(emb, w0d, w1d, alpha0, alpha1, g, c, mode, cache)
                d_w0 = p0 * alpha0 if need_w0 else None
                if need_w1:
                    from ..utils import wgrad as _wg

                    if w1.is_leaf and w1.requires_grad and _wg.deferring():
                        _wg.defer(w1, lambda: _launch_wgrad(R, g) * alpha1, R, g)
                    else:
                        d_w1 = _launch_wgrad(R, g) * alpha1
            if need_g:
                d_g = _launch_fwd_tangent(emb, c, w0d, w1d, alpha0, alpha1, mode, cache)
            return d_emb, d_w0, d_w1, d_g, None, None, None, None
        W0, W1 = w0d * alpha0, w1d * alpha1
        P = emb @ W0
        s1, s2 = _silu_derivs(P)
        Q = c @ W0
        R = Q * s1
        G_h = g @ W1.t()
        cotP = Q * G_h * s2
        d_emb = cotP @ W0.t() if need_emb else None
        d_g = R @ W1 if need_g else None
        if need_w1:
            d_w1 = _launch_wgrad(R, g) * alpha1
        if need_w0:
            d_w0 = (_launch_wgrad(emb, cotP) + _launch_wgrad(c, G_h * s1)) * alpha0
        return d_emb, d_w0, d_w1, d_g, None, None, None, None


# ... 216 lines not shown
```

Baseline: 4.686 million atom-steps/s.

## Fold per-layer gradient sums into kernels via accumulate flags and split grad_x finish

Adds accumulate modes so the radial MLP backward adds into a shared grad-embedding buffer and the pair TP backward adds grad_y atomically into a shared tensor across layers. This removes separate per-layer gradient allocations and the torch add ops that summed them. It also splits the pair backward so the grad_w-ready event fires before the grad_x row-sum finish, letting the side-stream MLP backward start earlier. The grad_x accumulator memset is replaced with a vectorised zero kernel. The cost is more cross-stream coupling and ordering constraints on the shared accumulators.

```diff
diff --git a/include/nequip_amd.h b/include/nequip_amd.h
--- a/include/nequip_amd.h
+++ b/include/nequip_amd.h
@@ -114,6 +114,7 @@
 #define NQA_MLP_BF16X6 1
 #define NQA_MLP_F16X3 2
 #define NQA_MLP_HINT_DEVICE_IS_IDLE 0x100
+#define NQA_MLP_ACCUMULATE 0x200
 int nqa_radial_mlp_supported(int32_t dtype, int32_t num_basis, int32_t hidden, int32_t out_features);
 int64_t nqa_radial_mlp_workspace_bytes(int32_t mode, int32_t backward, int32_t hidden, int32_t out_features);
 int nqa_radial_mlp_fwd(int32_t dtype, int32_t mode, const void* edge_embedding, const void* w0, double alpha0,
@@ -274,6 +275,16 @@
                              const int32_t* pair_edge_out, const int32_t* other_rowptr, const int32_t* other_slot,
                              void* grad_w, void* grad_y, void* grad_x, void* workspace, int64_t workspace_bytes,
                              int64_t num_nodes, int64_t num_edges, nqa_stream stream);
+#define NQA_PAIRS_GY_ACCUMULATE 1
+#define NQA_PAIRS_SKIP_GX_FINISH 2
+#define NQA_PAIRS_ONLY_GX_FINISH 4
+int32_t nqa_tp_bwd_pairs_can_accumulate(const nqa_plan* plan, int32_t dtype);
+int nqa_tp_bwd_pairs_accumulate(const nqa_plan* plan, const void* plan_image, int32_t dtype, const void* x, const void* y,
+                                const void* w, const void* grad_out, const int32_t* owner_rowptr,
+                                const int32_t* pair_other, const int32_t* pair_row, const int32_t* pair_edge_in,
+                                const int32_t* pair_edge_out, const int32_t* other_rowptr, const int32_t* other_slot,
+                                void* grad_w, void* grad_y, void* grad_x, void* workspace, int64_t workspace_bytes,
+                                int64_t num_nodes, int64_t num_edges, int32_t flags, nqa_stream stream);
 
 int32_t nqa_tp_bwd_pairs_dual_supported(const nqa_plan* plan, int32_t dtype);
 int nqa_tp_scatter_bwd_pairs_dual(const nqa_plan* plan, const void* plan_image, int32_t dtype, const void* x,
diff --git a/nequip_amd/_lib.py b/nequip_amd/_lib.py
--- a/nequip_amd/_lib.py
+++ b/nequip_amd/_lib.py
@@ -16,6 +16,8 @@
 NQA_MLP_BF16X6 = 1
 NQA_MLP_F16X3 = 2
 NQA_MLP_HINT_DEVICE_IS_IDLE = 0x100
+NQA_MLP_ACCUMULATE = 0x200
+NQA_PAIRS_GY_ACCUMULATE, NQA_PAIRS_SKIP_GX_FINISH, NQA_PAIRS_ONLY_GX_FINISH = 1, 2, 4
 NQA_LAYOUT_MUL_IR = 0
 NQA_LAYOUT_IR_MUL = 1
 
@@ -159,6 +161,13 @@
         [c_void_p, c_void_p, c_int32, c_void_p, c_void_p, c_void_p, c_void_p]
         + [c_void_p] * 7
         + [c_void_p, c_void_p, c_void_p, c_void_p, c_int64, c_int64, c_int64, c_void_p],
+    ),
+    "nqa_tp_bwd_pairs_can_accumulate": (c_int32, [c_void_p, c_int32]),
+    "nqa_tp_bwd_pairs_accumulate": (
+        c_int32,
+        [c_void_p, c_void_p, c_int32, c_void_p, c_void_p, c_void_p, c_void_p]
+        + [c_void_p] * 7
+        + [c_void_p, c_void_p, c_void_p, c_void_p, c_int64, c_int64, c_int64, c_int32, c_void_p],
     ),
     "nqa_tp_fwd_jvp_supported": (c_int32, [c_void_p, c_int32]),
     "nqa_tp_scatter_fwd_jvp": (
diff --git a/nequip_amd/csrc/radial_mlp.hip b/nequip_amd/csrc/radial_mlp.hip
--- a/nequip_amd/csrc/radial_mlp.hip
+++ b/nequip_amd/csrc/radial_mlp.hip
@@ -874,17 +874,20 @@
 #include "radial_mlp_pipe.h"
 namespace nqa {
 
+constexpr int kMlpBwdAblationMask = 31;
+constexpr int kMlpBwdAccumulate = 32;
 template <int H, int TM, bool PAIR = false, bool F16 = false, bool XIN = false>
 __global__ __launch_bounds__(256, 2) void radial_mlp_bwd_split_kernel(const float* __restrict__ emb,
                                                                     const float* __restrict__ W0,
                                                                     const u32x4* __restrict__ Wb,
                                                                     const float* __restrict__ gw, float a0, int nb,
                                                                     int W, int64_t E, float* __restrict__ g_emb,
-                                                                    int dbg, const float* __restrict__ cemb,
+                                                                    int flags, const float* __restrict__ cemb,
                                                                     float* __restrict__ hid_out,
                                                                     float* __restrict__ w0_part,
                                                                     const float* __restrict__ gw2 = nullptr,
                                                                     const int* __restrict__ chunk_exp = nullptr) {
+  const int dbg = flags & kMlpBwdAblationMask;
   constexpr int NT = H / 32;
   constexpr int NPL = F16 ? 2 : 3;
   constexpr int CH = 2 * NPL * NT * 64;
@@ -1214,7 +1217,12 @@
 #pragma unroll
     for (int c = 0; c < kMaxNb; ++c) sacc[c] += __shfl_xor(sacc[c], 1, 64);
     if (kh == 0 && blk0 + r < E) {
-      for (int c = 0; c < nb; ++c) g_emb[(blk0 + r) * nb + c] = sacc[c];
+      float* __restrict__ orow = g_emb + (blk0 + r) * nb;
+      if (TM == 0 && (flags & kMlpBwdAccumulate)) {
+        for (int c = 0; c < nb; ++c) orow[c] += sacc[c];
+      } else {
+        for (int c = 0; c < nb; ++c) orow[c] = sacc[c];
+      }
     }
   }
   if (TM != 0) {
@@ -1447,9 +1455,13 @@
             void* grad_in) {
   const std::string fn(c.fn);
   const bool device_idle = !c.xin && (c.mode & NQA_MLP_HINT_DEVICE_IS_IDLE) != 0;
-  if (!c.xin) c.mode &= ~NQA_MLP_HINT_DEVICE_IS_IDLE;
+  const bool accumulate = !c.xin && (c.mode & NQA_MLP_ACCUMULATE) != 0;
+  if (!c.xin) c.mode &= ~(NQA_MLP_HINT_DEVICE_IS_IDLE | NQA_MLP_ACCUMULATE);
   int rc = mlp_check(c, gw != nullptr && grad_in != nullptr);
   if (rc != NQA_OK || c.E == 0) return rc;
+  if (accumulate && (tm != 0 || c.mode == NQA_MLP_FP32))
+    return fail(NQA_ERR_UNSUPPORTED, fn + ": NQA_MLP_ACCUMULATE goes with the inference backward of NQA_MLP_BF16X6 / NQA_MLP_F16X3");
+  const int kflags = accumulate ? kMlpBwdAccumulate : 0;
   if (gw == nullptr || grad_in == nullptr || c.W % 4 != 0)
     return fail(NQA_ERR_INVALID, fn + ": invalid argument (needs out_features % 4 == 0)");
   const MlpLayout lay = mlp_layout(c.mode, 1, c.H, c.W);
@@ -1481,7 +1493,7 @@
     int* ce = ws.second_as<int>();
     if (!c.workspace_ready)
       hipLaunchKernelGGL(radial_mlp_split_w1_bwd_f16_kernel, dim3((unsigned)nchunks), dim3(256), 0, s, b, a1, H, W, wb, ce);
-    if (!c.xin && tm == 0 && g2 == nullptr && env_flag("NQA_MLP_PIPE", true)) {
+    if (!c.xin && tm == 0 && g2 == nullptr && !accumulate && env_flag("NQA_MLP_PIPE", true)) {
       const int small_mode = env_int("NQA_MLP_BWD_SMALL", 0);
       if ((small_mode == 2 || (small_mode == 1 && device_idle)) && H == 128 && W % 32 == 0 && W <= 256) {
         const size_t lds = (size_t)nchunks * (2 * 2 * (H / 32) * 64) * 16 + (size_t)(H / 32) * 16 * 2 * kMaxNb * 4 +
@@ -1530,7 +1542,7 @@
         }
       }
       hipLaunchKernelGGL((radial_mlp_bwd_split_kernel<HH, TT, PP, true>), dim3(grid), dim3(256), 0, s, e, a, wb, g, a0, nb,
-                         W, E, o, 0, ct, ho, wp, g2, ce);
+                         W, E, o, kflags, ct, ho, wp, g2, ce);
     });
     return launch_status(launch_fn);
   }
@@ -1543,7 +1555,7 @@
       constexpr int HH = decltype(h)::value, TT = decltype(t)::value;
       constexpr bool PP = decltype(p)::value;
       hipLaunchKernelGGL((radial_mlp_bwd_split_kernel<HH, TT, PP>), dim3(grid), dim3(256), 0, s, e, a, wb, g, a0, nb, W, E,
-                         o, 0, ct, ho, wp, g2, nullptr);
+                         o, kflags, ct, ho, wp, g2, nullptr);
     });
     return launch_status(launch_fn);
   }
diff --git a/nequip_amd/csrc/tp_generic.hip b/nequip_amd/csrc/tp_generic.hip
--- a/nequip_amd/csrc/tp_generic.hip
+++ b/nequip_amd/csrc/tp_generic.hip
@@ -515,6 +515,19 @@
 struct PairForm {
   bool ring, gx_atomic, gy_atomic;
 };
+
+__global__ __launch_bounds__(256) void zero_f32x4_kernel(float4* __restrict__ q, int64_t n4) {
+  const int64_t step = (int64_t)gridDim.x * 256;
+  for (int64_t i = (int64_t)blockIdx.x * 256 + threadIdx.x; i < n4; i += step) q[i] = make_float4(0.f, 0.f, 0.f, 0.f);
+}
+static bool zero_f32(float* p, int64_t n, hipStream_t s) {
+  if (n <= 0) return true;
+  if ((reinterpret_cast<uintptr_t>(p) & 15) != 0 || (n & 3) != 0) return hipMemsetAsync(p, 0, (size_t)n * 4, s) == hipSuccess;
+  const int64_t n4 = n >> 2, want = (n4 + 255) / 256;
+  hipLaunchKernelGGL(zero_f32x4_kernel, dim3((unsigned)(want < 4096 ? want : 4096)), dim3(256), 0, s,
+                     reinterpret_cast<float4*>(p), n4);
+  return hipGetLastError() == hipSuccess;
+}
 static PairForm pair_form(const nqa_plan* plan, const TpWsLayout& l, int64_t N, int64_t E, bool want_gx) {
   const bool R = env_flag("NQA_PAIR_RING", true), A = env_flag("NQA_PAIR_GX_ATOMIC", true);
   const int ring = plan->spec->ring;
@@ -752,13 +765,23 @@
                   num_nodes, num_edges, &paired, static_cast<hipStream_t>(stream));
 }
 
-int nqa_tp_scatter_bwd_pairs(const nqa_plan* plan, const void* plan_image, int32_t dtype, const void* x, const void* y,
-                             const void* w, const void* grad_out, const int32_t* owner_rowptr,
-                             const int32_t* pair_other, const int32_t* pair_row, const int32_t* pair_edge_in,
-                             const int32_t* pair_edge_out, const int32_t* other_rowptr, const int32_t* other_slot,
-                             void* grad_w, void* grad_y, void* grad_x, void* workspace, int64_t workspace_bytes,
-                             int64_t num_nodes, int64_t num_edges, nqa_stream stream) {
+static bool pairs_can_accumulate_gy(const nqa_plan* plan) {
+  return plan->spec->ring == 1 && (plan->uniform_mul & 63) == 0 && env_flag("NQA_PAIR_RING", true) &&
+         env_flag("NQA_PAIR_GX_ATOMIC", true);
+}
+
+static int tp_bwd_pairs(const nqa_plan* plan, const void* plan_image, int32_t dtype, const void* x, const void* y,
+                        const void* w, const void* grad_out, const int32_t* owner_rowptr, const int32_t* pair_other,
+                        const int32_t* pair_row, const int32_t* pair_edge_in, const int32_t* pair_edge_out,
+                        const int32_t* other_rowptr, const int32_t* other_slot, void* grad_w, void* grad_y, void* grad_x,
+                        void* workspace, int64_t workspace_bytes, int64_t num_nodes, int64_t num_edges, int32_t flags,
+                        nqa_stream stream) {
   const char* fn = "nqa_tp_scatter_bwd_pairs";
+  const bool gy_accumulate = (flags & NQA_PAIRS_GY_ACCUMULATE) != 0;
+  const bool skip_finish = (flags & NQA_PAIRS_SKIP_GX_FINISH) != 0, only_finish = (flags & NQA_PAIRS_ONLY_GX_FINISH) != 0;
+  if ((flags & ~(NQA_PAIRS_GY_ACCUMULATE | NQA_PAIRS_SKIP_GX_FINISH | NQA_PAIRS_ONLY_GX_FINISH)) != 0 ||
+      (skip_finish && only_finish))
+    return fail(NQA_ERR_INVALID, "nqa_tp_bwd_pairs_accumulate", ": unknown or contradictory flags");
   int rc = check_common(plan, plan_image, dtype, fn);
   if (rc != NQA_OK) return rc;
   const TpWsLayout l = tp_ws_layout(plan, dtype, TpWs::Pairs, num_edges);
@@ -769,6 +792,9 @@
                          (grad_x && !other_slot) || !grad_w || !grad_y)))
     return fail(NQA_ERR_INVALID, fn, kNullOperand);
   if (num_edges > 0 && (workspace == nullptr || workspace_bytes < l.total)) return fail(NQA_ERR_WORKSPACE, fn, kWorkspace);
+  if (gy_accumulate && !pairs_can_accumulate_gy(plan))
+    return fail(NQA_ERR_UNSUPPORTED, "nqa_tp_bwd_pairs_accumulate",
+                ": this plan's pair kernel cannot add to grad_y (nqa_tp_bwd_pairs_can_accumulate)");
   if (num_nodes == 0) return NQA_OK;
   hipStream_t s = static_cast<hipStream_t>(stream);
   const PairForm form = pair_form(plan, l, num_nodes, num_edges, grad_x != nullptr);
@@ -779,18 +805,28 @@
   a.gxe = grad_x ? gxe : nullptr;
   a.out = static_cast<float*>(grad_x);
   a.gx_atomic = form.gx_atomic;
-  if (form.gx_atomic && hipMemsetAsync(gxe, 0, (size_t)num_nodes * plan->dim_in1 * 4, s) != hipSuccess)
-    return fail(NQA_ERR_LAUNCH, fn, ": hipMemsetAsync of the grad_x accumulator failed");
-  const GyMode mode = l.nchunk == 1 ? GyMode::Direct : (form.gy_atomic ? GyMode::Atomic : GyMode::Partial);
-  if (mode == GyMode::Atomic && hipMemsetAsync(grad_y, 0, (size_t)num_edges * plan->dim_in2 * 4, s) != hipSuccess)
-    return fail(NQA_ERR_LAUNCH, fn, ": hipMemsetAsync of grad_y failed");
-  route_gy(a, l, grad_y, workspace, mode);
-  if (spec_launch(plan, SpecKernel::BwdPairs, a, s, form.ring) != 0) return fail(NQA_ERR_UNSUPPORTED, fn, ": kernel not available");
-  rc = check_launch("nqa_tp_scatter_bwd_pairs(pairs)");
-  if (rc != NQA_OK) return rc;
-  rc = finish_gy(plan, l, grad_y, workspace, mode, num_edges, "nqa_tp_scatter_bwd_pairs(reduce)", s);
-  if (rc != NQA_OK) return rc;
-  if (grad_x == nullptr) return NQA_OK;
+  const auto pairs_pass = [&]() -> int {
+    if (form.gx_atomic) {
+      const int64_t acc_floats = num_nodes * (int64_t)plan->dim_in1;
+      const bool ok = env_set("NQA_NO_STEP_FOLDS")
+                          ? hipMemsetAsync(gxe, 0, (size_t)acc_floats * 4, s) == hipSuccess
+                          : zero_f32(gxe, acc_floats, s);
+      if (!ok) return fail(NQA_ERR_LAUNCH, fn, ": zeroing the grad_x accumulator failed");
+    }
+    const GyMode mode = gy_accumulate ? GyMode::Atomic
+                                      : (l.nchunk == 1 ? GyMode::Direct : (form.gy_atomic ? GyMode::Atomic : GyMode::Partial));
+    if (mode == GyMode::Atomic && !gy_accumulate &&
+        hipMemsetAsync(grad_y, 0, (size_t)num_edges * plan->dim_in2 * 4, s) != hipSuccess)
+      return fail(NQA_ERR_LAUNCH, fn, ": hipMemsetAsync of grad_y failed");
+    route_gy(a, l, grad_y, workspace, mode);
+    if (spec_launch(plan, SpecKernel::BwdPairs, a, s, form.ring) != 0) return fail(NQA_ERR_UNSUPPORTED, fn, ": kernel not available");
+    rc = check_launch("nqa_tp_scatter_bwd_pairs(pairs)");
+    if (rc != NQA_OK) return rc;
+    rc = finish_gy(plan, l, grad_y, workspace, mode, num_edges, "nqa_tp_scatter_bwd_pairs(reduce)", s);
+    return rc;
+  };
+  if (!only_finish && (rc = pairs_pass()) != NQA_OK) return rc;
+  if (grad_x == nullptr || skip_finish) return NQA_OK;
   SpecArgs<float> b = spec_node_operands(plan, num_nodes);
   b.gxe = gxe;
   b.out = static_cast<float*>(grad_x);
@@ -804,6 +840,32 @@
   if (spec_launch(plan, SpecKernel::RowsSumPairs, b, s) != 0)
     return fail(NQA_ERR_UNSUPPORTED, fn, ": this structure has no grad_x row-sum kernel");
   return check_launch("nqa_tp_scatter_bwd_pairs(sum)");
+}
+
+int nqa_tp_scatter_bwd_pairs(const nqa_plan* plan, const void* plan_image, int32_t dtype, const void* x, const void* y,
+                             const void* w, const void* grad_out, const int32_t* owner_rowptr,
+                             const int32_t* pair_other, const int32_t* pair_row, const int32_t* pair_edge_in,
+                             const int32_t* pair_edge_out, const int32_t* other_rowptr, const int32_t* other_slot,
+                             void* grad_w, void* grad_y, void* grad_x, void* workspace, int64_t workspace_bytes,
+                             int64_t num_nodes, int64_t num_edges, nqa_stream stream) {
+  return tp_bwd_pairs(plan, plan_image, dtype, x, y, w, grad_out, owner_rowptr, pair_other, pair_row, pair_edge_in,
+                      pair_edge_out, other_rowptr, other_slot, grad_w, grad_y, grad_x, workspace, workspace_bytes, num_nodes,
+                      num_edges, 0, stream);
+}
+
+int32_t nqa_tp_bwd_pairs_can_accumulate(const nqa_plan* plan, int32_t dtype) {
+  return (plan != nullptr && tp_ws_layout(plan, dtype, TpWs::Pairs, 0).total >= 0 && pairs_can_accumulate_gy(plan)) ? 1 : 0;
+}
+
+int nqa_tp_bwd_pairs_accumulate(const nqa_plan* plan, const void* plan_image, int32_t dtype, const void* x, const void* y,
+                                 const void* w, const void* grad_out, const int32_t* owner_rowptr,
+                                 const int32_t* pair_other, const int32_t* pair_row, const int32_t* pair_edge_in,
+                                 const int32_t* pair_edge_out, const int32_t* other_rowptr, const int32_t* other_slot,
+                                 void* grad_w, void* grad_y, void* grad_x, void* workspace, int64_t workspace_bytes,
+                                 int64_t num_nodes, int64_t num_edges, int32_t flags, nqa_stream stream) {
+  return tp_bwd_pairs(plan, plan_image, dtype, x, y, w, grad_out, owner_rowptr, pair_other, pair_row, pair_edge_in,
+                      pair_edge_out, other_rowptr, other_slot, grad_w, grad_y, grad_x, workspace, workspace_bytes, num_nodes,
+                      num_edges, flags, stream);
 }
 
 int32_t nqa_tp_bwd_pairs_dual_supported(const nqa_plan* plan, int32_t dtype) {
diff --git a/nequip_amd/nn/_paired_radial.py b/nequip_amd/nn/_paired_radial.py
--- a/nequip_amd/nn/_paired_radial.py
+++ b/nequip_amd/nn/_paired_radial.py
@@ -12,6 +12,10 @@
 
 
 _side_streams = {}
+
+
+def step_folds() -> bool:
+    return os.environ.get("NQA_NO_STEP_FOLDS", "") in ("", "0")
 
 
 def side_stream(device: torch.device, slot: int = 0) -> torch.cuda.Stream:
@@ -29,6 +33,23 @@
         self.layers = 0
         self.acc = None
         self.pending = None
+        self.fold = step_folds()
+        self.y_ref = None
+        self.y_shared = True
+        self.gy = None
+
+    def saw_y(self, y: torch.Tensor) -> None:
+        if self.y_ref is None:
+            self.y_ref = y
+        elif self.y_ref is not y:
+            self.y_shared = False
+
+    def abandon(self, cur: "torch.cuda.Stream") -> None:
+        cur.wait_stream(self.stream)
+        self.reset()
+
+    def reset(self) -> None:
+        self.acc, self.layers, self.pending, self.gy = None, 0, None, None
 
     @staticmethod
     def lagged() -> bool:
@@ -43,8 +64,11 @@
         def item():
             self.stream.wait_event(ready)
             with torch.cuda.stream(self.stream):
-                part = launch()
-                self.acc = part if self.acc is None else self.acc.add_(part)
+                if self.fold:
+                    self.acc = launch(self.acc)
+                else:
+                    part = launch(None)
+                    self.acc = part if self.acc is None else self.acc.add_(part)
             for t in reads:
                 t.record_stream(self.stream)
 
@@ -93,43 +117,67 @@
         gx = gy = G = None
         fused = None
         folded = False
-        if need_emb and need_x and need_y and k.prefer_fused_bwd and os.environ.get("NQA_NO_FUSED_BWD", "") in ("", "0"):
-            if _pair_backward_pays(g):
-                fused = k.bwd_pairs(x, y, w_half, g, topo, pairing)
-                folded = fused is not None
-            if fused is None and k.fused_rows_ok:
-                fused = k.bwd_fused(x, y, w_half, g, topo, pairing=pairing)
-        if fused is not None:
-            gx, G, gy = fused
-        else:
-            if need_x:
-                gx = k.bwd_x(y, w_half, g, topo, pairing)
-            pairs = k.bwd_pairs(x, y, w_half, g, topo, pairing, need_gx=False) if (need_emb and need_y and _pair_backward_pays(g)) else None
-            if pairs is not None:
-                _, G, gy = pairs
-                folded = True
+        q = ctx.queue
+        sum_gy = q is not None and q.fold and q.y_shared and need_emb and need_y
+        gy_into = q.gy if (sum_gy and _pair_backward_pays(g) and k.pairs_accumulate_gy(x.dtype)) else None
+        ready = None
+        mark = None
+        if gy_into is not None:
+            ready = torch.cuda.Event()
+            fork_stream = torch.cuda.current_stream(g.device)
+            mark = lambda: ready.record(fork_stream)
+        try:
+            if need_emb and need_x and need_y and k.prefer_fused_bwd and os.environ.get("NQA_NO_FUSED_BWD", "") in ("", "0"):
+                if _pair_backward_pays(g):
+                    fused = k.bwd_pairs(x, y, w_half, g, topo, pairing, gy_into=gy_into, gw_ready=mark)
+                    folded = fused is not None
+                if fused is None and k.fused_rows_ok:
+                    fused = k.bwd_fused(x, y, w_half, g, topo, pairing=pairing)
+            if fused is not None:
+                gx, G, gy = fused
             else:
-                G, gy = k.bwd_edge(x, y, w_half, g, topo, need_gw=need_emb, need_gy=need_y, pairing=pairing)
+                if need_x:
+                    gx = k.bwd_x(y, w_half, g, topo, pairing)
+                pairs = (k.bwd_pairs(x, y, w_half, g, topo, pairing, need_gx=False, gy_into=gy_into, gw_ready=mark)
+                         if (need_emb and need_y and _pair_backward_pays(g)) else None)
+                if pairs is not None:
+                    _, G, gy = pairs
+                    folded = True
+                else:
+                    G, gy = k.bwd_edge(x, y, w_half, g, topo, need_gw=need_emb, need_gy=need_y, pairing=pairing)
+        except BaseException:
+            if q is not None:
+                q.abandon(torch.cuda.current_stream(g.device))
+            raise
+        if need_emb and q is not None and not (folded and mark is not None):
+            ready = torch.cuda.Event()
+            ready.record(torch.cuda.current_stream(g.device))
         g_emb = None
-        q = ctx.queue
         if q is not None:
             q.layers -= 1
+        if sum_gy:
+            if q.gy is None:
+                q.gy = gy
+            elif gy is not q.gy:
+                q.gy.add_(gy)
+            gy = q.gy
+            if q.layers > 0:
+                gy = None
+            else:
+                q.gy = None
         if need_emb and q is not None:
             cur = torch.cuda.current_stream(g.device)
             try:
-                ready = torch.cuda.Event()
-                ready.record(cur)
                 last = q.layers <= 0
 
-                def launch():
+                def launch(into):
                     if folded:
-                        return _mlp._launch_bwd(emb_half, w0, w1, alpha0, alpha1, G, mode, cache, device_idle=last)
-                    return _mlp._launch_bwd_paired(emb_half, w0, w1, alpha0, alpha1, G[:P], G[P:], mode, cache)
+                        return _mlp._launch_bwd(emb_half, w0, w1, alpha0, alpha1, G, mode, cache, device_idle=last, into=into)
+                    return _mlp._launch_bwd_paired(emb_half, w0, w1, alpha0, alpha1, G[:P], G[P:], mode, cache, into=into)
 
                 q.submit(launch, ready, (G, emb_half, w0, w1), last)
             except BaseException:
-                cur.wait_stream(q.stream)
-                q.acc, q.layers, q.pending = None, 0, None
+                q.abandon(cur)
                 raise
             if q.layers <= 0:
                 assert q.acc is not None and q.layers == 0, "radial backward queue out of step with the layers"
@@ -216,6 +264,8 @@
     if differentiable_parameters(edge_mlp.training, edge_mlp.mlp[0].weight, edge_mlp.mlp[2].weight):
         w_half = edge_mlp(emb_half)
         return tp_scatter(x, edge_attr, w_half, topo._dst, topo._src, topology=topo, pairing=pairing)
+    if queue is not None:
+        queue.saw_y(edge_attr)
     return _PairedRadialTPFn.apply(
         emb_half, x, edge_attr, edge_mlp.mlp[0].weight.detach(), edge_mlp.mlp[2].weight.detach(),
         edge_mlp._alphas[0], edge_mlp._alphas[1], _mlp.radial_mlp_mode(), cache, tp_scatter._get_kernels(), topo, pairing,
diff --git a/nequip_amd/nn/_tp_scatter_base.py b/nequip_amd/nn/_tp_scatter_base.py
--- a/nequip_amd/nn/_tp_scatter_base.py
+++ b/nequip_amd/nn/_tp_scatter_base.py
@@ -152,7 +152,10 @@
                        gw, gy, gx, ws, ws_bytes, N, E)
         return gx, gw, gy
 
-    def bwd_pairs(self, x, y, w, g, topo: EdgeTopology, pairing, need_gx: bool = True):
+    def pairs_accumulate_gy(self, dtype: torch.dtype) -> bool:
+        return bool(_lib.load().nqa_tp_bwd_pairs_can_accumulate(self.plan.handle, _nqa_dtype(dtype)))
+
+    def bwd_pairs(self, x, y, w, g, topo: EdgeTopology, pairing, need_gx: bool = True, gy_into=None, gw_ready=None):
         lib = _lib.load()
         E, N = topo.num_edges, topo.num_nodes
         ws_bytes = lib.nqa_tp_bwd_pairs_workspace_bytes(self.plan.handle, _nqa_dtype(x.dtype), E)
@@ -162,15 +165,37 @@
         P = pairing.num_pairs
         gx = torch.empty((N, self.dim_in1), dtype=x.dtype, device=x.device) if need_gx else None
         gw = torch.empty((P, self.weight_numel), dtype=x.dtype, device=x.device)
-        gy = torch.empty((E, self.dim_in2), dtype=x.dtype, device=x.device)
+        if gy_into is not None:
+            assert gy_into.shape == (E, self.dim_in2) and gy_into.dtype == x.dtype and gy_into.is_contiguous()
+            gy = gy_into
+        else:
+            gy = torch.empty((E, self.dim_in2), dtype=x.dtype, device=x.device)
         ws = torch.empty(max(ws_bytes, 1), dtype=torch.uint8, device=x.device)
         owner = pairing.owner_csr
         es = x.element_size()
         nbytes = E * (es * (2 * self.weight_numel + 2 * self.dim_in2) + 16) + N * es * (
             (2 if need_gx else 1) * self.dim_in1 + self.dim_out)
+        split = gw_ready is not None and need_gx
+        flags = _lib.NQA_PAIRS_GY_ACCUMULATE if gy_into is not None else 0
+
+        def launch(fl: int) -> None:
+            rc = lib.nqa_tp_bwd_pairs_accumulate(
+                self.plan.handle, _ptr(self.image), _nqa_dtype(x.dtype), *(_ptr(t) for t in (x, y, w, g, *owner, gw, gy, gx, ws)),
+                ws_bytes, N, E, fl, current_stream_ptr(x.device))
+            _lib.check(rc, "nqa_tp_bwd_pairs_accumulate")
+
         with torch.cuda.device(x.device), ktimer.region("tp_bwd_fused" if need_gx else "tp_bwd_edge", nbytes, 0.0,
                                                         E * es * 2 * self.weight_numel, self.weight_numel):
-            self._call("bwd_pairs", None, None, x, x, y, w, g, *owner, gw, gy, gx, ws, ws_bytes, N, E)
+            if split:
+                launch(flags | _lib.NQA_PAIRS_SKIP_GX_FINISH)
+                gw_ready()
+                launch(flags | _lib.NQA_PAIRS_ONLY_GX_FINISH)
+            elif flags:
+                launch(flags)
+            else:
+                self._call("bwd_pairs", None, None, x, x, y, w, g, *owner, gw, gy, gx, ws, ws_bytes, N, E)
+        if gw_ready is not None and not split:
+            gw_ready()
         return gx, gw, gy
 
     def fwd_jvp(self, x, y, w, c_x, c_y, c_w, topo: EdgeTopology, pairing=None) -> torch.Tensor:
diff --git a/nequip_amd/nn/embedding/_edge.py b/nequip_amd/nn/embedding/_edge.py
--- a/nequip_amd/nn/embedding/_edge.py
+++ b/nequip_amd/nn/embedding/_edge.py
@@ -215,6 +215,10 @@
         _lib.check(rc, "nqa_edge_embed_fwd_paired")
         ctx.save_for_backward(vec, bessel_weights)
         ctx.cfg, ctx.pairing = cfg, pairing
+        from .._paired_radial import step_folds
+
+        if step_folds():
+            ctx.set_materialize_grads(False)
         return sh, emb, emb_pairs
 
     @staticmethod
diff --git a/nequip_amd/nn/mlp.py b/nequip_amd/nn/mlp.py
--- a/nequip_amd/nn/mlp.py
+++ b/nequip_amd/nn/mlp.py
@@ -80,11 +80,19 @@
     return out
 
 
-def _launch_bwd(emb, w0, w1, alpha0: float, alpha1: float, g_w, mode: int, cache: _WeightImages, device_idle: bool = False):
+def _accumulator(into, emb):
+    if into is None:
+        return torch.empty_like(emb), 0
+    assert into.shape == emb.shape and into.dtype == emb.dtype and into.device == emb.device and into.is_contiguous()
+    return into, _lib.NQA_MLP_ACCUMULATE
+
+
+def _launch_bwd(emb, w0, w1, alpha0: float, alpha1: float, g_w, mode: int, cache: _WeightImages, device_idle: bool = False,
+                into=None):
     E, nb = emb.shape
     H, W = w1.shape
-    g_emb = torch.empty_like(emb)
-    hint = _lib.NQA_MLP_HINT_DEVICE_IS_IDLE if device_idle else 0
+    g_emb, acc = _accumulator(into, emb)
+    hint = (_lib.NQA_MLP_HINT_DEVICE_IS_IDLE if device_idle else 0) | acc
     _launch("nqa_radial_mlp_bwd", region="radial_mlp_bwd", nbytes=4.0 * E * (2 * nb + W),
             flops=2.0 * E * (nb * H * 2 + H * W), resolve=backward_mode, mode=mode, backward=1, w1=w1, cache=cache, rows=E,
             device=emb.device, alloc=lambda: (g_emb,),
@@ -120,15 +128,15 @@
     return out
 
 
-def _launch_bwd_paired(emb, w0, w1, alpha0: float, alpha1: float, g_a, g_b, mode: int, cache: _WeightImages):
+def _launch_bwd_paired(emb, w0, w1, alpha0: float, alpha1: float, g_a, g_b, mode: int, cache: _WeightImages, into=None):
     E, nb = emb.shape
     H, W = w1.shape
     assert g_a.shape == (E, W) and g_b.shape == (E, W) and g_a.is_contiguous() and g_b.is_contiguous()
-    g_emb = torch.empty_like(emb)
+    g_emb, acc = _accumulator(into, emb)
     _launch("nqa_radial_mlp_bwd_paired", region="radial_mlp_bwd", nbytes=4.0 * E * (2 * nb + 2 * W),
             flops=2.0 * E * (nb * H * 2 + H * W), resolve=backward_mode, mode=mode, backward=1, w1=w1, cache=cache, rows=E,
             device=emb.device, alloc=lambda: (g_emb,),
-            call=lambda fn, m, outs, *ws: fn(_lib.NQA_F32, m, _P(emb), _P(w0), alpha0, _P(w1), alpha1, _P(g_a), _P(g_b), nb,
+            call=lambda fn, m, outs, *ws: fn(_lib.NQA_F32, m | acc, _P(emb), _P(w0), alpha0, _P(w1), alpha1, _P(g_a), _P(g_b), nb,
                                              H, W, E, _P(g_emb), *ws))
     return g_emb
 
```

Measured after the change: 4.702 million atom-steps/s (median of 2 runs). Within noise of the previous version (+0.3%).
